# alexlee-gk/video_prediction

Measured on AMD Instinct MI355X. Metric: train frames/sec (whole node), BAIR 64x64 seq30 SAVP, higher is better.
Workload: dtype bf16

## Files before the change

### include/savp_hip.h

```cpp
#ifndef SAVP_HIP_H
#define SAVP_HIP_H

#include <stdint.h>

#ifdef __cplusplus
extern "C" {
#endif

#define SAVP_OK 0
#define SAVP_EINVAL (-1)
#define SAVP_ELAUNCH (-2)

const char* savp_version(void);

int savp_set_option(const char* name, int32_t value);
int savp_get_option(const char* name, int32_t* value);

int savp_allreduce_bucket(void* comm, void* stream, void* buf, int64_t count);

int savp_prof_event_create(void** ev);
int savp_prof_event_destroy(void* ev);
int savp_prof_arm(void* start, void* stop);
int savp_prof_armed(void);
int savp_prof_elapsed_us(void* start, void* stop, float* us);

enum { SAVP_CONV_FPROP = 0, SAVP_CONV_DGRAD = 1, SAVP_CONV_WGRAD = 2 };
enum { SAVP_PREC_F32 = 0, SAVP_PREC_BF16 = 1 };
enum { SAVP_ACT_NONE = 0, SAVP_ACT_LRELU = 1, SAVP_ACT_SIGMOID = 2, SAVP_ACT_DLRELU_FROM_OUT = 3 };

typedef struct SavpConvArgs {
    int32_t mode;
    int32_t N, D, H, W, Cx;
    int32_t Do, Ho, Wo, Cy;
    int32_t kd, kh, kw;
    int32_t sd, sh, sw;
    int32_t pd, ph, pw;
    int32_t beta;
    int32_t act;
    float alpha;
    int32_t splitk;
    int32_t tile;
    int32_t precision;
    void* x; int64_t x_sn, x_sd, x_sh, x_sw;
    void* y; int64_t y_sn, y_sd, y_sh, y_sw;
    void* w;
    const float* bias;
    const float* aux;
    const void* w_bf16;
    int32_t src_bf16;
    int32_t out_bf16;
    double* stats;
    void* ws; int64_t ws_bytes;
    int32_t dst_gap_at, dst_gap;
    const float* nb_x; int64_t nb_x_sn, nb_x_sp;
    const float *nb_mean, *nb_rstd;
    const float *nb_gamma, *nb_beta;
    double* nb_ws;
    int32_t nb_c0, nb_nc, nb_act; float nb_alpha;
    const void* w_frag;
    const void* w_frag_il;
} SavpConvArgs;

int savp_conv(void* stream, const SavpConvArgs* args);

int savp_tiled_z_weff(void* stream, const float* w, int32_t kh, int32_t kw, int32_t ph, int32_t pw, int32_t Cin, int32_t Cout,
                      int32_t z0, int32_t nz, float* weff);
int savp_tiled_z_grad(void* stream, const void* dy, int32_t dy_bf16, int64_t nimg, int32_t H, int32_t W, int32_t C,
                      const float* weff, int32_t nz, float* dz, int32_t beta, void* ws, int64_t ws_bytes);
int64_t savp_tiled_z_workspace_bytes(int64_t nimg, int32_t C);
int savp_conv_stats_ok(const SavpConvArgs* args);
int64_t savp_conv_workspace_bytes(const SavpConvArgs* args);
int savp_conv_special(const SavpConvArgs* args);


typedef struct SavpView { void* p; int64_t sn; int64_t sp; } SavpView;

typedef struct SavpInormArgs {
    int32_t N, HW, C;
    int32_t act; float alpha; float eps;
    SavpView x;
    const float* gamma; const float* beta;
    int32_t nout; SavpView out[4];
    float* mean; float* rstd;
    int32_t ndy; SavpView dy[4];
    SavpView dx; int32_t dx_beta;
    double* dgamma; double* dbeta;
    void* ws;
    int32_t ws_clean;
    int32_t out_c0[4], out_nc[4];
    int32_t dy_c0[4], dy_nc[4];
    int32_t out_bf16;
    int32_t stats_ready;
    const float* stats_shift;
    int32_t dx_bf16;
} SavpInormArgs;
int savp_instnorm_act_fwd(void* stream, const SavpInormArgs* a);
int savp_instnorm_act_bwd(void* stream, const SavpInormArgs* a);

typedef struct SavpGnormArgs {
    SavpInormArgs norm;
    int32_t G;
    double* ws_group;
    double* dsum;
} SavpGnormArgs;
int savp_groupnorm_act_fwd(void* stream, const SavpGnormArgs* a);
int savp_groupnorm_act_bwd(void* stream, const SavpGnormArgs* a);

typedef struct SavpLnLstmArgs {
    int32_t N, HW, F; float forget_bias;
    const float* gn;
    SavpView c_prev;
    float* c_pre;
    const float* cn;
    int32_t nh; SavpView h[4]; int32_t h_bf16;
    int32_t ndh; SavpView dh[4];
    const float* dc_new;
    float* dcn;
    float* dgn;
    const float* dc_pre;
    float* dc_prev;
} SavpLnLstmArgs;
int savp_lnlstm_fwd(void* stream, const SavpLnLstmArgs* a, int32_t stage);
int savp_lnlstm_bwd(void* stream, const SavpLnLstmArgs* a, int32_t stage);

typedef struct SavpLstmArgs {
    int32_t N, HW, F;
    float eps, forget_bias;
    const void* gates;
    SavpView c_prev;
    const float *gamma1, *beta1, *gamma2, *beta2;
    float* c_new;
    int32_t nh; SavpView h[4];
    float *mean1, *rstd1, *mean2, *rstd2;
    int32_t ndh; SavpView dh[4];
    const float* dc_new;
    float* dgates;
    float* dc_prev;
    double *dgamma1, *dbeta1, *dgamma2, *dbeta2;
    float* ws; int64_t ws_floats;
    float* ws_stats;
    int32_t ws_stats_clean;
    int32_t gates_bf16;
    int32_t stats1_ready;
    int32_t h_bf16;
    int32_t dgates_bf16;
    float* dgates_raw;
    int32_t no_norm;
} SavpLstmArgs;
int savp_convlstm_gates_fwd(void* stream, const SavpLstmArgs* a);
int savp_convlstm_gates_bwd(void* stream, const SavpLstmArgs* a);

int savp_tile_channels(void* stream, const float* z, int64_t R, int32_t HW, int32_t C, float scale, SavpView out, int32_t beta);
int savp_tile_channels_bf16(void* stream, const float* z, int64_t R, int32_t HW, int32_t C, float scale, SavpView out);
#define SAVP_COLSUM_WS_FLOATS (1024 * 4 * 256)
int savp_colsum(void* stream, SavpView in, int64_t R, int32_t HW, int32_t C, float scale, float* out, int32_t per_row,
                float* ws, int64_t ws_floats);
int savp_select(void* stream, int32_t N, int32_t HW, int32_t C, const int32_t* mask, SavpView a, SavpView b, int32_t nout,
                const SavpView* outs);
int savp_select_bwd(void* stream, int32_t N, int32_t HW, int32_t C, const int32_t* mask, int32_t nin, const SavpView* dins,
                    SavpView db);
int savp_gather_clips(void* stream, float* src, float* dst, const int32_t* t_start, int32_t B, int32_t clip, int64_t E,
                      int64_t src_t_stride, int32_t adjoint);
int savp_sigmoid_bwd(void* stream, SavpView dy, SavpView y, float* out, int64_t N, int32_t HW, int32_t C);
int savp_dense_fwd(void* stream, const float* x, int64_t x_row_stride, int32_t M, int64_t K, int32_t C, const float* W,
                   const float* bias, const float* scale, float* out, float* ws, int64_t ws_floats);
int savp_axpby(void* stream, int64_t n, float a, const float* x, float b, const float* y, float* out);
int savp_fill_view(void* stream, SavpView out, int64_t R, int32_t HW, int32_t C, float value);
int savp_adam(void* stream, int64_t n, float* p, const float* g, float* m, float* v, float lr_t, float beta1, float beta2,
              float eps, float gscale, const float* lr_t_dev);

int savp_cdna_kernels_fwd(void* stream, const float* raw, float* kern, int32_t N, int32_t kh, int32_t kw, int32_t K);
int savp_cdna_kernels_bwd(void* stream, const float* raw, const double* dkern, float* draw, int32_t N, int32_t kh, int32_t kw,
                          int32_t K);
typedef struct SavpCdnaArgs {
    int32_t N, H, W, C, K, kh, kw;
    SavpView img;
    const float* kern;
    SavpView out;
    SavpView dout;
    SavpView dimg; int32_t dimg_beta;
    double* dkern;
} SavpCdnaArgs;
int savp_cdna_apply_fwd(void* stream, const SavpCdnaArgs* a);
int savp_cdna_apply_bwd(void* stream, const SavpCdnaArgs* a);
#define SAVP_MAX_SOURCES 4
typedef struct SavpCdnaMultiArgs {
    int32_t N, H, W, C, K, kh, kw;
    int32_t nsrc;
    SavpView img[SAVP_MAX_SOURCES];
    const float* kern;
    SavpView out;
    SavpView dout;
    SavpView dimg[SAVP_MAX_SOURCES]; int32_t dimg_beta[SAVP_MAX_SOURCES];
    double* dkern;
} SavpCdnaMultiArgs;
int savp_cdna_apply_multi_fwd(void* stream, const SavpCdnaMultiArgs* a);
int savp_cdna_apply_multi_bwd(void* stream, const SavpCdnaMultiArgs* a);
typedef struct SavpCompositeArgs {
    int32_t N, HW, M, C;
    const float* logits;
    int32_t logits_stride;
    SavpView timgs;
    SavpView gen;
    float* masks;
    SavpView dgen;
    float* dlogits;
    SavpView drow;
    int32_t timgs_offset, row_channels;
    int32_t nnext; SavpView next[2];
    const int32_t* gt_mask;
    SavpView gt_img;
} SavpCompositeArgs;
int savp_composite_fwd(void* stream, const SavpCompositeArgs* a);
int savp_composite_bwd(void* stream, const SavpCompositeArgs* a);

typedef struct SavpConvLstmCellArgs { SavpConvArgs conv; SavpLstmArgs gates; } SavpConvLstmCellArgs;
typedef struct SavpConvNormArgs { SavpConvArgs conv; SavpInormArgs norm; } SavpConvNormArgs;
int savp_convlstm_cell_fwd(void* stream, const SavpConvLstmCellArgs* a);
int savp_convlstm_cell_bwd(void* stream, const SavpConvLstmCellArgs* a);
int savp_conv_in_act_fwd(void* stream, const SavpConvNormArgs* a);
int savp_conv_in_act_bwd(void* stream, const SavpConvNormArgs* a);

int savp_lstm_z_fwd(void* stream, const float* zs, const float* W, const float* bias, float* hout, float* gates, float* cs,
                    int32_t T, int32_t B, int32_t nz, float forget_bias);
int savp_lstm_z_bwd(void* stream, const float* zs, const float* W, const float* hout, const float* gates, const float* cs,
                    const float* dh_out, float* dzs, double* dW, double* db, int32_t T, int32_t B, int32_t nz, float forget_bias);
int savp_lstm_z_fwd_init(void* stream, const float* zs, const float* W, const float* bias, float* hout, float* gates, float* cs,
                         int32_t T, int32_t B, int32_t nz, float forget_bias, const float* c0, const float* h0);
int savp_lstm_z_bwd_init(void* stream, const float* zs, const float* W, const float* hout, const float* gates, const float* cs,
                         const float* dh_out, float* dzs, double* dW, double* db, int32_t T, int32_t B, int32_t nz, float forget_bias,
                         const float* c0, const float* h0, double* dc0, double* dh0);
int savp_lstm_seq_fwd(void* stream, float* A, const float* W, const float* bias, float* hout, float* gates, float* cs,
                      int32_t T, int32_t B, int32_t I, int32_t U, float forget_bias);
int savp_lstm_seq_bwd(void* stream, const float* A, const float* W, const float* gates, const float* cs, const float* dh_out,
                      float* dG, float* dA, int32_t T, int32_t B, int32_t I, int32_t U, float forget_bias);
int savp_gru_seq_fwd(void* stream, float* A, float* A2, const float* Wg, const float* bg, const float* Wc, const float* bc, float* hout,
                     float* ru, float* cand, int32_t T, int32_t B, int32_t I, int32_t U);
int savp_gru_seq_bwd(void* stream, const float* A, const float* Wg, const float* Wc, const float* ru, const float* cand, const float* dh_out,
                     float* dGg, float* dGc, float* dA, int32_t T, int32_t B, int32_t I, int32_t U);
int savp_gru_seq_fwd_init(void* stream, float* A, float* A2, const float* Wg, const float* bg, const float* Wc, const float* bc, float* hout,
                          float* ru, float* cand, int32_t T, int32_t B, int32_t I, int32_t U, const float* h0);
int savp_gru_seq_bwd_init(void* stream, const float* A, const float* Wg, const float* Wc, const float* ru, const float* cand, const float* dh_out,
                          float* dGg, float* dGc, float* dA, int32_t T, int32_t B, int32_t I, int32_t U, double* dh0);
int savp_kl_gauss(void* stream, int64_t n, int32_t rows, const float* mu1, const float* ls1_raw, const float* mu2,
                  const float* ls2_raw, double* kl_out, float klw, const float* klw_dev, float* dmu1, float* dls1, float* dmu2,
                  float* dls2);
int savp_reparam_fwd(void* stream, int64_t n, int32_t rows, const float* mu, const float* ls_raw, const float* eps, float* ls,
                     float* z, double* kl_out);
int savp_reparam_bwd(void* stream, int64_t n, int32_t rows, const float* mu, const float* ls_raw, const float* eps,
                     const float* dz, float klw, float* dmu, float* dls_raw, const float* klw_dev);
int savp_lp_loss(void* stream, int64_t rows, int64_t row_len, int64_t pred_row_stride, int64_t target_row_stride, int32_t p2,
                 const float* pred, const float* target, float weight, double* loss_out, float* dpred);
int savp_tv_loss(void* stream, const float* flows, int32_t n_img, int32_t H, int32_t W, int32_t C, int64_t img_stride, int64_t px_stride,
                 float s1, float s2, float weight, double* loss_out, float* dflows);
int savp_gan_loss(void* stream, int32_t n, int32_t type, const float* logits, float label, float weight, double* loss_out,
                  float* dlogits, int32_t beta);
int savp_lsgan_loss(void* stream, int32_t n, const float* logits, float label, float weight, double* loss_out, float* dlogits,
                    int32_t beta);
int savp_cosine_distance(void* stream, int64_t P, int32_t C, const float* f0, const float* f1, float weight, float eps,
                         double* loss_out, float* df0, int32_t beta);

int savp_pack_weights(void* stream, const float* src, int64_t T, int32_t Cx, int32_t Cy, const float* scale, float* wt, float* wd,
                      void* wt_bf16, void* wd_bf16);

typedef struct {
    const float* src; const float* scale;
    float* wt; float* wd; void* wt_bf16; void* wd_bf16;
    int64_t T; int32_t Cx, Cy;
} SavpPackItem;
int savp_pack_weights_batch(void* stream, int32_t n, const SavpPackItem* items);
int savp_fold_pool(void* stream, const float* in, float* out, int32_t k, int64_t C, int32_t adjoint);
int savp_fold_bilinear(void* stream, const float* in, float* out, int32_t k, int32_t Cin, int32_t F, int32_t adjoint);
int savp_sn_fwd(void* stream, const float* W, int64_t K, int32_t C, const float* u, float* ws, float* u_new);
int savp_sn_bwd(void* stream, const float* W, int64_t K, int32_t C, const float* u, float* ws, const float* G, float* dW,
                int32_t beta);
typedef struct SavpSnItem {
    const float* W; int64_t K; int32_t C; const float* u; float* ws; float* u_new; const float* G; float* dW; int32_t beta;
} SavpSnItem;
int savp_sn_fwd_batch(void* stream, int32_t n, const SavpSnItem* items);
int savp_sn_bwd_batch(void* stream, int32_t n, const SavpSnItem* items);

typedef struct SavpWarpArgs {
    int32_t N, H, W, C, K;
    SavpView img;
    const float* flows;
    SavpView out;
    SavpView dout;
    float* dflows;
    float* dimg;
} SavpWarpArgs;
int savp_image_warp_fwd(void* stream, const SavpWarpArgs* a);
int savp_image_warp_bwd(void* stream, const SavpWarpArgs* a);
typedef struct SavpDnaArgs {
    int32_t N, H, W, C, K, kh, kw;
    SavpView img;
    const float* raw;
    float* kern;
    SavpView out;
    SavpView dout;
    float* draw;
    SavpView dimg; int32_t dimg_beta;
} SavpDnaArgs;
int savp_dna_apply_fwd(void* stream, const SavpDnaArgs* a);
int savp_dna_apply_bwd(void* stream, const SavpDnaArgs* a);
typedef struct SavpWarpMultiArgs {
    int32_t N, H, W, C, K;
    int32_t nsrc;
    SavpView img[SAVP_MAX_SOURCES];
    const float* flows;
    SavpView out;
    SavpView dout;
    float* dflows;
    SavpView dimg[SAVP_MAX_SOURCES]; int32_t dimg_beta[SAVP_MAX_SOURCES];
} SavpWarpMultiArgs;
int savp_image_warp_multi_fwd(void* stream, const SavpWarpMultiArgs* a);
int savp_image_warp_multi_bwd(void* stream, const SavpWarpMultiArgs* a);
typedef struct SavpDnaMultiArgs {
    int32_t N, H, W, C, K, kh, kw;
    int32_t nsrc;
    SavpView img[SAVP_MAX_SOURCES];
    const float* raw;
    float* kern;
    SavpView out;
    SavpView dout;
    float* draw;
    SavpView dimg[SAVP_MAX_SOURCES]; int32_t dimg_beta[SAVP_MAX_SOURCES];
} SavpDnaMultiArgs;
int savp_dna_apply_multi_fwd(void* stream, const SavpDnaMultiArgs* a);
int savp_dna_apply_multi_bwd(void* stream, const SavpDnaMultiArgs* a);

typedef struct SavpGruArgs {
    int32_t N, HW, F;
    float eps;
    const float* pre;
    SavpView h;
    const float *gamma, *beta;
    float *mean, *rstd;
    float* u;
    SavpView rh;
    int32_t nout; SavpView out[4];
    int32_t ndy; SavpView dy[4];
    float* dpre;
    float* du;
    SavpView dh;
    SavpView drh;
    double *dgamma, *dbeta;
} SavpGruArgs;
int savp_convgru_gates_fwd(void* stream, const SavpGruArgs* a);
int savp_convgru_out_fwd(void* stream, const SavpGruArgs* a);
int savp_convgru_out_bwd(void* stream, const SavpGruArgs* a);
int savp_convgru_gates_bwd(void* stream, const SavpGruArgs* a);

int savp_u8_frames_to_f32(void* stream, const uint8_t* in, float* out, int32_t B, int32_t T, int64_t frame);

int savp_frame_mse_psnr(void* stream, const float* a, int64_t a_st, int64_t a_sb, const float* b, int64_t b_st, int64_t b_sb,
                        int32_t T, int32_t B, int32_t inner, float* mse, float* psnr);
int savp_frame_ssim(void* stream, const float* a, int64_t a_st, int64_t a_sb, const float* b, int64_t b_st, int64_t b_sb,
                    int32_t T, int32_t B, int32_t H, int32_t W, int32_t C, float* out);
int savp_eval_accumulate(void* stream, const float* metric, float* vmin, float* vsum, float* vmax, int32_t* cond_min,
                         int32_t* cond_max, int32_t T, int32_t B);
int savp_select_batch(void* stream, const int32_t* cond, const float* x, int64_t x_st, int64_t x_sb, float* out, int64_t o_st,
                      int64_t o_sb, int32_t T, int32_t B, int32_t inner, int32_t mode);

#define SAVP_EVAL_PSNR 0
#define SAVP_EVAL_MSE 1
#define SAVP_EVAL_SSIM 2
#define SAVP_EVAL_NMETRICS 3
typedef struct {
    float *vmin, *vsum, *vmax;
    float *gmin, *gsum, *gmax;
} SavpEvalFoldState;
int64_t savp_eval_fold_ws_floats(int32_t F, int32_t S, int32_t B, int32_t C);
int savp_eval_fold_samples(void* stream, const float* target, int64_t t_st, int64_t t_sb, const float* pred, int64_t p_st, int64_t p_sb,
                           int32_t F, int32_t T1, int32_t S, int32_t B, int32_t H, int32_t W, int32_t C, const int32_t* n_valid,
                           const SavpEvalFoldState* states, float* ws, int64_t ws_floats);

int savp_fold_f64(void* stream, const int32_t* idx, int64_t n, double* src, float* dst);

int savp_state_pred_fwd(void* stream, int32_t T, int32_t N, int32_t na, int32_t ns, const float* actions, const float* states_in,
                        const int32_t* gt, const float* W, const float* b, float* sa, float* gen);
int savp_state_pred_bwd(void* stream, int32_t T, int32_t N, int32_t na, int32_t ns, const int32_t* gt, const float* W, const float* sa,
                        float* dgen, double* dW, double* db);

int64_t savp_gate_weights_bytes(int32_t taps, int32_t Cx, int32_t Cy);
int savp_pack_gate_weights(void* stream, const float* src, int32_t taps, int32_t Cx, int32_t Cy, void* out, int32_t interleave);

int savp_debug_poison_lds(void* stream, uint32_t pattern, void* sink);
int savp_debug_fill_u32(void* stream, void* p, int64_t words, uint32_t pattern);
int savp_debug_probe_lds(void* stream, uint32_t pattern, void* out2);

#ifdef __cplusplus
}
#endif
#endif
```

### video_prediction_amd/csrc/common.hip

```cpp
#include <hip/hip_runtime.h>
#include <dlfcn.h>
#include <string.h>
#include "savp_hip.h"
#include "opts.h"
#include "conv_common.h"

extern "C" const char* savp_version(void) { return "savp_hip 0.1 gfx950"; }

thread_local hipEvent_t g_savp_prof_start = nullptr;
thread_local hipEvent_t g_savp_prof_stop = nullptr;

extern "C" int savp_prof_event_create(void** ev) {
    if (!ev) return SAVP_EINVAL;
    hipEvent_t e;
    if (hipEventCreate(&e) != hipSuccess) return SAVP_ELAUNCH;
    *ev = (void*)e;
    return SAVP_OK;
}
extern "C" int savp_prof_event_destroy(void* ev) { return (ev && hipEventDestroy((hipEvent_t)ev) == hipSuccess) ? SAVP_OK : SAVP_EINVAL; }
extern "C" int savp_prof_arm(void* start, void* stop) {
    if ((start == nullptr) != (stop == nullptr)) return SAVP_EINVAL;
    g_savp_prof_start = (hipEvent_t)start; g_savp_prof_stop = (hipEvent_t)stop;
    return SAVP_OK;
}
extern "C" int savp_prof_armed(void) { return g_savp_prof_start != nullptr; }
extern "C" int savp_prof_elapsed_us(void* start, void* stop, float* us) {
    if (!start || !stop || !us) return SAVP_EINVAL;
    float ms = 0.f;
    if (hipEventElapsedTime(&ms, (hipEvent_t)start, (hipEvent_t)stop) != hipSuccess) return SAVP_ELAUNCH;
    *us = ms * 1e3f;
    return SAVP_OK;
}

static struct { const char* name; int value; } g_opts[OPT_COUNT] = {
    {"conv_ring", 0}, {"s2dgrad", 1}, {"thin", 1}, {"wgp_cfg", 0}, {"wgp_split", 0}, {"inorm_min_hw", 64}, {"colsum_2stage", 1},
    {"dense_legacy", 0}, {"cdna_legacy", 0}, {"lstm_fused", 1}, {"ring_dma", 1}, {"lstm_q", 0}, {"ring_wwarm", 1}, {"wgp_dma", 1}, {"ring_early", 1}, {"gate_kernel", 1}, {"gate_alt", 0}, {"gate_cell", 1}, {"gate_wwarm", 1}, {"splitk_reduced", 0},
};
int savp_opt(int id) { return g_opts[id].value; }
void savp_opt_count(int id) { ++g_opts[id].value; }
extern "C" int savp_set_option(const char* name, int value) {
    if (!name) return SAVP_EINVAL;
    for (int i = 0; i < OPT_COUNT; ++i)
        if (!strcmp(g_opts[i].name, name)) { g_opts[i].value = value; return SAVP_OK; }
    return SAVP_EINVAL;
}
extern "C" int savp_get_option(const char* name, int* value) {
    if (!name || !value) return SAVP_EINVAL;
    for (int i = 0; i < OPT_COUNT; ++i)
        if (!strcmp(g_opts[i].name, name)) { *value = g_opts[i].value; return SAVP_OK; }
    return SAVP_EINVAL;
}

typedef int (*rccl_allreduce_fn)(const void*, void*, size_t, int, int, void*, hipStream_t);
extern "C" int savp_allreduce_bucket(void* comm, void* stream, void* buf, int64_t count) {
    if (!comm || !buf || count < 0) return SAVP_EINVAL;
    if (count == 0) return SAVP_OK;
    static rccl_allreduce_fn fn = nullptr;
    if (!fn) {
        void* h = dlopen("librccl.so", RTLD_NOW | RTLD_GLOBAL);
        if (!h) h = dlopen("librccl.so.1", RTLD_NOW | RTLD_GLOBAL);
        if (!h) h = dlopen("/opt/rocm/lib/librccl.so", RTLD_NOW | RTLD_GLOBAL);
        if (!h) return SAVP_ELAUNCH;
        fn = (rccl_allreduce_fn)dlsym(h, "ncclAllReduce");
        if (!fn) return SAVP_ELAUNCH;
    }
    return fn(buf, buf, (size_t)count, 7, 0, comm, (hipStream_t)stream) == 0 ? SAVP_OK : SAVP_ELAUNCH;
}

int splitk_fit(const SavpConvArgs* a, int want, long long block_elems) {
    if (want <= 1) return 1;
    if (!a->ws || a->ws_bytes <= 0 || block_elems <= 0 || (((uintptr_t)a->ws) & 15)) { savp_opt_count(OPT_SPLITK_REDUCED); return 1; }
    const long long fit = a->ws_bytes / (block_elems * (long long)sizeof(float));
    if (fit < want) savp_opt_count(OPT_SPLITK_REDUCED);
    if (fit < 2) return 1;
    return want < fit ? want : (int)fit;
}

__global__ __launch_bounds__(256) void splitk_fold_kernel(float* __restrict__ out, const float* __restrict__ part, int splitk, long long n4, long long n,
                                                          int beta, int Cd, int gap_at, int gap) {
    const long long stride = (long long)gridDim.x * 256;
    for (long long i = (long long)blockIdx.x * 256 + threadIdx.x; i < n4; i += stride) {
        float4 s = beta ? reinterpret_cast<const float4*>(out)[i] : make_float4(0.f, 0.f, 0.f, 0.f);
        for (int k = 0; k < splitk; ++k) {
            const float4 v = reinterpret_cast<const float4*>(part + (long long)k * n)[i];
            s.x += v.x; s.y += v.y; s.z += v.z; s.w += v.w;
        }
        if (gap) {
            const int c = (int)((i * 4) % Cd);
            float* e = &s.x;
#pragma unroll
            for (int j = 0; j < 4; ++j)
                if (c + j >= gap_at && c + j < gap_at + gap) e[j] = beta ? reinterpret_cast<const float*>(out)[i * 4 + j] : 0.f;
        }
        reinterpret_cast<float4*>(out)[i] = s;
    }
}

__global__ __launch_bounds__(256) void splitk_fold_scalar_kernel(float* __restrict__ out, const float* __restrict__ part, int splitk, long long n, int beta,
                                                                 int Cd, int gap_at, int gap) {
    const long long stride = (long long)gridDim.x * 256;
    for (long long i = (long long)blockIdx.x * 256 + threadIdx.x; i < n; i += stride) {
        const int c = (int)(i % Cd);
        if (gap && c >= gap_at && c < gap_at + gap) { if (!beta) out[i] = 0.f; continue; }
        float s = beta ? out[i] : 0.f;
        for (int k = 0; k < splitk; ++k) s += part[(long long)k * n + i];
        out[i] = s;
    }
}

void splitk_fold(float* out, const float* part, int splitk, long long n, int beta, int Cd, int gap_at, int gap, hipStream_t st) {
    const bool vec = (n % 4 == 0) && (Cd % 4 == 0) && ((((uintptr_t)out) & 15) == 0) && ((((uintptr_t)part) & 15) == 0);
    const long long work = vec ? n / 4 : n;
    long long blocks = (work + 255) / 256;
    if (blocks > 2048) blocks = 2048;
    if (blocks < 1) blocks = 1;
    if (vec) hipLaunchKernelGGL(splitk_fold_kernel, dim3((unsigned)blocks), dim3(256), 0, st, out, part, splitk, n / 4, n, beta, Cd, gap_at, gap);
    else hipLaunchKernelGGL(splitk_fold_scalar_kernel, dim3((unsigned)blocks), dim3(256), 0, st, out, part, splitk, n, beta, Cd, gap_at, gap);
}

typedef float fold_f4 __attribute__((ext_vector_type(4)));
template <bool VEC>
__global__ __launch_bounds__(256) void wgrad_fold_kernel(float* __restrict__ out, const float* __restrict__ part, int nsplit, long long n, long long slice) {
    const long long i = (long long)blockIdx.x * 256 + threadIdx.x;
    if (i >= n) return;
    if constexpr (VEC) {
        fold_f4 s = reinterpret_cast<const fold_f4*>(out)[i];
        const fold_f4* __restrict__ q = reinterpret_cast<const fold_f4*>(part) + i;
        const long long st4 = slice >> 2;
        int k = 0;
        for (; k + 8 <= nsplit; k += 8) {
            fold_f4 v[8];
#pragma unroll
            for (int j = 0; j < 8; ++j) v[j] = __builtin_nontemporal_load(q + (long long)(k + j) * st4);
#pragma unroll
            for (int j = 0; j < 8; ++j) s += v[j];
        }
        for (; k < nsplit; ++k) s += __builtin_nontemporal_load(q + (long long)k * st4);
        reinterpret_cast<fold_f4*>(out)[i] = s;
    } else {
        float s = out[i];
        for (int k = 0; k < nsplit; ++k) s += part[(long long)k * slice + i];
        out[i] = s;
    }
}

void wgrad_fold(float* out, const float* part, int nsplit, long long n, hipStream_t st, long long slice) {
    if (nsplit < 1 || n <= 0) return;
    if (slice <= 0) slice = n;
    const bool vec = (n % 4 == 0) && (slice % 4 == 0) && ((((uintptr_t)out) & 15) == 0) && ((((uintptr_t)part) & 15) == 0);
    const long long work = vec ? n / 4 : n;
    const unsigned blocks = (unsigned)((work + 255) / 256);
    if (vec) hipLaunchKernelGGL(wgrad_fold_kernel<true>, dim3(blocks), dim3(256), 0, st, out, part, nsplit, work, slice);
    else hipLaunchKernelGGL(wgrad_fold_kernel<false>, dim3(blocks), dim3(256), 0, st, out, part, nsplit, work, slice);
}
```

### video_prediction_amd/csrc/conv_common.h

```cpp
#pragma once
#include <hip/hip_runtime.h>
#include <stdint.h>
#include "savp_hip.h"
#include "opts.h"

typedef float f32x16 __attribute__((ext_vector_type(16)));
typedef __bf16 bf16x8 __attribute__((ext_vector_type(8)));
typedef __bf16 bf16x4 __attribute__((ext_vector_type(4)));

#define BK 32
#define BKP 36
#define NTHREADS 256

struct DimGeom {
    int Mdim;
    int base, mstep;
    int jstep;
    int nt;
    int t0, tstep;
    int ob, os;
    int srcN;
};

__host__ __device__ __forceinline__ DimGeom make_geom(bool dgrad, int f, int In, int Out, int k, int s, int p) {
    DimGeom g;
    if (!dgrad) {
        g.Mdim = Out; g.base = -p; g.mstep = s; g.jstep = 1; g.nt = k; g.t0 = 0; g.tstep = 1;
        g.ob = 0; g.os = 1; g.srcN = In;
    } else {
        int u0 = (f + p) % s;
        g.nt = (k > u0) ? (k - u0 + s - 1) / s : 0;
        g.base = (f + p - u0) / s; g.mstep = 1; g.jstep = -1;
        g.t0 = u0; g.tstep = s;
        g.Mdim = (In > f) ? (In - f + s - 1) / s : 0;
        g.ob = f; g.os = s; g.srcN = Out;
    }
    return g;
}

struct ConvP {
    int mode;
    int N, D, H, W, Cx;
    int Do, Ho, Wo, Cy;
    int kd, kh, kw, sd, sh, sw, pd, ph, pw;
    int beta, act;
    float alpha;
    const float* x; long long x_sn, x_sd, x_sh, x_sw;
    const float* y; long long y_sn, y_sd, y_sh, y_sw;
    const float* w;
    const unsigned short* w16;
    float* out;
    const float* bias;
    const float* aux;
    int splitk;
    float* part; long long part_sz;
    int bf16;
    int tm, tn;
    unsigned long long magW, magHW, magDHW;
    int s1_pitch, s1_nch, s1_spp;
    int s1_ph, s1_pw, s1_th, s1_tw, s1_tih;
    unsigned long long s1_magDm;
    unsigned long long s1_magPI, s1_magPW, s1_magC4;
    int src16;
    int cell;
    double* stats;
    int dma_patch;
    const void* zero16;
    unsigned long long s1_magPI8, s1_magP8, s1_magC8;
    int pre;
    const float* nb_x; long long nb_x_sn, nb_x_sp; const float *nb_mean, *nb_rstd, *nb_gamma, *nb_beta; double* nb_ws;
    int nb_c0, nb_nc, nb_act; float nb_alpha;
    int gap_at, gap;
    int wwarm;
    int early;
    DimGeom gD, gH, gW;
    int s1_tih_sh;
    int s1_ngs, s1_itper;
    unsigned long long s1_magTm, s1_magTHW, s1_magTW;
    unsigned long long s1_magKw, s1_magSpp, s1_magTail;
};

__device__ __forceinline__ unsigned fastdiv(unsigned p, unsigned long long magic) {
    return (unsigned)(((unsigned long long)p * magic) >> 40);
}

__device__ __forceinline__ float4 ldg4(const float* p) { return *reinterpret_cast<const float4*>(p); }

__device__ __forceinline__ int xcd_logical(int b, int n) {
    const int q = n >> 3, r = n & 7, xcd = b & 7;
    return (xcd < r ? xcd * (q + 1) : r * (q + 1) + (xcd - r) * q) + (b >> 3);
}


static inline unsigned long long magic40(int d) {
    if (d <= 0) d = 1;
    return ((1ULL << 40) + (unsigned long long)d - 1ULL) / (unsigned long long)d;
}

static inline void patch_launch_constants(ConvP& p, const SavpConvArgs* a, int phases, int tih, int nch, int spp, int tW, int splitk) {
    const bool dg = a->mode == SAVP_CONV_DGRAD;
    int sh_ = 0;
    while ((1 << sh_) < tih) ++sh_;
    p.s1_tih_sh = sh_;
    const int ngs = (nch + spp - 1) / spp;
    p.s1_ngs = ngs;
    p.pre = 0;
    if (phases != 1 || (dg && (a->sh != 1 || a->sw != 1))) return;
    p.gD = make_geom(dg, 0, a->D, a->Do, a->kd, 1, a->pd);
    p.gH = make_geom(dg, 0, a->H, a->Ho, a->kh, a->sh, a->ph);
    p.gW = make_geom(dg, 0, a->W, a->Wo, a->kw, a->sw, a->pw);
    const long long it_all = (long long)p.gD.nt * p.gH.nt * p.gW.nt * nch;
    p.s1_itper = (int)((it_all + splitk - 1) / splitk);
    const int thw = p.s1_th * tW;
    p.s1_magTm = magic40(p.tm); p.s1_magTHW = magic40(thw); p.s1_magTW = magic40(tW);
    p.s1_magKw = magic40(p.gW.nt); p.s1_magSpp = magic40(spp); p.s1_magTail = magic40(nch - (ngs - 1) * spp);
    if ((long long)p.tm * p.tn < (1 << 24) && p.tm < 65536 && thw < 65536 && it_all < (1 << 24) && p.gW.nt >= 1 && p.gH.nt >= 1) p.pre = 1;
}

bool conv_thin_try(const SavpConvArgs* a, hipStream_t st, int* rc);
bool conv_thin_applies(const SavpConvArgs* a);
long long conv_thin_workspace_bytes(const SavpConvArgs* a);

bool conv_s2dgrad_try(const SavpConvArgs* a, hipStream_t st, int* rc);
bool conv_s2dgrad_applies(const SavpConvArgs* a);

extern thread_local hipEvent_t g_savp_prof_start, g_savp_prof_stop;

int splitk_fit(const SavpConvArgs* a, int want, long long block_elems);
void splitk_fold(float* out, const float* part, int splitk, long long n, int beta, int Cd, int gap_at, int gap, hipStream_t st);

static inline bool aligned16(const void* p) { return (((uintptr_t)p) & 15) == 0; }

#ifdef SAVP_CONV_ABLATE
#include <stdlib.h>
static __constant__ int g_ablate;
#define ABL(bit) (g_ablate & (bit))
static inline void ablate_init() {
    static bool done = false;
    if (!done) { const char* e = getenv("SAVP_ABLATE"); int v = e ? atoi(e) : 0; hipMemcpyToSymbol(HIP_SYMBOL(g_ablate), &v, sizeof(int)); done = true; }
}
#else
#define ABL(bit) false
static inline void ablate_init() {}
#endif

bool conv_patch_try(ConvP& p, const SavpConvArgs* a, int wm, int wn, bool forced, hipStream_t st, int* rc);
bool conv_wgrad_patch_try(ConvP& p, const SavpConvArgs* a, hipStream_t st, int* rc, long long* plan_bytes = nullptr);
void wgrad_fold(float* out, const float* part, int nsplit, long long n, hipStream_t st, long long slice = 0);
bool conv_ring_try(ConvP& p, const SavpConvArgs* a, int wm, int wn, hipStream_t st, int* rc, bool dry = false);
bool conv_gate_applies(const SavpConvArgs* a);
bool conv_gate_try(const SavpConvArgs* a, hipStream_t st, int* rc);
struct SavpConvLstmCellArgs;
bool conv_gate_cell_try(const SavpConvLstmCellArgs* c, hipStream_t st, int* rc);
```

### video_prediction_amd/csrc/conv_igemm.hip

```cpp
#include <hip/hip_runtime.h>
#include <stdint.h>
#include "savp_hip.h"
#include "zero_fill.h"

#include "conv_common.h"
#include <stdlib.h>

template <int WM, int WN, bool VEC, bool BF16, bool WB16>
__global__ __launch_bounds__(NTHREADS) void conv_fd_kernel(ConvP p) {
    constexpr int BM = 64 * WM, BN = 64 * WN;
    constexpr int BKT = BF16 ? 64 : 32;
    constexpr int KV = BKT / 4;
    constexpr int RP = NTHREADS / KV;
    constexpr int RA = BM / RP, RB = BN / RP;
    constexpr int ROWB = BF16 ? (BKT + 8) * 2 : BKP * 4;
    extern __shared__ __attribute__((aligned(16))) float smem[];
    char* As = reinterpret_cast<char*>(smem);
    char* Bs = As + 2 * BM * ROWB;

    const bool dgrad = (p.mode == SAVP_CONV_DGRAD);
    const int split = blockIdx.z % p.splitk;
    int fz = blockIdx.z / p.splitk;
    int fw = dgrad ? fz % p.sw : 0; fz = dgrad ? fz / p.sw : 0;
    int fh = dgrad ? fz % p.sh : 0; fz = dgrad ? fz / p.sh : 0;
// ... 449 lines not shown

template <int WM, int WN>
__global__ __launch_bounds__(NTHREADS) void conv_wgrad_bf16_kernel(ConvP p) {
    constexpr int BM = 64 * WM, BN = 64 * WN;
    constexpr int BKT = 64;
    constexpr int ROWB = (BKT + 8) * 2;
    constexpr int PA = BM / 64, PB = BN / 64;
    extern __shared__ __attribute__((aligned(16))) float smem[];
    char* As = reinterpret_cast<char*>(smem);
    char* Bs = As + 2 * BM * ROWB;

    const int M = p.kd * p.kh * p.kw * p.Cx;
    const int Nn = p.Cy;
    const int HWo = p.Ho * p.Wo, DHWo = p.Do * HWo;
    const int Ktot = p.N * DHWo;
    const int llog = xcd_logical(blockIdx.x, p.tm * p.tn * p.splitk);
    const int zsplit = llog / (p.tm * p.tn), tl = llog % (p.tm * p.tn);
    const int m0 = (tl % p.tm) * BM, n0 = (tl / p.tm) * BN;
    const int ktiles = (Ktot + BKT - 1) / BKT;
    const int per = (ktiles + p.splitk - 1) / p.splitk;
    const int kt_begin = zsplit * per;
    const int kt_end = min(ktiles, kt_begin + per);
    if (kt_begin >= kt_end) return;

    const float* __restrict__ X = p.x;
    const float* __restrict__ Y = p.y;
    const int tid = threadIdx.x, lane = tid & 63, wave = tid >> 6;
    const int kq = tid & 15, rq0 = tid >> 4;

    int a_c[PA], a_td[PA], a_th[PA], a_tw[PA]; bool a_ok[PA];
#pragma unroll
    for (int j = 0; j < PA; ++j) {
        int m = m0 + 4 * (rq0 + 16 * j);
        a_ok[j] = m < M;
        int mm = a_ok[j] ? m : 0;
        a_c[j] = mm % p.Cx; int tap = mm / p.Cx;
        a_tw[j] = tap % p.kw; tap /= p.kw;
        a_th[j] = tap % p.kh; a_td[j] = tap / p.kh;
    }
    int b_n[PB]; bool b_ok[PB];
#pragma unroll
    for (int j = 0; j < PB; ++j) { b_n[j] = n0 + 4 * (rq0 + 16 * j); b_ok[j] = b_n[j] < Nn; }

    float4 ra[PA][4], rb[PB][4];

    auto fetch = [&](int kt) {
        if (ABL(1)) return;
#pragma unroll
        for (int i = 0; i < 4; ++i) {
            const int pix = kt * BKT + kq * 4 + i;
            const bool pok = pix < Ktot;
            unsigned up = (unsigned)(pok ? pix : 0);
            int n = (int)fastdiv(up, p.magDHW); unsigned r = up - (unsigned)n * DHWo;
            int od = (int)fastdiv(r, p.magHW); r -= (unsigned)od * HWo;
            int oy = (int)fastdiv(r, p.magW); int ox = (int)(r - (unsigned)oy * p.Wo);
            const long long nb = (long long)n * p.x_sn;
#pragma unroll
            for (int j = 0; j < PA; ++j) {
                int zd = od * p.sd - p.pd + a_td[j], zh = oy * p.sh - p.ph + a_th[j], zw = ox * p.sw - p.pw + a_tw[j];
                float4 v = make_float4(0.f, 0.f, 0.f, 0.f);
                if (pok && a_ok[j] && (unsigned)zd < (unsigned)p.D && (unsigned)zh < (unsigned)p.H && (unsigned)zw < (unsigned)p.W)
                    v = ldg4(X + nb + zd * p.x_sd + zh * p.x_sh + zw * p.x_sw + a_c[j]);
                ra[j][i] = v;
            }
            const float* q = Y + (long long)n * p.y_sn + od * p.y_sd + oy * p.y_sh + ox * p.y_sw;
#pragma unroll
            for (int j = 0; j < PB; ++j) {
                float4 v = make_float4(0.f, 0.f, 0.f, 0.f);
                if (pok && b_ok[j]) v = ldg4(q + b_n[j]);
                rb[j][i] = v;
            }
        }
    };
    auto stage = [&](int buf) {
        if (ABL(64)) return;
        char* a = As + buf * BM * ROWB;
        char* b = Bs + buf * BN * ROWB;
#pragma unroll
        for (int j = 0; j < PA; ++j) {
            char* base = a + (4 * (rq0 + 16 * j)) * ROWB + kq * 8;
            bf16x4 v0 = {(__bf16)ra[j][0].x, (__bf16)ra[j][1].x, (__bf16)ra[j][2].x, (__bf16)ra[j][3].x};
            bf16x4 v1 = {(__bf16)ra[j][0].y, (__bf16)ra[j][1].y, (__bf16)ra[j][2].y, (__bf16)ra[j][3].y};
            bf16x4 v2 = {(__bf16)ra[j][0].z, (__bf16)ra[j][1].z, (__bf16)ra[j][2].z, (__bf16)ra[j][3].z};
            bf16x4 v3 = {(__bf16)ra[j][0].w, (__bf16)ra[j][1].w, (__bf16)ra[j][2].w, (__bf16)ra[j][3].w};
            *reinterpret_cast<bf16x4*>(base) = v0;
            *reinterpret_cast<bf16x4*>(base + ROWB) = v1;
            *reinterpret_cast<bf16x4*>(base + 2 * ROWB) = v2;
            *reinterpret_cast<bf16x4*>(base + 3 * ROWB) = v3;
        }
#pragma unroll
        for (int j = 0; j < PB; ++j) {
            char* base = b + (4 * (rq0 + 16 * j)) * ROWB + kq * 8;
            bf16x4 v0 = {(__bf16)rb[j][0].x, (__bf16)rb[j][1].x, (__bf16)rb[j][2].x, (__bf16)rb[j][3].x};
            bf16x4 v1 = {(__bf16)rb[j][0].y, (__bf16)rb[j][1].y, (__bf16)rb[j][2].y, (__bf16)rb[j][3].y};
            bf16x4 v2 = {(__bf16)rb[j][0].z, (__bf16)rb[j][1].z, (__bf16)rb[j][2].z, (__bf16)rb[j][3].z};
            bf16x4 v3 = {(__bf16)rb[j][0].w, (__bf16)rb[j][1].w, (__bf16)rb[j][2].w, (__bf16)rb[j][3].w};
            *reinterpret_cast<bf16x4*>(base) = v0;
            *reinterpret_cast<bf16x4*>(base + ROWB) = v1;
            *reinterpret_cast<bf16x4*>(base + 2 * ROWB) = v2;
            *reinterpret_cast<bf16x4*>(base + 3 * ROWB) = v3;
        }
    };

    f32x16 acc[WM][WN];
#pragma unroll
    for (int i = 0; i < WM; ++i)
#pragma unroll
        for (int j = 0; j < WN; ++j)
#pragma unroll
            for (int r = 0; r < 16; ++r) acc[i][j][r] = 0.f;

    const int wm0 = (wave >> 1) * 32 * WM, wn0 = (wave & 1) * 32 * WN;
    const int l31 = lane & 31, khalf = lane >> 5;

    fetch(kt_begin);
    stage(0);
    __syncthreads();
    for (int kt = kt_begin; kt < kt_end; ++kt) {
        const int cur = (kt - kt_begin) & 1;
        if (kt + 1 < kt_end) fetch(kt + 1);
        const char* a = As + cur * BM * ROWB;
        const char* b = Bs + cur * BN * ROWB;
#pragma unroll
        for (int ks = 0; ks < (ABL(2) ? 0 : BKT / 16); ++ks) {
            bf16x8 af[WM], bf[WN];
#pragma unroll
            for (int i = 0; i < WM; ++i)
                af[i] = *reinterpret_cast<const bf16x8*>(a + (wm0 + i * 32 + l31) * ROWB + (ks * 16 + khalf * 8) * 2);
#pragma unroll
            for (int j = 0; j < WN; ++j)
                bf[j] = *reinterpret_cast<const bf16x8*>(b + (wn0 + j * 32 + l31) * ROWB + (ks * 16 + khalf * 8) * 2);
#pragma unroll
            for (int i = 0; i < WM; ++i)
#pragma unroll
                for (int j = 0; j < WN; ++j)
                    acc[i][j] = __builtin_amdgcn_mfma_f32_32x32x16_bf16(af[i], bf[j], acc[i][j], 0, 0, 0);
        }
        if (kt + 1 < kt_end) stage(cur ^ 1);
        __syncthreads();
    }

    const bool sliced = p.part != nullptr;
    float* __restrict__ dW = sliced ? p.part + (long long)zsplit * p.part_sz : p.out;
#pragma unroll
    for (int j = 0; j < WN; ++j) {
        const int col = n0 + wn0 + j * 32 + l31;
        if (col >= Nn) continue;
#pragma unroll
        for (int i = 0; i < WM; ++i)
#pragma unroll
            for (int r = 0; r < 16; ++r) {
                const int row = m0 + wm0 + i * 32 + (r & 3) + 8 * (r >> 2) + 4 * khalf;
                if (row < M) {
                    if (sliced) dW[(long long)row * Nn + col] = acc[i][j][r];
                    else unsafeAtomicAdd(dW + (long long)row * Nn + col, acc[i][j][r]);
                }
            }
    }
}

template <int WM, int WN>
static hipError_t launch_wg_bf16(const ConvP& p, dim3 grid, hipStream_t st) {
    size_t lds = (size_t)2 * (64 * WM + 64 * WN) * (64 + 8) * 2;
    static bool attr_done = false;
    if (!attr_done) {
        hipFuncSetAttribute((const void*)conv_wgrad_bf16_kernel<WM, WN>, hipFuncAttributeMaxDynamicSharedMemorySize, (int)lds);
        attr_done = true;
    }
    hipLaunchKernelGGL((conv_wgrad_bf16_kernel<WM, WN>), grid, dim3(NTHREADS), lds, st, p);
    return hipGetLastError();
}


template <int WM, int WN, bool VEC, bool BF16, bool WB16 = false>
static hipError_t launch_fd1(const ConvP& p, dim3 grid, hipStream_t st) {
    constexpr int BKT = BF16 ? 64 : 32;
    constexpr size_t rowb = BF16 ? (BKT + 8) * 2 : BKP * 4;
    size_t lds = (size_t)2 * (64 * WM + 64 * WN) * rowb;
    if (lds < (size_t)64 * WM * sizeof(long long)) lds = (size_t)64 * WM * sizeof(long long);
    static bool attr_done = false;
    if (!attr_done) {
        hipFuncSetAttribute((const void*)conv_fd_kernel<WM, WN, VEC, BF16, WB16>, hipFuncAttributeMaxDynamicSharedMemorySize, (int)lds);
        attr_done = true;
    }
    hipLaunchKernelGGL((conv_fd_kernel<WM, WN, VEC, BF16, WB16>), grid, dim3(NTHREADS), lds, st, p);
    return hipGetLastError();
}

template <int WM, int WN>
static hipError_t launch_fd(const ConvP& p, bool vec, dim3 grid, hipStream_t st) {
    if (p.bf16 && vec && p.w16) return launch_fd1<WM, WN, true, true, true>(p, grid, st);
    if (p.bf16) return vec ? launch_fd1<WM, WN, true, true>(p, grid, st) : launch_fd1<WM, WN, false, true>(p, grid, st);
    return vec ? launch_fd1<WM, WN, true, false>(p, grid, st) : launch_fd1<WM, WN, false, false>(p, grid, st);
}

template <int WM, int WN>
static hipError_t launch_wg(const ConvP& p, bool va, bool vb, dim3 grid, hipStream_t st) {
    size_t lds = (size_t)2 * BK * ((64 * WM + 4) + (64 * WN + 4)) * sizeof(float);
#define WG_CASE(A, B)                                                                                              \
    {                                                                                                              \
        hipFuncSetAttribute((const void*)conv_wgrad_kernel<WM, WN, A, B>, hipFuncAttributeMaxDynamicSharedMemorySize, \
                            (int)lds);                                                                             \
        hipLaunchKernelGGL((conv_wgrad_kernel<WM, WN, A, B>), grid, dim3(NTHREADS), lds, st, p);                   \
    }
    if (va && vb) WG_CASE(true, true)
    else if (va) WG_CASE(true, false)
    else if (vb) WG_CASE(false, true)
    else WG_CASE(false, false)
#undef WG_CASE
    return hipGetLastError();
}


static void pick_tile(long long M, long long N, int& wm, int& wn) {
    const int opts[4][2] = {{2, 2}, {2, 1}, {1, 2}, {1, 1}};
    double best = 1e300;
    for (int i = 0; i < 4; ++i) {
        long long bm = 64 * opts[i][0], bn = 64 * opts[i][1];
        long long tm = (M + bm - 1) / bm, tn = (N + bn - 1) / bn;
        double wgs = (double)tm * tn;
        double rounds = wgs <= 256.0 ? 1.0 : wgs / 256.0;
        double eff = (bm * bn == 128 * 128) ? 1.0 : (bm * bn == 64 * 64 ? 1.3 : 1.12);
        double cost = rounds * (double)(bm * bn) * eff;
        if (cost < best) { best = cost; wm = opts[i][0]; wn = opts[i][1]; }
    }
}

static bool ring_default() {
    return savp_opt(OPT_CONV_RING) != 0;
}

struct WgPlan { int wm, wn, splitk; long long M, ktiles, part_sz; bool va, vb, wbf16; };
static bool wgrad_generic_plan(const SavpConvArgs* a, bool bf16, int wm, int wn, WgPlan& g) {
    const bool xs4 = (a->x_sn % 4 == 0) && (a->x_sd % 4 == 0) && (a->x_sh % 4 == 0) && (a->x_sw % 4 == 0) && aligned16(a->x);
    const bool ys4 = (a->y_sn % 4 == 0) && (a->y_sd % 4 == 0) && (a->y_sh % 4 == 0) && (a->y_sw % 4 == 0) && aligned16(a->y);
    g.M = (long long)a->kd * a->kh * a->kw * a->Cx;
    const long long Ktot = (long long)a->N * a->Do * a->Ho * a->Wo;
    if (Ktot <= 0 || (double)Ktot * (double)((long long)a->Do * a->Ho * a->Wo) >= 1099511627776.0) return false;
    g.va = (a->Cx % 4 == 0) && xs4;
    g.vb = (a->Cy % 4 == 0) && ys4;
    if (!wm) {
        wm = (g.M > 64) ? 2 : 1;
        wn = (a->Cy > 64) ? 2 : 1;
    }
    g.wm = wm; g.wn = wn;
    const int BM = 64 * wm, BN = 64 * wn;
    const long long tiles = ((g.M + BM - 1) / BM) * ((a->Cy + BN - 1) / BN);
    g.wbf16 = bf16 && g.va && g.vb;
    const int bkt = g.wbf16 ? 64 : BK;
    g.ktiles = (Ktot + bkt - 1) / bkt;
    long long splitk = a->splitk;
    if (splitk <= 0) {
        long long want = (512 + tiles - 1) / tiles;
        long long maxs = g.ktiles / 8 > 0 ? g.ktiles / 8 : 1;
        splitk = want < maxs ? want : maxs;
    }
    if (splitk > g.ktiles) splitk = g.ktiles;
    if (splitk < 1) splitk = 1;
    const long long per = (g.ktiles + splitk - 1) / splitk;
    g.splitk = (int)((g.ktiles + per - 1) / per);
    g.part_sz = g.M * a->Cy;
    return true;
}

extern "C" int64_t savp_conv_workspace_bytes(const SavpConvArgs* a) {
    if (!a) return 0;
    if (a->mode == SAVP_CONV_FPROP || a->mode == SAVP_CONV_DGRAD) {
        if (a->act != SAVP_ACT_NONE || a->out_bf16 || a->stats || a->splitk == 1) return 0;
        const bool dg = a->mode == SAVP_CONV_DGRAD;
        const long long dD = dg ? a->D : a->Do, dH = dg ? a->H : a->Ho, dW_ = dg ? a->W : a->Wo;
        const long long Cd = (dg ? a->Cx : a->Cy) + (a->dst_gap > 0 ? a->dst_gap : 0);
        const long long block = (long long)a->N * dD * dH * dW_ * Cd;
        long long S = a->splitk;
        if (S <= 0) {
            const long long tiles = ((block / Cd + 255) / 256) * ((Cd + 127) / 128);
            if (tiles > 192) return 0;
            S = 512 / tiles;
            if (S > 16) S = 16;
        }
        return S > 1 ? S * block * (long long)sizeof(float) : 0;
    }
    if (a->mode != SAVP_CONV_WGRAD) return 0;
    const int algo = (a->tile >> 8) & 3;
    long long need = 0;
    const long long thin = algo == 0 ? conv_thin_workspace_bytes(a) : 0;
    if (thin) need = thin;
    else {
        int wm = 0, wn = 0;
        if (a->tile & 0xff) { wm = (a->tile >> 4) & 15; wn = a->tile & 15; if (wm < 1 || wm > 2 || wn < 1 || wn > 2) return 0; }
        ConvP p;
        p.bf16 = (a->precision == SAVP_PREC_BF16) ? 1 : 0;
        int rc = SAVP_OK;
        long long patch_bytes = 0;
        WgPlan g;
        if (algo != 1 && conv_wgrad_patch_try(p, a, nullptr, &rc, &patch_bytes)) need = patch_bytes;
        else if (algo != 2 && wgrad_generic_plan(a, p.bf16 != 0, wm, wn, g) && g.splitk > 1) need = (long long)g.splitk * g.part_sz * (long long)sizeof(float);
        const long long bias = a->bias ? (long long)SAVP_COLSUM_WS_FLOATS * 4 : 0;
        if (bias > need) need = bias;
    }
    return need;
}

extern "C" int savp_conv_special(const SavpConvArgs* a) {
    if (a && conv_gate_applies(a)) return 1;
    if (!a || ((a->tile >> 8) & 3) != 0) return 0;
    return (conv_thin_applies(a) || conv_s2dgrad_applies(a) || conv_gate_applies(a)) ? 1 : 0;
}

extern "C" int savp_conv_stats_ok(const SavpConvArgs* a) {
    if (!a || (a->mode != SAVP_CONV_FPROP && a->mode != SAVP_CONV_DGRAD) || a->precision != SAVP_PREC_BF16) return 0;
    if (((a->tile >> 8) & 3) == 0 && (conv_thin_applies(a) || conv_s2dgrad_applies(a))) return 0;
    const bool dg = a->mode == SAVP_CONV_DGRAD;
    const int Cred = dg ? a->Cy : a->Cx;
    if (!(a->w_bf16 && (Cred % 8 == 0) && aligned16(a->w_bf16))) return 0;
    ConvP p;
    p.bf16 = 1; p.w16 = (const unsigned short*)a->w_bf16; p.src16 = a->src_bf16 ? 1 : 0; p.splitk = 1; p.tm = p.tn = 1;
    p.gap_at = a->dst_gap ? a->dst_gap_at : 0x7fffffff; p.gap = a->dst_gap;
    p.nb_ws = (double*)a->nb_ws; p.nb_c0 = a->nb_c0; p.nb_nc = a->nb_nc; p.part = nullptr; p.part_sz = 0;
    if (a->dst_gap && !a->nb_ws) return 0;
    SavpConvArgs b = *a;
    if (!b.stats && !b.nb_ws) b.stats = (double*)(uintptr_t)16;
    int wm = 0, wn = 0;
    if (b.tile & 0xff) { wm = (b.tile >> 4) & 15; wn = b.tile & 15; if (wm < 1 || wm > 2 || wn < 1 || wn > 2) return 0; }
    int rc = SAVP_OK;
    return conv_ring_try(p, &b, wm, wn, nullptr, &rc, true) ? 1 : 0;
}

extern "C" int savp_conv(void* stream, const SavpConvArgs* a) {
    if (!a || !a->x || !a->y || !a->w) return SAVP_EINVAL;
    if (a->sd < 1 || a->sh < 1 || a->sw < 1 || a->kd < 1 || a->kh < 1 || a->kw < 1) return SAVP_EINVAL;
    hipStream_t st = (hipStream_t)stream;
    ConvP p;
    p.mode = a->mode;
    p.N = a->N; p.D = a->D; p.H = a->H; p.W = a->W; p.Cx = a->Cx;
    p.Do = a->Do; p.Ho = a->Ho; p.Wo = a->Wo; p.Cy = a->Cy;
    p.kd = a->kd; p.kh = a->kh; p.kw = a->kw; p.sd = a->sd; p.sh = a->sh; p.sw = a->sw;
    p.pd = a->pd; p.ph = a->ph; p.pw = a->pw;
    p.beta = a->beta; p.act = a->act; p.alpha = a->alpha;
    p.x = (const float*)a->x; p.x_sn = a->x_sn; p.x_sd = a->x_sd; p.x_sh = a->x_sh; p.x_sw = a->x_sw;
    p.y = (const float*)a->y; p.y_sn = a->y_sn; p.y_sd = a->y_sd; p.y_sh = a->y_sh; p.y_sw = a->y_sw;
    p.w = (const float*)a->w;
    p.w16 = nullptr;
    p.bias = a->bias; p.aux = a->aux;
    p.splitk = 1; p.tm = p.tn = 1; p.part = nullptr; p.part_sz = 0;
    p.src16 = a->src_bf16 ? 1 : 0; p.cell = 0; p.stats = nullptr;
    p.bf16 = (a->precision == SAVP_PREC_BF16) ? 1 : 0;
    const bool gapped = a->dst_gap != 0;
    if (gapped && (a->dst_gap < 0 || a->dst_gap_at < 0 || a->mode == SAVP_CONV_WGRAD)) return SAVP_EINVAL;
    p.gap_at = gapped ? a->dst_gap_at : 0x7fffffff; p.gap = gapped ? a->dst_gap : 0;
    p.nb_ws = (double*)a->nb_ws;
    if (a->nb_ws) {
        if (a->mode == SAVP_CONV_WGRAD || !a->nb_x || !a->nb_mean || !a->nb_rstd || !a->nb_gamma || !a->nb_beta || a->nb_c0 < 0 || a->nb_nc < 1 ||
            a->nb_act < 0 || a->nb_act > 2)
            return SAVP_EINVAL;
        p.nb_x = a->nb_x; p.nb_x_sn = a->nb_x_sn; p.nb_x_sp = a->nb_x_sp; p.nb_mean = a->nb_mean; p.nb_rstd = a->nb_rstd;
        p.nb_gamma = a->nb_gamma; p.nb_beta = a->nb_beta; p.nb_c0 = a->nb_c0; p.nb_nc = a->nb_nc; p.nb_act = a->nb_act; p.nb_alpha = a->nb_alpha;
    }
    p.magW = magic40(a->Wo); p.magHW = magic40(a->Ho * a->Wo); p.magDHW = magic40(a->Do * a->Ho * a->Wo);
    int wm = 0, wn = 0;
    const int algo = (a->tile >> 8) & 3;
    if (a->tile & 0xff) { wm = (a->tile >> 4) & 15; wn = a->tile & 15; if (wm < 1 || wm > 2 || wn < 1 || wn > 2) return SAVP_EINVAL; }
    hipError_t err;
    ablate_init();
    const bool xs4 = (a->x_sn % 4 == 0) && (a->x_sd % 4 == 0) && (a->x_sh % 4 == 0) && (a->x_sw % 4 == 0) && aligned16(a->x);
    const bool ys4 = (a->y_sn % 4 == 0) && (a->y_sd % 4 == 0) && (a->y_sh % 4 == 0) && (a->y_sw % 4 == 0) && aligned16(a->y);
    if (algo == 0 && !gapped && !a->nb_ws) {
        int rc = SAVP_OK;
        if (conv_thin_try(a, st, &rc)) return rc;
    }
    if (algo == 0 && !gapped && !a->nb_ws && a->mode == SAVP_CONV_DGRAD) {
        int rc = SAVP_OK;
        if (conv_s2dgrad_try(a, st, &rc)) return rc;
    }
    if (a->mode == SAVP_CONV_FPROP) {
        int rc = SAVP_OK;
        if (conv_gate_try(a, st, &rc)) return rc;
    }
    if (a->mode == SAVP_CONV_FPROP || a->mode == SAVP_CONV_DGRAD) {
        const bool dg = a->mode == SAVP_CONV_DGRAD;
        p.out = (float*)(dg ? a->x : a->y);
        const int Cred = dg ? a->Cy : a->Cx;
        const int Nout = dg ? a->Cx : a->Cy;
        const bool vec = (Cred % 4 == 0) && (dg ? ys4 : xs4) && aligned16(a->w);
        if (a->w_bf16 && (Cred % 8 == 0) && aligned16(a->w_bf16)) p.w16 = (const unsigned short*)a->w_bf16;
        long long Mmax;
        int phases = 1;
        if (dg) {
            phases = a->sd * a->sh * a->sw;
            Mmax = (long long)a->N * ((a->D + a->sd - 1) / a->sd) * ((a->H + a->sh - 1) / a->sh) * ((a->W + a->sw - 1) / a->sw);
        } else {
            Mmax = (long long)a->N * a->Do * a->Ho * a->Wo;
        }
        if (Mmax <= 0 || Nout <= 0) return SAVP_EINVAL;
        const bool needs_ring = a->out_bf16 || a->src_bf16 || a->stats || gapped || a->nb_ws;
        if (algo == 3 || needs_ring || (algo == 0 && ring_default())) {
            int rc = SAVP_OK;
            if (conv_ring_try(p, a, wm, wn, st, &rc)) return rc;
            if (algo == 3 || needs_ring) return SAVP_EINVAL;
        }
        if (algo != 1) {
            int rc = SAVP_OK;
            if (conv_patch_try(p, a, wm, wn, algo == 2, st, &rc)) return rc;
            if (algo == 2) return SAVP_EINVAL;
        }
        if (!wm) pick_tile(Mmax * phases, Nout, wm, wn);
        const int BM = 64 * wm, BN = 64 * wn;
        int splitk = a->splitk;
        const long long tiles = ((Mmax + BM - 1) / BM) * ((Nout + BN - 1) / BN) * phases;
        const long long taps_max = (long long)a->kd * a->kh * a->kw / (dg ? phases : 1);
        const long long nkt = (taps_max * Cred + (p.bf16 ? 63 : 31)) / (p.bf16 ? 64 : 32);
        const bool can_split = (a->act == SAVP_ACT_NONE);
        if (!can_split) splitk = 1;
        else if (splitk <= 0) {
            splitk = 1;
            if (tiles <= 192 && nkt >= 16) {
                long long s1 = 512 / tiles, s2 = nkt / 8;
                splitk = (int)(s1 < s2 ? s1 : s2);
                if (splitk < 1) splitk = 1;
                if (splitk > 16) splitk = 16;
            }
        }
        if (splitk > 1) {
            const long long dD = dg ? a->D : a->Do, dH = dg ? a->H : a->Ho, dW_ = dg ? a->W : a->Wo;
            const long long s_n = dg ? a->x_sn : a->y_sn, s_d = dg ? a->x_sd : a->y_sd, s_h = dg ? a->x_sh : a->y_sh,
                            s_w = dg ? a->x_sw : a->y_sw;
            const bool dense = (s_w == Nout) && (s_h == dW_ * Nout) && (dD == 1 || s_d == dH * dW_ * Nout) &&
                               (s_n == dD * dH * dW_ * Nout);
            if (!dense) splitk = 1;
            else {
                p.part_sz = (long long)a->N * dD * dH * dW_ * Nout;
                splitk = splitk_fit(a, splitk, p.part_sz);
                p.part = (float*)a->ws;
            }
        }
        p.splitk = splitk;
        p.tm = (int)((Mmax + BM - 1) / BM); p.tn = (int)((Nout + BN - 1) / BN);
        dim3 grid((unsigned)(p.tm * p.tn), 1, (unsigned)(phases * splitk));
        if (wm == 2 && wn == 2) err = launch_fd<2, 2>(p, vec, grid, st);
        else if (wm == 2 && wn == 1) err = launch_fd<2, 1>(p, vec, grid, st);
        else if (wm == 1 && wn == 2) err = launch_fd<1, 2>(p, vec, grid, st);
        else err = launch_fd<1, 1>(p, vec, grid, st);
        if (splitk > 1 && err == hipSuccess) {
            splitk_fold(p.out, p.part, splitk, p.part_sz, a->beta, Nout, 0, 0, st);
            err = hipGetLastError();
        }
    } else if (a->mode == SAVP_CONV_WGRAD) {
        p.out = (float*)a->w;
        if (algo != 1) {
            int rc = SAVP_OK;
            if (conv_wgrad_patch_try(p, a, st, &rc)) return rc;
            if (algo == 2) return SAVP_EINVAL;
        }
        if (a->src_bf16 || a->out_bf16) return SAVP_EINVAL;
        WgPlan g;
        if (!wgrad_generic_plan(a, p.bf16 != 0, wm, wn, g)) return SAVP_EINVAL;
        wm = g.wm; wn = g.wn;
        const long long M = g.M, ktiles = g.ktiles;
        const bool va = g.va, vb = g.vb, wbf16 = g.wbf16;
        const int BM = 64 * wm, BN = 64 * wn;
        int splitk = g.splitk;
        p.part = nullptr; p.part_sz = g.part_sz;
        if (splitk > 1) {
            const int fit = splitk_fit(a, splitk, p.part_sz);
            if (fit > 1) {
                const long long per = (ktiles + fit - 1) / fit;
                splitk = (int)((ktiles + per - 1) / per);
                p.part = (float*)a->ws;
            }
        }
        p.splitk = splitk;
        p.tm = (int)((M + BM - 1) / BM); p.tn = (int)((a->Cy + BN - 1) / BN);
        dim3 grid((unsigned)(p.tm * p.tn * splitk), 1, 1);
        if (wbf16) {
            if (wm == 2 && wn == 2) err = launch_wg_bf16<2, 2>(p, grid, st);
            else if (wm == 2 && wn == 1) err = launch_wg_bf16<2, 1>(p, grid, st);
            else if (wm == 1 && wn == 2) err = launch_wg_bf16<1, 2>(p, grid, st);
            else err = launch_wg_bf16<1, 1>(p, grid, st);
        } else if (wm == 2 && wn == 2) err = launch_wg<2, 2>(p, va, vb, grid, st);
        else if (wm == 2 && wn == 1) err = launch_wg<2, 1>(p, va, vb, grid, st);
        else if (wm == 1 && wn == 2) err = launch_wg<1, 2>(p, va, vb, grid, st);
        else err = launch_wg<1, 1>(p, va, vb, grid, st);
        if (p.part && err == hipSuccess) {
            wgrad_fold(p.out, p.part, splitk, p.part_sz, st);
            err = hipGetLastError();
        }
        if (a->bias && err == hipSuccess) {
            const long long px = (long long)a->Do * a->Ho * a->Wo;
            const bool joint = (a->y_sh == a->Wo * a->y_sw) && (a->Do == 1 || a->y_sd == a->Ho * a->y_sh);
            if (!joint) return SAVP_EINVAL;
            SavpView yv; yv.p = (void*)a->y; yv.sn = a->y_sn; yv.sp = a->y_sw;
            int rc2 = savp_colsum(stream, yv, a->N, (int32_t)px, a->Cy, 1.f, (float*)a->bias, 0, (float*)a->ws, a->ws ? a->ws_bytes / 4 : 0);
            if (rc2 != SAVP_OK) return rc2;
        }
    } else {
        return SAVP_EINVAL;
    }
    return err == hipSuccess ? SAVP_OK : SAVP_ELAUNCH;
}
```

### video_prediction_amd/csrc/opts.h

```cpp
#pragma once

enum SavpOptId {
    OPT_CONV_RING = 0,
    OPT_S2DGRAD,
    OPT_THIN,
    OPT_WGP_CFG,
    OPT_WGP_SPLIT,
    OPT_INORM_MIN_HW,
    OPT_COLSUM_2STAGE,
    OPT_DENSE_LEGACY,
    OPT_CDNA_LEGACY,
    OPT_LSTM_FUSED,
    OPT_RING_DMA,
    OPT_LSTM_Q,
    OPT_RING_WWARM,
    OPT_WGP_DMA,
    OPT_RING_EARLY,
    OPT_GATE_KERNEL,
    OPT_GATE_ALT,
    OPT_GATE_CELL,
    OPT_GATE_WWARM,
    OPT_SPLITK_REDUCED,
    OPT_COUNT
};

int savp_opt(int id);
void savp_opt_count(int id);

#ifdef __HIPCC__
template <int BYTES>
__device__ __forceinline__ void kernarg_warm() {
    constexpr int LINES = (BYTES + 63) / 64;
    const unsigned long long ka = (unsigned long long)__builtin_amdgcn_kernarg_segment_ptr();
    unsigned t[LINES];
#pragma unroll
    for (int i = 0; i < LINES; ++i) asm volatile("s_load_dword %0, %1, %2" : "=&s"(t[i]) : "s"(ka), "n"(i * 64) : "memory");
    asm volatile("s_waitcnt lgkmcnt(0)" ::: "memory");
#pragma unroll
    for (int i = 0; i < LINES; ++i) asm volatile("" :: "s"(t[i]));
}
#endif
```

### video_prediction_amd/csrc/weight_prep.hip

```cpp
#include <hip/hip_runtime.h>
#include <stdint.h>
#include "savp_hip.h"
#include "zero_fill.h"

#define NT 256
#define LAUNCH_OK() (hipGetLastError() == hipSuccess ? SAVP_OK : SAVP_ELAUNCH)

__device__ __forceinline__ float wsum(float v) {
#pragma unroll
    for (int o = 32; o > 0; o >>= 1) v += __shfl_xor(v, o);
    return v;
}
__device__ __forceinline__ float block_sum1(float v, float* sh) {
    const int lane = threadIdx.x & 63, wave = threadIdx.x >> 6;
    __syncthreads();
    float s = wsum(v);
    if (lane == 0) sh[wave] = s;
    __syncthreads();
    float t = 0.f;
    for (int w = 0; w < (int)(blockDim.x >> 6); ++w) t += sh[w];
    return t;
}

__global__ void pack_weights_kernel(const float* __restrict__ src, long long T, int Cx, int Cy, const float* scale, float* wt,
                                    float* wd, __bf16* wt16, __bf16* wd16) {
    const long long total = T * Cx * Cy;
    const float s = scale ? *scale : 1.f;
    for (long long i = blockIdx.x * (long long)blockDim.x + threadIdx.x; i < total; i += (long long)gridDim.x * blockDim.x) {
        int cy = (int)(i % Cy);
        long long r = i / Cy;
        int cx = (int)(r % Cx);
        long long t = r / Cx;
        float v = src[i] * s;
        if (wt) wt[(long long)cy * (T * Cx) + t * Cx + cx] = v;
        if (wd) wd[(long long)cx * (T * Cy) + t * Cy + cy] = v;
        if (wt16) wt16[(long long)cy * (T * Cx) + t * Cx + cx] = (__bf16)v;
        if (wd16) wd16[(long long)cx * (T * Cy) + t * Cy + cy] = (__bf16)v;
    }
}

extern "C" int savp_pack_weights(void* stream, const float* src, int64_t T, int32_t Cx, int32_t Cy, const float* scale,
                                 float* wt, float* wd, void* wt_bf16, void* wd_bf16) {
    if (!src || (!wt && !wd && !wt_bf16 && !wd_bf16)) return SAVP_EINVAL;
    long long total = (long long)T * Cx * Cy;
    unsigned nb = (unsigned)((total + NT - 1) / NT);
    if (nb > 8192) nb = 8192;
    hipLaunchKernelGGL(pack_weights_kernel, dim3(nb), dim3(NT), 0, (hipStream_t)stream, src, (long long)T, Cx, Cy, scale, wt, wd,
                       (__bf16*)wt_bf16, (__bf16*)wd_bf16);
    return LAUNCH_OK();
}

#define PACK_MAX 32
struct PackBatch {
    const float* src[PACK_MAX]; const float* scale[PACK_MAX];
    float* wt[PACK_MAX]; float* wd[PACK_MAX]; __bf16* wt16[PACK_MAX]; __bf16* wd16[PACK_MAX];
    long long T[PACK_MAX]; int Cx[PACK_MAX], Cy[PACK_MAX];
};

#define PK_T 64
__global__ __launch_bounds__(256) void pack_weights_batch_kernel(PackBatch b) {
    __shared__ float tile[PK_T][PK_T + 1];
    const int it = blockIdx.y;
    const float* __restrict__ src = b.src[it];
    const long long T = b.T[it];
    const int Cx = b.Cx[it], Cy = b.Cy[it];
    float* __restrict__ wt = b.wt[it]; float* __restrict__ wd = b.wd[it];
    __bf16* __restrict__ wt16 = b.wt16[it]; __bf16* __restrict__ wd16 = b.wd16[it];
    const long long R = T * Cx;
    const float s = b.scale[it] ? *b.scale[it] : 1.f;
    const int tc = (Cy + PK_T - 1) / PK_T;
    const long long tiles = ((R + PK_T - 1) / PK_T) * tc;
    const int tx = threadIdx.x & 63, ty = threadIdx.x >> 6;
    for (long long tl = blockIdx.x; tl < tiles; tl += gridDim.x) {
        const long long r0 = (tl / tc) * PK_T;
        const int c0 = (int)(tl % tc) * PK_T;
        __syncthreads();
#pragma unroll 4
        for (int j = ty; j < PK_T; j += 4) {
            const long long r = r0 + j;
            const int cy = c0 + tx;
            if (r < R && cy < Cy) {
                const float v = src[r * Cy + cy] * s;
                tile[j][tx] = v;
                const long long t = r / Cx;
                const int cx = (int)(r - t * Cx);
                const long long o = (long long)cx * (T * Cy) + t * Cy + cy;
                if (wd) wd[o] = v;
                if (wd16) wd16[o] = (__bf16)v;
            }
        }
        __syncthreads();
        if (wt || wt16) {
#pragma unroll 4
            for (int j = ty; j < PK_T; j += 4) {
                const int cy = c0 + j;
                const long long r = r0 + tx;
                if (r < R && cy < Cy) {
                    const float v = tile[tx][j];
                    if (wt) wt[(long long)cy * R + r] = v;
                    if (wt16) wt16[(long long)cy * R + r] = (__bf16)v;
                }
            }
        }
    }
}

extern "C" int savp_pack_weights_batch(void* stream, int32_t n, const SavpPackItem* items) {
    if (!items || n < 1 || n > PACK_MAX) return SAVP_EINVAL;
    PackBatch b;
    long long most = 0;
    for (int i = 0; i < n; ++i) {
        const SavpPackItem& q = items[i];
        if (!q.src || (!q.wt && !q.wd && !q.wt_bf16 && !q.wd_bf16) || q.T < 1 || q.Cx < 1 || q.Cy < 1) return SAVP_EINVAL;
        b.src[i] = q.src; b.scale[i] = q.scale; b.wt[i] = q.wt; b.wd[i] = q.wd;
        b.wt16[i] = (__bf16*)q.wt_bf16; b.wd16[i] = (__bf16*)q.wd_bf16;
        b.T[i] = q.T; b.Cx[i] = q.Cx; b.Cy[i] = q.Cy;
        const long long tiles = (((long long)q.T * q.Cx + PK_T - 1) / PK_T) * ((q.Cy + PK_T - 1) / PK_T);
        if (tiles > most) most = tiles;
    }
    long long nb = most;
    if (nb > 512) nb = 512;
    hipLaunchKernelGGL(pack_weights_batch_kernel, dim3((unsigned)nb, (unsigned)n), dim3(256), 0, (hipStream_t)stream, b);
    return LAUNCH_OK();
}

__global__ void fold_pool_kernel(const float* __restrict__ in, float* __restrict__ out, int k, long long C, int adjoint) {
    const int ko = k + 1;
    const long long total = adjoint ? (long long)k * k * C : (long long)ko * ko * C;
    for (long long i = blockIdx.x * (long long)blockDim.x + threadIdx.x; i < total; i += (long long)gridDim.x * blockDim.x) {
        long long c = i % C;
        long long r = i / C;
        float s = 0.f;
        if (!adjoint) {
            int b = (int)(r % ko), a = (int)(r / ko);
            for (int di = 0; di < 2; ++di)
                for (int dj = 0; dj < 2; ++dj) {
                    int u = a - di, v = b - dj;
                    if (u >= 0 && u < k && v >= 0 && v < k) s += in[((long long)u * k + v) * C + c];
                }
            out[i] = 0.25f * s;
        } else {
            int v = (int)(r % k), u = (int)(r / k);
            for (int di = 0; di < 2; ++di)
                for (int dj = 0; dj < 2; ++dj) s += in[((long long)(u + di) * ko + (v + dj)) * C + c];
            out[i] += 0.25f * s;
        }
    }
}

extern "C" int savp_fold_pool(void* stream, const float* in, float* out, int32_t k, int64_t C, int32_t adjoint) {
    if (!in || !out || k < 1) return SAVP_EINVAL;
    long long total = (long long)(k + 1) * (k + 1) * C;
    unsigned nb = (unsigned)((total + NT - 1) / NT);
    if (nb > 8192) nb = 8192;
    hipLaunchKernelGGL(fold_pool_kernel, dim3(nb), dim3(NT), 0, (hipStream_t)stream, in, out, k, (long long)C, adjoint);
    return LAUNCH_OK();
}

__device__ __forceinline__ float bil1(int i) { return (i == 0 || i == 3) ? 0.25f : ((i == 1 || i == 2) ? 0.75f : 0.f); }

__global__ void fold_bilinear_kernel(const float* __restrict__ in, float* __restrict__ out, int k, int Cin, int F, int adjoint) {
    const int ko = k + 3;
    const long long total = adjoint ? (long long)k * k * Cin * F : (long long)ko * ko * Cin * F;
    for (long long i = blockIdx.x * (long long)blockDim.x + threadIdx.x; i < total; i += (long long)gridDim.x * blockDim.x) {
        if (!adjoint) {
            int ci = (int)(i % Cin); long long r = i / Cin;
            int f = (int)(r % F); r /= F;
            int b = (int)(r % ko), a = (int)(r / ko);
            float s = 0.f;
            for (int u = 0; u < k; ++u) {
                float wu = bil1(a + u - (k - 1));
                if (wu == 0.f) continue;
                for (int v = 0; v < k; ++v) {
                    float wv = bil1(b + v - (k - 1));
                    if (wv == 0.f) continue;
                    s += wu * wv * in[(((long long)u * k + v) * Cin + ci) * F + f];
                }
            }
            out[i] = s;
        } else {
            int f = (int)(i % F); long long r = i / F;
            int ci = (int)(r % Cin); r /= Cin;
            int v = (int)(r % k), u = (int)(r / k);
            float s = 0.f;
            for (int a = 0; a < ko; ++a) {
                float wu = bil1(a + u - (k - 1));
                if (wu == 0.f) continue;
                for (int b = 0; b < ko; ++b) {
                    float wv = bil1(b + v - (k - 1));
                    if (wv == 0.f) continue;
                    s += wu * wv * in[(((long long)a * ko + b) * F + f) * Cin + ci];
                }
            }
            out[i] += s;
        }
    }
}

extern "C" int savp_fold_bilinear(void* stream, const float* in, float* out, int32_t k, int32_t Cin, int32_t F, int32_t adjoint) {
    if (!in || !out || k < 1) return SAVP_EINVAL;
    long long total = (long long)(k + 3) * (k + 3) * Cin * F;
    unsigned nb = (unsigned)((total + NT - 1) / NT);
    if (nb > 8192) nb = 8192;
    hipLaunchKernelGGL(fold_bilinear_kernel, dim3(nb), dim3(NT), 0, (hipStream_t)stream, in, out, k, Cin, F, adjoint);
    return LAUNCH_OK();
}

#define SN_EPS 1e-12f
__host__ __device__ __forceinline__ double* sn_acc64(float* ws, long long K, int C) { return reinterpret_cast<double*>(ws + 8 + 2 * C + 2 * K); }

__device__ __forceinline__ void sn_rows_body(const float* __restrict__ W, long long K, int C, const float* __restrict__ x,
                                             float xscale, float* __restrict__ y, double* sq, const float* z, double* dotz, int bx, int gx) {
    const int lane = threadIdx.x & 63, wave = threadIdx.x >> 6;
    float sqacc = 0.f, dzacc = 0.f;
    for (long long k = bx * 4LL + wave; k < K; k += (long long)gx * 4) {
        float s = 0.f;
        for (int c = lane; c < C; c += 64) s += W[k * C + c] * x[c];
        s = wsum(s) * xscale;
        if (lane == 0) {
            y[k] = s;
            sqacc += s * s;
            if (z) dzacc += s * z[k];
        }
    }
    if (lane == 0) {
        if (sq) unsafeAtomicAdd(sq, (double)sqacc);
        if (dotz) unsafeAtomicAdd(dotz, (double)dzacc);
    }
}

__global__ __launch_bounds__(NT) void sn_gemv_rows_kernel(const float* __restrict__ W, long long K, int C, const float* __restrict__ x,
                                                          float xscale, float* __restrict__ y, double* sq, const float* z,
                                                          double* dotz) {
    sn_rows_body(W, K, C, x, xscale, y, sq, z, dotz, blockIdx.x, gridDim.x);
}

__device__ __forceinline__ void sn_rows_vec_body(const float* __restrict__ W, long long K, int C, const float* __restrict__ x,
                                                 float xscale, float* __restrict__ y, double* sq, const float* z, double* dotz, int bx, int gx) {
    const int lane = threadIdx.x & 63, wave = threadIdx.x >> 6;
    const int lpr = C >> 2, rpw = 64 / lpr;
    const int c4 = lane & (lpr - 1), sub = lane / lpr;
    const float4 xv = *reinterpret_cast<const float4*>(x + c4 * 4);
    float sqacc = 0.f, dzacc = 0.f;
    const long long stride = (long long)gx * 4 * rpw;
    for (long long k0 = ((long long)bx * 4 + wave) * rpw; k0 < K; k0 += 2 * stride) {
        const long long ka = k0 + sub, kb = k0 + stride + sub;
        float4 wa = make_float4(0.f, 0.f, 0.f, 0.f), wb = wa;
        if (ka < K) wa = *reinterpret_cast<const float4*>(W + ka * C + c4 * 4);
        if (kb < K) wb = *reinterpret_cast<const float4*>(W + kb * C + c4 * 4);
        float sa = wa.x * xv.x + wa.y * xv.y + wa.z * xv.z + wa.w * xv.w;
        float sb = wb.x * xv.x + wb.y * xv.y + wb.z * xv.z + wb.w * xv.w;
        for (int o = lpr >> 1; o > 0; o >>= 1) { sa += __shfl_xor(sa, o); sb += __shfl_xor(sb, o); }
        if (c4 == 0) {
            sa *= xscale; sb *= xscale;
            if (ka < K) { y[ka] = sa; sqacc += sa * sa; if (z) dzacc += sa * z[ka]; }
            if (kb < K) { y[kb] = sb; sqacc += sb * sb; if (z) dzacc += sb * z[kb]; }
        }
    }
    __shared__ float sn_part[2][4];
    sqacc = wsum(sqacc); dzacc = wsum(dzacc);
    if (lane == 0) { sn_part[0][wave] = sqacc; sn_part[1][wave] = dzacc; }
    __syncthreads();
    if (threadIdx.x == 0) {
        if (sq) unsafeAtomicAdd(sq, (double)(sn_part[0][0] + sn_part[0][1]) + (double)(sn_part[0][2] + sn_part[0][3]));
        if (dotz) unsafeAtomicAdd(dotz, (double)(sn_part[1][0] + sn_part[1][1]) + (double)(sn_part[1][2] + sn_part[1][3]));
    }
}

__global__ __launch_bounds__(NT) void sn_gemv_rows_vec_kernel(const float* __restrict__ W, long long K, int C, const float* __restrict__ x,
                                                              float xscale, float* __restrict__ y, double* sq, const float* z,
                                                              double* dotz) {
    sn_rows_vec_body(W, K, C, x, xscale, y, sq, z, dotz, blockIdx.x, gridDim.x);
}

static bool sn_vec_ok(const float* W, const float* x, int C) {
    const int lpr = C >> 2;
    return (C % 4 == 0) && lpr >= 1 && lpr <= 64 && (lpr & (lpr - 1)) == 0 && ((((uintptr_t)W) | ((uintptr_t)x)) & 15) == 0;
}

__device__ __forceinline__ void sn_rows_narrow_body(const float* __restrict__ W, long long K, int C, const float* __restrict__ x,
                                                    float xscale, float* __restrict__ y, double* sq, const float* z, double* dotz, int bx, int gx,
                                                    float* sh) {
    float sqacc = 0.f, dzacc = 0.f;
    for (long long k = bx * (long long)NT + threadIdx.x; k < K; k += (long long)gx * NT) {
        float s = 0.f;
        for (int c = 0; c < C; ++c) s += W[k * C + c] * x[c];
        s *= xscale;
        y[k] = s;
        sqacc += s * s;
        if (z) dzacc += s * z[k];
    }
    float t = block_sum1(sqacc, sh);
    if (threadIdx.x == 0 && sq) unsafeAtomicAdd(sq, (double)t);
    if (dotz) {
        float t2 = block_sum1(dzacc, sh);
        if (threadIdx.x == 0) unsafeAtomicAdd(dotz, (double)t2);
    }
}

__global__ __launch_bounds__(NT) void sn_gemv_rows_narrow_kernel(const float* __restrict__ W, long long K, int C, const float* __restrict__ x,
                                                                 float xscale, float* __restrict__ y, double* sq, const float* z,
                                                                 double* dotz) {
    __shared__ float sh[4];
    sn_rows_narrow_body(W, K, C, x, xscale, y, sq, z, dotz, blockIdx.x, gridDim.x, sh);
}

__device__ __forceinline__ void sn_cols_body(const float* __restrict__ W, long long K, int C, const float* __restrict__ x,
                                             double* __restrict__ y, int rows_per_block, int bx) {
    const long long k0 = (long long)bx * rows_per_block;
    const long long k1 = min(K, k0 + rows_per_block);
    for (int c = threadIdx.x; c < C; c += NT) {
        float s = 0.f;
        for (long long k = k0; k < k1; ++k) s += W[k * C + c] * x[k];
        unsafeAtomicAdd(y + c, (double)s);
    }
}

__global__ __launch_bounds__(NT) void sn_gemv_cols_kernel(const float* __restrict__ W, long long K, int C, const float* __restrict__ x,
                                                          double* __restrict__ y, int rows_per_block) {
    sn_cols_body(W, K, C, x, y, rows_per_block, blockIdx.x);
}

__device__ __forceinline__ void sn_cols_narrow_body(const float* __restrict__ W, long long K, int C, const float* __restrict__ x,
                                                    double* __restrict__ y, int rows_per_block, int bx, float* sh4) {
    const long long k0 = (long long)bx * rows_per_block;
    const long long k1 = min(K, k0 + rows_per_block);
    float acc[16];
#pragma unroll
    for (int c = 0; c < 16; ++c) acc[c] = 0.f;
    for (long long k = k0 + threadIdx.x; k < k1; k += NT) {
        const float xv = x[k];
#pragma unroll
        for (int c = 0; c < 16; ++c)
            if (c < C) acc[c] += W[k * C + c] * xv;
    }
#pragma unroll
    for (int c = 0; c < 16; ++c) {
        if (c < C) {
            const float t = block_sum1(acc[c], sh4);
            if (threadIdx.x == 0) unsafeAtomicAdd(y + c, (double)t);
        }
    }
}

__device__ __forceinline__ void sn_cols_vec_body(const float* __restrict__ W, long long K, int C, const float* __restrict__ x,
                                                 double* __restrict__ y, int rows_per_block, int bx, float4* sh) {
    const int lpr = C >> 2, slots = NT / lpr;
    const int c4 = threadIdx.x & (lpr - 1), sub = threadIdx.x / lpr;
    const long long k0 = (long long)bx * rows_per_block;
    const long long k1 = min(K, k0 + rows_per_block);
    float4 acc = make_float4(0.f, 0.f, 0.f, 0.f);
    long long k = k0 + sub;
    for (; k + 3 * slots < k1; k += 4 * slots) {
        float4 w[4];
        float xv[4];
#pragma unroll
        for (int j = 0; j < 4; ++j) { w[j] = *reinterpret_cast<const float4*>(W + (k + j * slots) * C + c4 * 4); xv[j] = x[k + j * slots]; }
#pragma unroll
        for (int j = 0; j < 4; ++j) { acc.x += w[j].x * xv[j]; acc.y += w[j].y * xv[j]; acc.z += w[j].z * xv[j]; acc.w += w[j].w * xv[j]; }
    }
    for (; k < k1; k += slots) {
        const float4 w = *reinterpret_cast<const float4*>(W + k * C + c4 * 4);
        const float xv = x[k];
        acc.x += w.x * xv; acc.y += w.y * xv; acc.z += w.z * xv; acc.w += w.w * xv;
    }
    sh[threadIdx.x] = acc;
    __syncthreads();
    if (threadIdx.x < lpr) {
        float4 t = sh[threadIdx.x];
        for (int r = 1; r < slots; ++r) { const float4 v = sh[r * lpr + threadIdx.x]; t.x += v.x; t.y += v.y; t.z += v.z; t.w += v.w; }
        unsafeAtomicAdd(y + c4 * 4, (double)t.x); unsafeAtomicAdd(y + c4 * 4 + 1, (double)t.y);
        unsafeAtomicAdd(y + c4 * 4 + 2, (double)t.z); unsafeAtomicAdd(y + c4 * 4 + 3, (double)t.w);
    }
}

__global__ __launch_bounds__(NT) void sn_gemv_cols_vec_kernel(const float* __restrict__ W, long long K, int C, const float* __restrict__ x,
                                                              double* __restrict__ y, int rows_per_block) {
    __shared__ float4 sh[NT];
    sn_cols_vec_body(W, K, C, x, y, rows_per_block, blockIdx.x, sh);
}

__device__ __forceinline__ void sn_finalize_body(float* ws, long long K, int C, float* u_new, float* sh) {
    const double* acc64 = sn_acc64(ws, K, C);
    const float na = sqrtf((float)acc64[0]);
    const float s = na + SN_EPS;
    float* b = ws + 8;
    float* up = ws + 8 + C;
    float acc = 0.f;
    for (int c = threadIdx.x; c < C; c += NT) { float v = (float)acc64[1 + c] / s; b[c] = v; acc += v * v; }
    const float nb2 = block_sum1(acc, sh);
    const float nb = sqrtf(nb2);
    for (int c = threadIdx.x; c < C; c += NT) { float v = b[c] / (nb + SN_EPS); up[c] = v; if (u_new) u_new[c] = v; }
    if (threadIdx.x == 0) {
        const float sigma = nb2 / (nb + SN_EPS);
        ws[0] = sigma; ws[1] = 1.f / sigma; ws[2] = na; ws[3] = nb;
        ws[4] = (nb + 2.f * SN_EPS) / ((nb + SN_EPS) * (nb + SN_EPS));
    }
}

__global__ __launch_bounds__(NT) void sn_finalize_kernel(float* ws, long long K, int C, float* u_new) {
    __shared__ float sh[4];
    sn_finalize_body(ws, K, C, u_new, sh);
}

extern "C" int savp_sn_fwd(void* stream, const float* W, int64_t K, int32_t C, const float* u, float* ws, float* u_new) {
    if (!W || !u || !ws || K < 1 || C < 1 || (((uintptr_t)ws) & 7)) return SAVP_EINVAL;
    hipStream_t st = (hipStream_t)stream;
    double* acc64 = sn_acc64(ws, K, C);
    savp_zero_async(acc64, (size_t)(C + 1) * sizeof(double), st);
    float* a = ws + 8 + 2 * C;
    unsigned nb = (unsigned)((K + 3) / 4);
    if (nb > 2048) nb = 2048;
    if (C <= 16) {
        unsigned nbn = (unsigned)((K + NT - 1) / NT);
        if (nbn > 1024) nbn = 1024;
        hipLaunchKernelGGL(sn_gemv_rows_narrow_kernel, dim3(nbn), dim3(NT), 0, st, W, (long long)K, C, u, 1.f, a, acc64,
                           (const float*)nullptr, (double*)nullptr);
    } else if (sn_vec_ok(W, u, C)) {
// ... 236 lines not shown
```

### video_prediction_amd/engine.py

```python
import math
import os
from collections import OrderedDict

import numpy as np
import torch

from . import kernels as K
from . import lib
from .variables import is_trainable


def _align4(n):
    return (n + 3) // 4 * 4


class Arena(object):

    def __init__(self, shapes, device):
        self.offsets = OrderedDict()
        off = 0
        for name, shape in shapes.items():
            n = int(np.prod(shape)) if len(shape) else 1
            self.offsets[name] = (off, n, tuple(shape))
            off += _align4(n)
        self.size = max(off, 4)
        self.device = device
        self.flat = torch.zeros(self.size, device=device, dtype=torch.float32)
        self._views = {}

    def view_of(self, flat, name):
        off, n, shape = self.offsets[name]
        return flat[off:off + n].view(shape)

    def __getitem__(self, name):
        v = self._views.get(name)
        if v is None:
            v = self._views[name] = self.view_of(self.flat, name)
        return v

    def __contains__(self, name):
        return name in self.offsets

    def names(self):
        return list(self.offsets.keys())

    def like(self):
        return torch.zeros_like(self.flat)


class ParamGroup(object):

    def __init__(self, shapes, device):
        self.arena = Arena(shapes, device)
        self.p = self.arena.flat
        self.g = self.arena.like()
        self.m = self.arena.like()
        self.v = self.arena.like()
        self.t = 0
        self._gviews = {}
        self.g64 = torch.zeros(self.arena.size, device=device, dtype=torch.float64)
        self._g64views, self._g64idx, self._g64names = {}, None, []

    def param(self, name):
        return self.arena[name]

    def grad(self, name):
        v = self._gviews.get(name)
        if v is None:
            v = self._gviews[name] = self.arena.view_of(self.g, name)
        return v

    def grad64(self, name):
        v = self._g64views.get(name)
        if v is None:
            v = self._g64views[name] = self.arena.view_of(self.g64, name)
            self._g64names.append(name)
            self._g64idx = None
        return v

    def fold64(self):
        if not self._g64names:
            return
        if self._g64idx is None:
            idx = []
            for name in self._g64names:
                off, n, _ = self.arena.offsets[name]
                idx.append(torch.arange(off, off + n, dtype=torch.int32))
            self._g64idx = torch.cat(idx).to(self.g.device)
        K.fold64(self.g64, self.g, self._g64idx)

    def zero_grad(self):
        self.g.zero_()

    def next_lr_t(self, lr, beta1, beta2):
        self.t += 1
        return lr * math.sqrt(1.0 - beta2 ** self.t) / (1.0 - beta1 ** self.t)

    def adam_apply(self, lr_t, beta1, beta2, gscale=1.0, eps=1e-8, lr_t_dev=None):
        K.adam(self.p, self.g, self.m, self.v, lr_t, beta1, beta2, eps=eps, gscale=gscale, lr_t_dev=lr_t_dev)

    def adam_step(self, lr, beta1, beta2, gscale=1.0, eps=1e-8):
        self.adam_apply(self.next_lr_t(lr, beta1, beta2), beta1, beta2, gscale=gscale, eps=eps)


class ParamStore(object):

    def __init__(self, specs, values, device):
        shapes = {'g': OrderedDict(), 'd': OrderedDict(), 'aux': OrderedDict()}
        self.group_of = {}
        for name, (shape, _) in specs.items():
            if not is_trainable(name):
                grp = 'aux'
            elif name.startswith('discriminator/'):
                grp = 'd'
            else:
                grp = 'g'
            shapes[grp][name] = shape
            self.group_of[name] = grp
        self.groups = {k: ParamGroup(v, device) for k, v in shapes.items()}
        self.specs = specs
        self.device = device
        self.load(values)

    def load(self, values):
        for name, val in values.items():
            if name not in self.group_of:
                continue
            t = torch.as_tensor(np.asarray(val, dtype=np.float32))
            self[name].copy_(t.reshape(self[name].shape))

    def __getitem__(self, name):
        return self.groups[self.group_of[name]].param(name)

    def __contains__(self, name):
        return name in self.group_of

    def grad(self, name):
        return self.groups[self.group_of[name]].grad(name)

    def grad64(self, name):
        return self.groups[self.group_of[name]].grad64(name)

    def names(self):
        return list(self.group_of.keys())

    def chunk_of(self, group, prefix):
        offs = self.groups[group].arena.offsets
        lo = hi = None
        inside = done = False
        for name, (off, n, _) in offs.items():
            if name.startswith(prefix):
                if done:
                    raise ValueError('variables under %r are not contiguous in group %r' % (prefix, group))
                if not inside:
                    lo, inside = off, True
                hi = off + _align4(n)
            elif inside:
                inside, done = False, True
        if lo is None:
            return (0, 0)
        return (lo, hi)

    def to_numpy(self):
        return OrderedDict((n, self[n].detach().cpu().numpy().copy()) for n in self.specs)

    def grads_to_numpy(self):
        for grp in self.groups.values():
            grp.fold64()
        return OrderedDict((n, self.grad(n).detach().cpu().numpy().copy()) for n in self.specs if self.group_of[n] != 'aux')


def same_pad_before(k, s, in_size):
    out = -(-in_size // s)
    total = max((out - 1) * s + k - in_size, 0)
    return total // 2


class ConvLayer(object):

    def __init__(self, store, kernel_name, bias_name, kind, ksize, stride, pad, sn_u=None, cx_pad=None, cy_pad=None):
        self.store = store
        self.kernel_name, self.bias_name, self.kind = kernel_name, bias_name, kind
        W = store[kernel_name]
        self.W = W
        self.dW = store.grad(kernel_name) if store.group_of[kernel_name] != 'aux' else None
        self.bias = store[bias_name] if bias_name else None
        self.dbias = store.grad(bias_name) if bias_name else None
        dev = W.device
        if kind == 'conv':
            self.cx, self.cy = W.shape[-2], W.shape[-1]
            self.wf = W
            self.dwf = None
            k3 = tuple(ksize)
        elif kind == 'pool':
            k, _, cin, cout = W.shape
            self.cx, self.cy = cin, cout
            self.wf = torch.empty(k + 1, k + 1, cin, cout, device=dev)
            self.dwf = torch.zeros_like(self.wf)
            k3 = (1, k + 1, k + 1)
        elif kind == 'up':
            k, _, cin, f = W.shape
            self.cx, self.cy = f, cin
            self.wf = torch.empty(k + 3, k + 3, f, cin, device=dev)
            self.dwf = torch.zeros_like(self.wf)
            k3 = (1, k + 3, k + 3)
        else:
            raise ValueError(kind)
        if len(k3) == 2:
            k3 = (1,) + tuple(k3)
        s3 = tuple(stride) if len(stride) == 3 else (1,) + tuple(stride)
        p3 = tuple(pad) if len(pad) == 3 else (0,) + tuple(pad)
        self.geom = K.ConvGeom(k3, s3, p3)
        self.taps = k3[0] * k3[1] * k3[2]
        self.cx0, self.cy0 = self.cx, self.cy
        self.padded = False
        if (cx_pad and cx_pad != self.cx) or (cy_pad and cy_pad != self.cy):
            if kind == 'up' or sn_u:
                raise NotImplementedError('channel padding for upsample / spectral-norm layers')
            self.padded = True
            self.cx, self.cy = cx_pad or self.cx, cy_pad or self.cy
            self.wfp = torch.zeros(self.taps, self.cx, self.cy, device=dev)
            self.dwfp = torch.zeros(self.taps, self.cx, self.cy, device=dev)
            self.dw_tmp = torch.empty(self.taps, self.cx0, self.cy0, device=dev)
            if self.bias is not None:
                self.bias_master, self.dbias_master = self.bias, self.dbias
                self.bias = torch.zeros(self.cy, device=dev)
                self.dbias = torch.zeros(self.cy, device=dev)
        self.wt = torch.empty(self.cy, self.taps * self.cx, device=dev)
        self.wd = torch.empty(self.cx, self.taps * self.cy, device=dev)
        self.wt16 = torch.empty(self.cy, self.taps * self.cx, device=dev, dtype=torch.bfloat16)
        self.wd16 = torch.empty(self.cx, self.taps * self.cy, device=dev, dtype=torch.bfloat16)
        self.sn_u_name = sn_u
        if sn_u:
            self.u = store[sn_u]
            kdim = W.numel() // self.cy
            self.sn_ws = torch.zeros(K.sn_ws_size(kdim, self.cy), device=dev)
            self.u_next = torch.empty_like(self.u)
            self.dwf = torch.zeros_like(W)
        self.need_wt = self.need_wd = True
        self.wfrag = None
        self.wfrag_il = None
        self.prof = None
        self.ktimer = None

    def sn_entry(self, update_u=False):
        return {'W': self.W, 'u': self.u.reshape(-1), 'ws': self.sn_ws, 'u_new': self.u_next.reshape(-1) if update_u else None}

    def sn_bwd_entry(self):
        return {'W': self.W, 'u': self.u.reshape(-1), 'ws': self.sn_ws, 'G': self.dwf, 'dW': self.dW, 'beta': 1}

    def prep(self, update_u=False, sn_done=False, defer_pack=None):
        scale = None
        if self.kind == 'pool':
            K.fold_pool(self.W, self.wf, self.W.shape[0])
        elif self.kind == 'up':
            k, _, cin, f = self.W.shape
            K.fold_bilinear(self.W, self.wf, k, cin, f)
        if self.sn_u_name:
            if not sn_done:
                K.sn_fwd(self.W, self.u.reshape(-1), self.sn_ws, self.u_next.reshape(-1) if update_u else None)
            scale = self.sn_ws[1:2]
        src = self.wf
        if self.padded:
            copy_view(self.wf.reshape(self.taps, self.cx0, self.cy0), [self.wfp[:, :self.cx0, :self.cy0]])
            if self.bias is not None:
                K.axpby(1.0, self.bias_master, 0.0, None, self.bias[:self.cy0])
            src = self.wfp
        b16 = K.PRECISION['value'] == 1
        entry = {'src': src, 'wt': self.wt if self.need_wt else None, 'wd': self.wd if self.need_wd else None, 'scale': scale,
                 'wt16': self.wt16 if (b16 and self.need_wt) else None, 'wd16': self.wd16 if (b16 and self.need_wd) else None}
        if defer_pack is not None:
            defer_pack.append(entry)
        else:
            K.pack_weights(**entry)
        if self.wfrag is not None and b16:
            K.pack_gate_weights(src, self.wfrag)
            if self.wfrag_il is not None:
                K.pack_gate_weights(src, self.wfrag_il, interleave=True)

    def enable_gate_pack(self, cell=False):
        if self.kind == 'conv' and not self.padded and not self.sn_u_name:
            n = K.gate_weights_elems(self.taps, self.cx, self.cy)
            if n:
                self.wfrag = torch.empty(n, device=self.W.device, dtype=torch.bfloat16)
                if cell and self.cy % 32 == 0:
                    self.wfrag_il = torch.empty(n, device=self.W.device, dtype=torch.bfloat16)

    def commit_u(self):
        if self.sn_u_name:
            self.u.copy_(self.u_next)

    def forward(self, x, y, beta=0, act=0, alpha=0.0, use_bias=True, stats=None, defer=False):
        b = self.bias if use_bias else None
        if self.kind == 'conv' and x.dim() == 2 and x.shape[0] <= 64 and not act and not beta and y.is_contiguous():
            if defer:
                return None
            K.dense_fwd(x, self.W.reshape(-1, self.cy), b, y, scale=self.sn_ws[1:2] if self.sn_u_name else None)
            return
        if defer:
            if self.ktimer is not None or self.prof is not None:
                return None
            if self.kind == 'up':
                return K.conv(lib.CONV_DGRAD, self.geom, y, x, self.wd, bias=b, beta=beta, act=act, alpha=alpha, w16=self.wd16, stats=stats,
                              defer=True)
            return K.conv(lib.CONV_FPROP, self.geom, x, y, self.wt, bias=b, beta=beta, act=act, alpha=alpha, w16=self.wt16, stats=stats,
                          defer=True, w_frag=self.wfrag, w_frag_il=self.wfrag_il)
        if self.ktimer is not None:
            self.ktimer.arm()
        if self.prof is not None:
            e0, e1 = torch.cuda.Event(enable_timing=True), torch.cuda.Event(enable_timing=True)
            e0.record()
        if self.kind == 'up':
            K.conv(lib.CONV_DGRAD, self.geom, y, x, self.wd, bias=b, beta=beta, act=act, alpha=alpha, w16=self.wd16, stats=stats)
        else:
            K.conv(lib.CONV_FPROP, self.geom, x, y, self.wt, bias=b, beta=beta, act=act, alpha=alpha, w16=self.wt16, stats=stats, w_frag=self.wfrag)
        if self.prof is not None:
            e1.record()
            self.prof.append((e0, e1))
        if self.ktimer is not None:
            self.ktimer.taken()

    def stats_ok(self, x, y):
        if K.PRECISION['value'] != 1:
            return False
        if self.kind == 'up':
            return K.conv_stats_ok(lib.CONV_DGRAD, self.geom, y, x, self.wd, bias=self.bias, w16=self.wd16)
        return K.conv_stats_ok(lib.CONV_FPROP, self.geom, x, y, self.wt, bias=self.bias, w16=self.wt16)

    def backward_data(self, dy, dx, beta=0, act=0, alpha=0.0, aux=None, skip=None, norm_bwd=None, defer=False):
        if self.kind == 'up':
            return K.conv(lib.CONV_FPROP, self.geom, dy, dx, self.wt, beta=beta, act=act, alpha=alpha, aux=aux, w16=self.wt16, dst_gap=skip,
                          norm_bwd=norm_bwd, defer=defer)
        return K.conv(lib.CONV_DGRAD, self.geom, dx, dy, self.wd, beta=beta, act=act, alpha=alpha, aux=aux, w16=self.wd16, dst_gap=skip,
                      norm_bwd=norm_bwd, defer=defer)

    def norm_bwd_ok(self, dy, dx, norm_bwd, skip=None):
        if K.PRECISION['value'] != 1:
            return False
        nb = dict(norm_bwd, ws=None)
        if self.kind == 'up':
            return K.conv_stats_ok(lib.CONV_FPROP, self.geom, dy, dx, self.wt, w16=self.wt16, dst_gap=skip, norm_bwd=nb)
        return K.conv_stats_ok(lib.CONV_DGRAD, self.geom, dx, dy, self.wd, w16=self.wd16, dst_gap=skip, norm_bwd=nb)

    def backward_weights(self, x, dy, feeds_instance_norm=False):
        target = self.dwfp if self.padded else (self.dwf if self.dwf is not None else self.dW)
        if dy.dtype == torch.bfloat16 and self.dbias is not None and not feeds_instance_norm:
            raise NotImplementedError('bias gradient from a bf16 output gradient: only for a convolution in front of an instance norm '
                                      '(feeds_instance_norm=True), whose bias gradient is identically zero')
        db = None if (feeds_instance_norm and dy.dtype == torch.bfloat16) else self.dbias
        if self.kind == 'up':
            K.conv(lib.CONV_WGRAD, self.geom, dy, x, target)
            if db is not None:
                K.colsum(dy, db)
        else:
            K.conv(lib.CONV_WGRAD, self.geom, x, dy, target, bias=db)

    def finish_weight_grad(self, sn_done=False):
        if self.padded:
            copy_view(self.dwfp[:, :self.cx0, :self.cy0], [self.dw_tmp])
            tgt = self.dwf if self.dwf is not None else self.dW
            K.axpby(1.0, self.dw_tmp.reshape(-1), 1.0, tgt.reshape(-1), tgt.reshape(-1))
            self.dwfp.zero_()
            if self.bias is not None:
                K.axpby(1.0, self.dbias[:self.cy0], 1.0, self.dbias_master, self.dbias_master)
                self.dbias.zero_()
        if self.dwf is None:
            return
        if self.sn_u_name:
            if not sn_done:
                K.sn_bwd(self.W, self.u.reshape(-1), self.sn_ws, self.dwf, self.dW, beta=1)
        elif self.kind == 'pool':
            K.fold_pool(self.dwf, self.dW, self.W.shape[0], adjoint=True)
        elif self.kind == 'up':
            k, _, cin, f = self.W.shape
            K.fold_bilinear(self.dwf, self.dW, k, cin, f, adjoint=True)
        self.dwf.zero_()


class _TensorStore(object):

    def __init__(self, tensors, grads):
        self.t, self.g = tensors, grads
        self.group_of = {k: 'g' for k in tensors}

    def __getitem__(self, name):
        return self.t[name]

    def grad(self, name):
        return self.g[name]


def prep_layers(convs, **kw):
    if os.environ.get('SAVP_PACK_BATCH', '1') != '1':
        for c in convs:
            c.prep(**kw)
        return
    packs = []
    for c in convs:
        c.prep(defer_pack=packs, **kw)
    if packs:
        K.pack_weights_batch(packs)


class ConcatConv(object):

    def __init__(self, store, parts, ksize, stride, pad):
        self.parts = []
        off = 0
        W0 = store[parts[0][0]]
        self.lead = tuple(W0.shape[:-1])
        dev = W0.device
        for kname, bname in parts:
            W = store[kname]
            if tuple(W.shape[:-1]) != self.lead:
                raise ValueError('ConcatConv parts must share kernel size and input channels')
            cy = W.shape[-1]
            self.parts.append(dict(W=W, dW=store.grad(kname), b=store[bname], db=store.grad(bname), off=off, cy=cy))
            off += cy
        self.cy = off
        self.Wcat = torch.empty(self.lead + (off,), device=dev)
        self.dWcat = torch.zeros(self.lead + (off,), device=dev)
        self.bcat = torch.zeros(off, device=dev)
        self.dbcat = torch.zeros(off, device=dev)
        shim = _TensorStore({'k': self.Wcat, 'b': self.bcat}, {'k': self.dWcat, 'b': self.dbcat})
        self.inner = ConvLayer(shim, 'k', 'b', 'conv', ksize, stride, pad)
        self.R = int(np.prod(self.lead))

    @property
    def prof(self):
        return self.inner.prof

    def prep(self, update_u=False, defer_pack=None):
        R = self.R
        for P in self.parts:
            copy_view(P['W'].reshape(R, P['cy']), [self.Wcat.reshape(R, self.cy)[:, P['off']:P['off'] + P['cy']]])
            copy_view(P['b'].reshape(1, P['cy']), [self.bcat.reshape(1, self.cy)[:, P['off']:P['off'] + P['cy']]])
        self.inner.prep(defer_pack=defer_pack)

    def forward(self, x, y, **kw):
        return self.inner.forward(x, y, **kw)

    def stats_ok(self, x, y):
        return self.inner.stats_ok(x, y)

    def backward_data(self, dy, dx, **kw):
        return self.inner.backward_data(dy, dx, **kw)

    def norm_bwd_ok(self, dy, dx, norm_bwd, skip=None):
        return self.inner.norm_bwd_ok(dy, dx, norm_bwd, skip)

    def backward_weights(self, x, dy, feeds_instance_norm=False):
        self.inner.backward_weights(x, dy, feeds_instance_norm=feeds_instance_norm)

    def finish_weight_grad(self):
        self.inner.finish_weight_grad()
        R = self.R
        for P in self.parts:
            add_views([self.dWcat.reshape(R, self.cy)[:, P['off']:P['off'] + P['cy']]], P['dW'].reshape(R, P['cy']))
            add_views([self.dbcat.reshape(1, self.cy)[:, P['off']:P['off'] + P['cy']]], P['db'].reshape(1, P['cy']))
        self.dWcat.zero_()
        self.dbcat.zero_()

    def commit_u(self):
        pass


class Tape(object):

    def __init__(self):
        self.ops = []

    def add(self, fn):
        self.ops.append(fn)

    def backward(self):
        for fn in reversed(self.ops):
            fn()
        self.ops = []


_CONST = {}


def const_i32(n, value, device):
    key = (n, value, str(device))
    t = _CONST.get(key)
    if t is None:
        t = _CONST[key] = torch.full((n,), value, dtype=torch.int32, device=device)
    return t


def copy_view(src, dsts):
    K.select(const_i32(src.shape[0], 1, src.device), src, None, dsts)


def add_views(srcs, dst):
    K.select_bwd(const_i32(dst.shape[0], 0, dst.device), srcs, dst)
```

### video_prediction_amd/kernels.py

```python
import ctypes

import torch

from . import debug as _debug
from . import lib
from .lib import (c_f32, c_i32, c_i64, c_vp, ptr)


def _nd(t):
    if t.stride(-1) != 1 and t.shape[-1] != 1:
        raise ValueError('channel stride must be 1')
    if t.dim() == 4:
        N, H, W, C = t.shape
        sn, sh, sw, _ = t.stride()
        return N, 1, H, W, C, sn, 0, sh, sw
    if t.dim() == 5:
        N, D, H, W, C = t.shape
        sn, sd, sh, sw, _ = t.stride()
        return N, D, H, W, C, sn, sd, sh, sw
    if t.dim() == 2:
        N, C = t.shape
        return N, 1, 1, 1, C, t.stride(0), 0, 0, 0
    raise ValueError('expected 2-D, 4-D or 5-D tensor')

# ... 835 lines not shown

def gather_clips(src, dst, t_start, adjoint=False):
    lib.require_device(src, dst)
    L, B = src.shape[:2]
    clip = dst.shape[1]
    E = src[0, 0].numel()
    assert dst.is_contiguous() and dst.shape[0] == B and src[0, 0].is_contiguous() and src.stride(1) == E
    lib.check(_L().savp_gather_clips(lib.stream(), _p(src), _p(dst), _p(t_start), B, clip, E, src.stride(0), int(adjoint)),
              'savp_gather_clips')


def sigmoid_bwd(dy, y, out):
    assert out.is_contiguous()
    lib.check(_L().savp_sigmoid_bwd(lib.stream(), view(dy), view(y), _p(out), dy.shape[0], _hw(dy), dy.shape[-1]), 'savp_sigmoid_bwd')


def axpby(a, x, b, y, out):
    assert x.is_contiguous() and out.is_contiguous() and (y is None or y.is_contiguous())
    lib.check(_L().savp_axpby(lib.stream(), x.numel(), float(a), _p(x), float(b), _p(y), _p(out)), 'savp_axpby')


def fill_view(out, value=0.0):
    lib.check(_L().savp_fill_view(lib.stream(), view(out), out.shape[0], _hw(out), out.shape[-1], float(value)), 'savp_fill_view')


def fold64(src64, dst32, idx=None):
    lib.require_device(dst32)
    lib.require_stats(src64)
    if idx is not None:
        _require_i32(idx)
    n = idx.numel() if idx is not None else src64.numel()
    lib.check(_L().savp_fold_f64(lib.stream(), _p(idx), n, _p(src64), _p(dst32)), 'savp_fold_f64')


def state_pred_fwd(actions, states_in, gt, W, b, sa, gen):
    T, N, ns = states_in.shape
    na = actions.shape[-1] if actions is not None else 0
    for t_ in (actions, states_in, W, b, sa, gen):
        if t_ is not None:
            lib.require_device(t_)
            assert t_.is_contiguous() and t_.dtype == torch.float32
    _require_i32(gt)
    assert gt.is_contiguous() and tuple(gt.shape) == (T, N) and tuple(W.shape) == (na + ns, ns) and tuple(sa.shape) == (T, N, na + ns)
    assert tuple(gen.shape) == (T, N, ns) and (actions is None or tuple(actions.shape[:2]) == (T, N))
    lib.check(_L().savp_state_pred_fwd(lib.stream(), T, N, na, ns, _p(actions), _p(states_in), _p(gt), _p(W), _p(b), _p(sa), _p(gen)),
              'savp_state_pred_fwd')


def state_pred_bwd(gt, W, sa, dgen, dW64, db64):
    T, N, ns = dgen.shape
    na = sa.shape[-1] - ns
    lib.require_stats(dW64)
    lib.require_stats(db64)
    _require_i32(gt)
    assert dgen.is_contiguous() and sa.is_contiguous() and dW64.numel() == (na + ns) * ns and db64.numel() == ns
    lib.check(_L().savp_state_pred_bwd(lib.stream(), T, N, na, ns, _p(gt), _p(W), _p(sa), _p(dgen), _p(dW64), _p(db64)),
              'savp_state_pred_bwd')


def adam(p, g, m, v, lr_t, beta1, beta2, eps=1e-8, gscale=1.0, lr_t_dev=None):
    lib.check(_L().savp_adam(lib.stream(), p.numel(), _p(p), _p(g), _p(m), _p(v), float(lr_t), float(beta1), float(beta2),
                             float(eps), float(gscale), _p(lr_t_dev) if lr_t_dev is not None else None), 'savp_adam')


def cdna_kernels_fwd(raw, kern, kh, kw, K):
    lib.check(_L().savp_cdna_kernels_fwd(lib.stream(), _p(raw), _p(kern), raw.shape[0], kh, kw, K), 'savp_cdna_kernels_fwd')


def cdna_kernels_bwd(raw, dkern, draw, kh, kw, K):
    lib.require_stats(dkern)
    lib.check(_L().savp_cdna_kernels_bwd(lib.stream(), _p(raw), _p(dkern), _p(draw), raw.shape[0], kh, kw, K),
              'savp_cdna_kernels_bwd')


def _cdna_args(img, kern, kh, kw, K):
    a = lib.SavpCdnaArgs()
    a.N, a.H, a.W, a.C = img.shape
    a.K, a.kh, a.kw = K, kh, kw
    a.img = view(img)
    a.kern = _p(kern)
    return a


def cdna_apply_fwd(img, kern, out, kh, kw, K):
    a = _cdna_args(img, kern, kh, kw, K)
    a.out = view(out)
    lib.check(_L().savp_cdna_apply_fwd(lib.stream(), ctypes.byref(a)), 'savp_cdna_apply_fwd')


def cdna_apply_bwd(img, kern, dout, dimg, dkern, kh, kw, K, dimg_beta=0):
    a = _cdna_args(img, kern, kh, kw, K)
    a.dout = view(dout)
    if dimg is not None:
        a.dimg = view(dimg)
    a.dimg_beta = int(dimg_beta)
    lib.require_stats(dkern)
    a.dkern = _p(dkern)
    lib.check(_L().savp_cdna_apply_bwd(lib.stream(), ctypes.byref(a)), 'savp_cdna_apply_bwd')


def _set_sources(a, imgs, dimgs=None, dimg_beta=0):
    if not 1 <= len(imgs) <= lib.MAX_SOURCES:
        raise ValueError('1 .. %d source images, got %d' % (lib.MAX_SOURCES, len(imgs)))
    if any(tuple(im.shape) != tuple(imgs[0].shape) for im in imgs):
        raise ValueError('source images differ in shape: %s' % [tuple(im.shape) for im in imgs])
    a.N, a.H, a.W, a.C = imgs[0].shape
    a.nsrc = len(imgs)
    for j, im in enumerate(imgs):
        a.img[j] = view(im)
    if dimgs is not None:
        if len(dimgs) != len(imgs):
            raise ValueError('one gradient destination (or None) per source image')
        betas = dimg_beta if isinstance(dimg_beta, (list, tuple)) else [dimg_beta] * len(imgs)
        for j, d in enumerate(dimgs):
            if d is not None:
                a.dimg[j] = view(d)
            a.dimg_beta[j] = int(betas[j])
    return a


def cdna_apply_multi_fwd(imgs, kern, out, kh, kw, K):
    a = _set_sources(lib.SavpCdnaMultiArgs(), imgs)
    a.K, a.kh, a.kw = K, kh, kw
    a.kern = _p(kern)
    a.out = view(out)
    lib.check(_L().savp_cdna_apply_multi_fwd(lib.stream(), ctypes.byref(a)), 'savp_cdna_apply_multi_fwd')


def cdna_apply_multi_bwd(imgs, kern, dout, dimgs, dkern, kh, kw, K, dimg_beta=0):
    a = _set_sources(lib.SavpCdnaMultiArgs(), imgs, dimgs, dimg_beta)
    a.K, a.kh, a.kw = K, kh, kw
    a.kern = _p(kern)
    a.dout = view(dout)
    lib.require_stats(dkern)
    a.dkern = _p(dkern)
    lib.check(_L().savp_cdna_apply_multi_bwd(lib.stream(), ctypes.byref(a)), 'savp_cdna_apply_multi_bwd')


def _comp_args(logits, timgs, C, M):
    a = lib.SavpCompositeArgs()
    a.N, a.HW, a.M, a.C = logits.shape[0], _hw(logits), M, C
    assert logits.is_contiguous()
    a.logits = _p(logits)
    a.logits_stride = logits.shape[-1]
    a.timgs = view(timgs)
    return a


def composite_fwd(logits, timgs, gen, masks=None, M=None, next_inputs=None):
    M = M or logits.shape[-1]
    a = _comp_args(logits, timgs, gen.shape[-1], M)
    a.gen = view(gen)
    a.masks = _p(masks)
    if next_inputs is not None:
        gt_mask, gt_img, dsts = next_inputs
        lib.require_device(gt_img)
        _require_i32(gt_mask)
        if len(dsts) > 2:
            raise ValueError('composite_fwd: at most two next-input views')
        a.nnext = len(dsts)
        for i, d in enumerate(dsts):
            a.next[i] = view(d)
        a.gt_mask = gt_mask.data_ptr()
        a.gt_img = view(gt_img)
    lib.check(_L().savp_composite_fwd(lib.stream(), ctypes.byref(a)), 'savp_composite_fwd')


def composite_bwd(logits, timgs, dgen, dlogits, drow, timgs_offset, M=None):
    M = M or logits.shape[-1]
    a = _comp_args(logits, timgs, dgen.shape[-1], M)
    a.dgen = view(dgen)
    assert dlogits.is_contiguous() and dlogits.shape == logits.shape
    a.dlogits = _p(dlogits)
    a.drow = view(drow)
    a.timgs_offset, a.row_channels = int(timgs_offset), drow.shape[-1]
    lib.check(_L().savp_composite_bwd(lib.stream(), ctypes.byref(a)), 'savp_composite_bwd')


def lstm_z_fwd(zs, W, b, hout, gates, cs, forget_bias=1.0, init=None):
    T, B, nz = zs.shape
    c0, h0 = init if init is not None else (None, None)
    lib.require_device(zs, W, b, hout, gates, cs, c0, h0)
    lib.check(_L().savp_lstm_z_fwd_init(lib.stream(), _p(zs), _p(W), _p(b), _p(hout), _p(gates), _p(cs), T, B, nz, float(forget_bias),
                                        _p(c0), _p(h0)), 'savp_lstm_z_fwd')


def lstm_z_bwd(zs, W, hout, gates, cs, dh_out, dzs, dW, db, forget_bias=1.0, init=None, dinit=None):
    T, B, nz = zs.shape
    c0, h0 = init if init is not None else (None, None)
    dc0, dh0 = dinit if dinit is not None else (None, None)
    lib.require_device(c0, h0)
    acc = _Acc64(dW, db, dc0, dh0)
    lib.check(_L().savp_lstm_z_bwd_init(lib.stream(), _p(zs), _p(W), _p(hout), _p(gates), _p(cs), _p(dh_out), _p(dzs), acc.addr(0), acc.addr(1),
                                        T, B, nz, float(forget_bias), _p(c0), _p(h0), acc.addr(2), acc.addr(3)), 'savp_lstm_z_bwd')
    acc.finish()


def gru_seq_fwd(A, A2, Wg, bg, Wc, bc, hout, ru, cand, n_in, h0=None):
    T, B, Kd = A.shape
    U = Kd - n_in
    lib.require_device(A, A2, Wg, bg, Wc, bc, hout, ru, cand, h0)
    if h0 is not None:
        lib.check(_L().savp_gru_seq_fwd_init(lib.stream(), _p(A), _p(A2), _p(Wg), _p(bg), _p(Wc), _p(bc), _p(hout), _p(ru), _p(cand), T, B, n_in,
                                             U, _p(h0)), 'savp_gru_seq_fwd_init')
        return
    lib.check(_L().savp_gru_seq_fwd(lib.stream(), _p(A), _p(A2), _p(Wg), _p(bg), _p(Wc), _p(bc), _p(hout), _p(ru), _p(cand), T, B, n_in, U),
              'savp_gru_seq_fwd')


def gru_seq_bwd(A, Wg, Wc, ru, cand, dh_out, dGg, dGc, dA, n_in, dh0=None):
    T, B, Kd = A.shape
    U = Kd - n_in
    lib.require_device(A, Wg, Wc, ru, cand, dh_out, dGg, dGc, dA)
    if dh0 is not None:
        lib.require_stats(dh0)
        lib.check(_L().savp_gru_seq_bwd_init(lib.stream(), _p(A), _p(Wg), _p(Wc), _p(ru), _p(cand), _p(dh_out), _p(dGg), _p(dGc), _p(dA), T, B,
                                             n_in, U, _p(dh0)), 'savp_gru_seq_bwd_init')
        return
    lib.check(_L().savp_gru_seq_bwd(lib.stream(), _p(A), _p(Wg), _p(Wc), _p(ru), _p(cand), _p(dh_out), _p(dGg), _p(dGc), _p(dA), T, B, n_in, U),
              'savp_gru_seq_bwd')


def lstm_seq_fwd(A, W, b, hout, gates, cs, n_in, forget_bias=1.0):
    T, B, K = A.shape
    U = K - n_in
    lib.require_device(A, W, b, hout, gates, cs)
    lib.check(_L().savp_lstm_seq_fwd(lib.stream(), _p(A), _p(W), _p(b), _p(hout), _p(gates), _p(cs), T, B, n_in, U,
                                     float(forget_bias)), 'savp_lstm_seq_fwd')


def lstm_seq_bwd(A, W, gates, cs, dh_out, dG, dA, n_in, forget_bias=1.0):
    T, B, K = A.shape
    U = K - n_in
    lib.require_device(A, W, gates, cs, dh_out, dG, dA)
    lib.check(_L().savp_lstm_seq_bwd(lib.stream(), _p(A), _p(W), _p(gates), _p(cs), _p(dh_out), _p(dG), _p(dA), T, B, n_in, U,
                                     float(forget_bias)), 'savp_lstm_seq_bwd')


def kl_gauss(mu1, ls1_raw, mu2, ls2_raw, kl_out=None, klw=0.0, klw_dev=None, grads=None):
    rows = mu1.numel() // mu1.shape[-1]
    g = grads or (None, None, None, None)
    lib.require_device(mu1, ls1_raw, mu2, ls2_raw)
    acc = _Acc64(kl_out)
    lib.check(_L().savp_kl_gauss(lib.stream(), mu1.numel(), rows, _p(mu1), _p(ls1_raw), _p(mu2), _p(ls2_raw),
                                 acc.addr(0), float(klw),
                                 _p(klw_dev) if klw_dev is not None else None, *[(_p(t) if t is not None else None) for t in g]),
              'savp_kl_gauss')
    acc.finish()


def reparam_fwd(mu, ls_raw, eps, ls, z, kl_out=None):
    rows = mu.numel() // mu.shape[-1]
    acc = _Acc64(kl_out)
    lib.check(_L().savp_reparam_fwd(lib.stream(), mu.numel(), rows, _p(mu), _p(ls_raw), _p(eps), _p(ls), _p(z), acc.addr(0)),
              'savp_reparam_fwd')
    acc.finish()


def reparam_bwd(mu, ls_raw, eps, dz, klw, dmu, dls_raw, klw_dev=None):
    rows = mu.numel() // mu.shape[-1]
    lib.check(_L().savp_reparam_bwd(lib.stream(), mu.numel(), rows, _p(mu), _p(ls_raw), _p(eps), _p(dz), float(klw), _p(dmu),
                                    _p(dls_raw), _p(klw_dev) if klw_dev is not None else None), 'savp_reparam_bwd')


def lp_loss(pred, target, weight, loss_out=None, dpred=None, p2=False):
    rows = pred.shape[0]
    row_len = pred[0].numel()
    assert pred[0].is_contiguous() and target[0].is_contiguous() and target.shape == pred.shape
    if dpred is not None:
        assert dpred.stride() == pred.stride()
    acc = _Acc64(loss_out)
    lib.check(_L().savp_lp_loss(lib.stream(), rows, row_len, pred.stride(0), target.stride(0), int(p2), _p(pred), _p(target),
                                float(weight), acc.addr(0), _p(dpred)), 'savp_lp_loss')
    acc.finish()


def tv_loss(flows, n_channels, s1, s2, weight, loss_out=None, dflows=None):
    lib.require_device_any(flows)
    assert flows.dtype == torch.float32 and flows.dim() == 4 and flows.stride(3) == 1 and flows.stride(1) == flows.shape[2] * flows.stride(2)
    if dflows is not None:
        assert dflows.stride() == flows.stride() and dflows.dtype == torch.float32
    lib.require_stats(loss_out)
    n, H, W, _ = flows.shape
    lib.check(_L().savp_tv_loss(lib.stream(), _p(flows), n, H, W, int(n_channels), flows.stride(0), flows.stride(2), float(s1), float(s2),
                                float(weight), _p(loss_out), _p(dflows)), 'savp_tv_loss')


def lsgan_loss(logits, label, weight, loss_out=None, dlogits=None, beta=0):
    acc = _Acc64(loss_out)
    lib.check(_L().savp_lsgan_loss(lib.stream(), logits.numel(), _p(logits), float(label), float(weight), acc.addr(0), _p(dlogits),
                                   int(beta)), 'savp_lsgan_loss')
    acc.finish()


def cosine_distance(f0, f1, weight, loss_out=None, df0=None, beta=0, eps=1e-10):
    assert f0.is_contiguous() and f1.is_contiguous()
    C = f0.shape[-1]
    acc = _Acc64(loss_out)
    lib.check(_L().savp_cosine_distance(lib.stream(), f0.numel() // C, C, _p(f0), _p(f1), float(weight), float(eps), acc.addr(0),
                                        _p(df0), int(beta)), 'savp_cosine_distance')
    acc.finish()


def pack_weights(src, wt=None, wd=None, scale=None, wt16=None, wd16=None):
    Cx, Cy = src.shape[-2], src.shape[-1]
    T = src.numel() // (Cx * Cy)
    lib.check(_L().savp_pack_weights(lib.stream(), _p(src), T, Cx, Cy, _p(scale), _p(wt), _p(wd), _p(wt16), _p(wd16)),
              'savp_pack_weights')


def pack_weights_batch(entries):
    for lo in range(0, len(entries), 32):
        part = entries[lo:lo + 32]
        arr = (lib.SavpPackItem * len(part))()
        for i, e in enumerate(part):
            src = e['src']
            lib.require_device(src)
            it = arr[i]
            it.src, it.scale = _p(src), _p(e.get('scale'))
            it.wt, it.wd, it.wt_bf16, it.wd_bf16 = _p(e.get('wt')), _p(e.get('wd')), _p(e.get('wt16')), _p(e.get('wd16'))
            it.Cx, it.Cy = src.shape[-2], src.shape[-1]
            it.T = src.numel() // (it.Cx * it.Cy)
        lib.check(_L().savp_pack_weights_batch(lib.stream(), len(part), arr), 'savp_pack_weights_batch')


def gate_weights_elems(taps, Cx, Cy):
    return int(lib.get().savp_gate_weights_bytes(int(taps), int(Cx), int(Cy))) // 2


def pack_gate_weights(src, out, interleave=False):
    lib.require_device(src)
    Cx, Cy = src.shape[-2], src.shape[-1]
    taps = src.numel() // (Cx * Cy)
    if out.dtype != torch.bfloat16 or out.numel() != gate_weights_elems(taps, Cx, Cy):
        raise ValueError('gate weight pack: expected %d bf16 elements' % gate_weights_elems(taps, Cx, Cy))
    lib.check(_L().savp_pack_gate_weights(lib.stream(), _p(src), taps, Cx, Cy, _p(out), int(bool(interleave))), 'savp_pack_gate_weights')


def fold_pool(inp, out, k, adjoint=False):
    C = (out.numel() if adjoint else inp.numel()) // (k * k)
    lib.check(_L().savp_fold_pool(lib.stream(), _p(inp), _p(out), k, C, int(adjoint)), 'savp_fold_pool')


def fold_bilinear(inp, out, k, Cin, F, adjoint=False):
    lib.check(_L().savp_fold_bilinear(lib.stream(), _p(inp), _p(out), k, Cin, F, int(adjoint)), 'savp_fold_bilinear')


def sn_ws_size(K, C):
    return 8 + 2 * C + 2 * K + 2 * (C + 2)


def sn_fwd(W, u, ws, u_new=None):
    C = W.shape[-1]
    K = W.numel() // C
    lib.check(_L().savp_sn_fwd(lib.stream(), _p(W), K, C, _p(u), _p(ws), _p(u_new)), 'savp_sn_fwd')


def _sn_items(entries, bwd):
    arr = (lib.SavpSnItem * len(entries))()
    for i, e in enumerate(entries):
        W = e['W']
        C = W.shape[-1]
        arr[i].W, arr[i].K, arr[i].C = W.data_ptr(), W.numel() // C, C
        arr[i].u, arr[i].ws = e['u'].data_ptr(), e['ws'].data_ptr()
        arr[i].u_new = e['u_new'].data_ptr() if e.get('u_new') is not None else None
        if bwd:
            arr[i].G, arr[i].dW, arr[i].beta = e['G'].data_ptr(), e['dW'].data_ptr(), int(e.get('beta', 0))
    return arr


def sn_fwd_batch(entries):
    for lo in range(0, len(entries), 16):
        part = entries[lo:lo + 16]
        arr = _sn_items(part, False)
        lib.check(_L().savp_sn_fwd_batch(lib.stream(), len(part), arr), 'savp_sn_fwd_batch')


def sn_bwd_batch(entries):
    for lo in range(0, len(entries), 16):
        part = entries[lo:lo + 16]
        arr = _sn_items(part, True)
        lib.check(_L().savp_sn_bwd_batch(lib.stream(), len(part), arr), 'savp_sn_bwd_batch')


def sn_bwd(W, u, ws, G, dW, beta=0):
    C = W.shape[-1]
    K = W.numel() // C
    lib.check(_L().savp_sn_bwd(lib.stream(), _p(W), K, C, _p(u), _p(ws), _p(G), _p(dW), int(beta)), 'savp_sn_bwd')


def dense_fwd(x, W, bias, out, scale=None):
    M, Kd = x.shape
    C = W.shape[-1]
    assert out.is_contiguous() and x.stride(1) == 1 and W.is_contiguous()
    ws = scratch(x.device, 64 * M * C)
    lib.check(_L().savp_dense_fwd(lib.stream(), _p(x), x.stride(0), M, Kd, C, _p(W), _p(bias), _p(scale), _p(out), _p(ws), ws.numel()),
              'savp_dense_fwd')


def _warp_args(img, flows, K_):
    a = lib.SavpWarpArgs()
    a.N, a.H, a.W, a.C = img.shape
    a.K = K_
    a.img = view(img)
    assert flows.is_contiguous() and flows.shape[-1] == 2 * K_
    a.flows = _p(flows)
    return a


def image_warp_fwd(img, flows, out, K_):
    a = _warp_args(img, flows, K_)
    a.out = view(out)
    lib.check(_L().savp_image_warp_fwd(lib.stream(), ctypes.byref(a)), 'savp_image_warp_fwd')


def image_warp_bwd(img, flows, dout, dflows, dimg, K_):
    a = _warp_args(img, flows, K_)
    a.dout = view(dout)
    assert dflows.is_contiguous() and (dimg is None or dimg.is_contiguous())
    a.dflows, a.dimg = _p(dflows), _p(dimg)
    lib.check(_L().savp_image_warp_bwd(lib.stream(), ctypes.byref(a)), 'savp_image_warp_bwd')


def _warp_multi_args(imgs, flows, K_, dimgs=None, dimg_beta=0):
    a = _set_sources(lib.SavpWarpMultiArgs(), imgs, dimgs, dimg_beta)
    a.K = K_
    assert flows.is_contiguous() and flows.shape[-1] == 2 * K_ * len(imgs)
    a.flows = _p(flows)
    return a


def image_warp_multi_fwd(imgs, flows, out, K_):
    a = _warp_multi_args(imgs, flows, K_)
    a.out = view(out)
    lib.check(_L().savp_image_warp_multi_fwd(lib.stream(), ctypes.byref(a)), 'savp_image_warp_multi_fwd')


def image_warp_multi_bwd(imgs, flows, dout, dflows, dimgs, K_, dimg_beta=0):
    a = _warp_multi_args(imgs, flows, K_, dimgs, dimg_beta)
    a.dout = view(dout)
    assert dflows.is_contiguous()
    a.dflows = _p(dflows)
    lib.check(_L().savp_image_warp_multi_bwd(lib.stream(), ctypes.byref(a)), 'savp_image_warp_multi_bwd')


def _dna_args(img, raw, kern, kh, kw, K_):
    a = lib.SavpDnaArgs()
    a.N, a.H, a.W, a.C = img.shape
    a.K, a.kh, a.kw = K_, kh, kw
    a.img = view(img)
    assert raw.is_contiguous() and kern.is_contiguous()
    a.raw, a.kern = _p(raw), _p(kern)
    return a


def dna_apply_fwd(img, raw, kern, out, kh, kw, K_):
    a = _dna_args(img, raw, kern, kh, kw, K_)
    a.out = view(out)
    lib.check(_L().savp_dna_apply_fwd(lib.stream(), ctypes.byref(a)), 'savp_dna_apply_fwd')


def dna_apply_bwd(img, raw, kern, dout, draw, dimg, kh, kw, K_, dimg_beta=0):
    a = _dna_args(img, raw, kern, kh, kw, K_)
    a.dout = view(dout)
    a.draw = _p(draw)
    if dimg is not None:
        a.dimg = view(dimg)
    a.dimg_beta = int(dimg_beta)
    lib.check(_L().savp_dna_apply_bwd(lib.stream(), ctypes.byref(a)), 'savp_dna_apply_bwd')


def _dna_multi_args(imgs, raw, kern, kh, kw, K_, dimgs=None, dimg_beta=0):
    a = _set_sources(lib.SavpDnaMultiArgs(), imgs, dimgs, dimg_beta)
    a.K, a.kh, a.kw = K_, kh, kw
    assert raw.is_contiguous() and kern.is_contiguous()
    a.raw, a.kern = _p(raw), _p(kern)
    return a


def dna_apply_multi_fwd(imgs, raw, kern, out, kh, kw, K_):
    a = _dna_multi_args(imgs, raw, kern, kh, kw, K_)
    a.out = view(out)
    lib.check(_L().savp_dna_apply_multi_fwd(lib.stream(), ctypes.byref(a)), 'savp_dna_apply_multi_fwd')


def dna_apply_multi_bwd(imgs, raw, kern, dout, draw, dimgs, kh, kw, K_, dimg_beta=0):
    a = _dna_multi_args(imgs, raw, kern, kh, kw, K_, dimgs, dimg_beta)
    a.dout = view(dout)
    a.draw = _p(draw)
    lib.check(_L().savp_dna_apply_multi_bwd(lib.stream(), ctypes.byref(a)), 'savp_dna_apply_multi_bwd')


def _gru_args(pre, h, gamma, beta, mean, rstd, F, eps):
    a = lib.SavpGruArgs()
    a.N, a.HW, a.F, a.eps = pre.shape[0], _hw(pre), F, float(eps)
    assert pre.is_contiguous()
    a.pre = _p(pre)
    a.h = view(h)
    a.gamma, a.beta, a.mean, a.rstd = _p(gamma), _p(beta), _p(mean), _p(rstd)
    return a


def convgru_gates_fwd(pre, h, gamma, beta, mean, rstd, u, rh, eps=1e-6):
    a = _gru_args(pre, h, gamma, beta, mean, rstd, pre.shape[-1] // 2, eps)
    a.u, a.rh = _p(u), view(rh)
    lib.check(_L().savp_convgru_gates_fwd(lib.stream(), ctypes.byref(a)), 'savp_convgru_gates_fwd')


def convgru_out_fwd(pre, h, gamma, beta, mean, rstd, u, outs, eps=1e-6):
    a = _gru_args(pre, h, gamma, beta, mean, rstd, pre.shape[-1], eps)
    a.u = _p(u)
    a.nout = len(outs)
    _set_views(a.out, outs)
    lib.check(_L().savp_convgru_out_fwd(lib.stream(), ctypes.byref(a)), 'savp_convgru_out_fwd')


def convgru_out_bwd(pre, h, gamma, beta, mean, rstd, u, dys, dpre, du, dh, dgamma, dbeta, eps=1e-6):
    a = _gru_args(pre, h, gamma, beta, mean, rstd, pre.shape[-1], eps)
    a.u = _p(u)
    a.ndy = len(dys)
    _set_views(a.dy, dys)
    a.dpre, a.du, a.dh = _p(dpre), _p(du), view(dh)
    acc = _Acc64(dgamma, dbeta)
    a.dgamma, a.dbeta = acc.addr(0), acc.addr(1)
    lib.check(_L().savp_convgru_out_bwd(lib.stream(), ctypes.byref(a)), 'savp_convgru_out_bwd')
    acc.finish()


def convgru_gates_bwd(pre, h, gamma, beta, mean, rstd, du, drh, dpre, dh, dgamma, dbeta, eps=1e-6):
    a = _gru_args(pre, h, gamma, beta, mean, rstd, pre.shape[-1] // 2, eps)
    a.du, a.drh, a.dpre, a.dh = _p(du), view(drh), _p(dpre), view(dh)
    acc = _Acc64(dgamma, dbeta)
    a.dgamma, a.dbeta = acc.addr(0), acc.addr(1)
    lib.check(_L().savp_convgru_gates_bwd(lib.stream(), ctypes.byref(a)), 'savp_convgru_gates_bwd')
    acc.finish()


GAN_TYPES = {'LSGAN': 0, 'GAN': 1, 'SNGAN': 2}


def gan_loss(logits, label, weight, gan_loss_type='LSGAN', loss_out=None, dlogits=None, beta=0):
    acc = _Acc64(loss_out)
    lib.check(_L().savp_gan_loss(lib.stream(), logits.numel(), GAN_TYPES[gan_loss_type], _p(logits), float(label), float(weight),
                                 acc.addr(0), _p(dlogits), int(beta)), 'savp_gan_loss')
    acc.finish()


def _tb(x):
    if x.dim() < 3 or not x[0, 0].is_contiguous():
        raise ValueError('expected a time-major [T, B, ...] tensor with contiguous frames')
    return x.stride(0), x.stride(1), x[0, 0].numel()


def _require_i32(*tensors):
    for t in tensors:
        if t is not None and (not t.is_cuda or t.dtype != torch.int32):
            raise RuntimeError('expected an int32 device tensor, got %s on %s' % (t.dtype, t.device))


def frame_mse_psnr(a, b, mse=None, psnr=None):
    lib.require_device(a, b, mse, psnr)
    a_st, a_sb, inner = _tb(a)
    b_st, b_sb, _ = _tb(b)
    lib.check(_L().savp_frame_mse_psnr(lib.stream(), _p(a), a_st, a_sb, _p(b), b_st, b_sb, a.shape[0], a.shape[1], inner, _p(mse),
                                       _p(psnr)), 'savp_frame_mse_psnr')


def frame_ssim(a, b, out):
    lib.require_device(a, b, out)
    a_st, a_sb, _ = _tb(a)
    b_st, b_sb, _ = _tb(b)
    T, B, H, W, C = a.shape
    lib.check(_L().savp_frame_ssim(lib.stream(), _p(a), a_st, a_sb, _p(b), b_st, b_sb, T, B, H, W, C, _p(out)), 'savp_frame_ssim')


def eval_accumulate(metric, vmin, vsum, vmax, cond_min, cond_max):
    lib.require_device(metric, vmin, vsum, vmax)
    _require_i32(cond_min, cond_max)
    T, B = metric.shape
    lib.check(_L().savp_eval_accumulate(lib.stream(), _p(metric), _p(vmin), _p(vsum), _p(vmax), _p(cond_min), _p(cond_max), T, B),
              'savp_eval_accumulate')


def select_batch(cond, x, out, mode=0):
    lib.require_device(x, out)
    _require_i32(cond)
    x_st, x_sb, inner = _tb(x)
    o_st, o_sb, _ = _tb(out)
    lib.check(_L().savp_select_batch(lib.stream(), _p(cond), _p(x), x_st, x_sb, _p(out), o_st, o_sb, x.shape[0], x.shape[1], inner,
                                     int(mode)), 'savp_select_batch')


EVAL_FOLD_KEYS = ('psnr', 'mse', 'ssim')


def eval_fold_ws(F, S, B, C, device):
    n = int(_L().savp_eval_fold_ws_floats(int(F), int(S), int(B), int(C)))
    if n <= 0:
        raise ValueError('eval_fold_ws: bad shape %r' % ((F, S, B, C),))
    return torch.empty(n, device=device, dtype=torch.float32)


def eval_fold_samples(target, pred, n_valid, states, ws):
    lib.require_device(target, pred, ws)
    _require_i32(n_valid)
    F, B, H, W, C = target.shape
    T1, SB = pred.shape[:2]
    if tuple(pred.shape[2:]) != (H, W, C) or SB % B or T1 < F:
        raise ValueError('eval_fold_samples: pred %r does not fit target %r' % (tuple(pred.shape), tuple(target.shape)))
    S = SB // B
    t_st, t_sb, _ = _tb(target)
    p_st, p_sb, _ = _tb(pred)
    arr = (lib.SavpEvalFoldState * lib.EVAL_NMETRICS)()
    for k, name in enumerate(EVAL_FOLD_KEYS):
        a = states[name]
        for key, shape in (('min', (F, B)), ('sum', (F, B)), ('max', (F, B)), ('gmin', (T1, B, H, W, C)), ('gsum', (T1, B, H, W, C)),
                           ('gmax', (T1, B, H, W, C))):
            v = a[key]
            lib.require_device(v)
            if tuple(v.shape) != shape or not v.is_contiguous() or v.dtype != torch.float32:
                raise ValueError('eval_fold_samples: state %s/%s must be contiguous fp32 %r' % (name, key, shape))
        arr[k] = lib.SavpEvalFoldState(_p(a['min']), _p(a['sum']), _p(a['max']), _p(a['gmin']), _p(a['gsum']), _p(a['gmax']))
    lib.check(_L().savp_eval_fold_samples(lib.stream(), _p(target), t_st, t_sb, _p(pred), p_st, p_sb, F, T1, S, B, H, W, C, _p(n_valid),
# ... 53 lines not shown
```

### video_prediction_amd/lib.py

```python
import ctypes
import os

import torch

from . import debug as _debug

_HERE = os.path.dirname(os.path.abspath(__file__))
LIB_PATH = os.environ.get('SAVP_LIB') or os.path.join(_HERE, 'libsavp_hip.so')

c_i32, c_i64, c_f32, c_vp = ctypes.c_int32, ctypes.c_int64, ctypes.c_float, ctypes.c_void_p

CONV_FPROP, CONV_DGRAD, CONV_WGRAD = 0, 1, 2
ACT_NONE, ACT_LRELU, ACT_SIGMOID, ACT_DLRELU_FROM_OUT = 0, 1, 2, 3


class SavpConvArgs(ctypes.Structure):
    _fields_ = [
        ('mode', c_i32),
        ('N', c_i32), ('D', c_i32), ('H', c_i32), ('W', c_i32), ('Cx', c_i32),
        ('Do', c_i32), ('Ho', c_i32), ('Wo', c_i32), ('Cy', c_i32),
        ('kd', c_i32), ('kh', c_i32), ('kw', c_i32),
        ('sd', c_i32), ('sh', c_i32), ('sw', c_i32),
        ('pd', c_i32), ('ph', c_i32), ('pw', c_i32),
        ('beta', c_i32), ('act', c_i32), ('alpha', c_f32), ('splitk', c_i32), ('tile', c_i32), ('precision', c_i32),
        ('x', c_vp), ('x_sn', c_i64), ('x_sd', c_i64), ('x_sh', c_i64), ('x_sw', c_i64),
        ('y', c_vp), ('y_sn', c_i64), ('y_sd', c_i64), ('y_sh', c_i64), ('y_sw', c_i64),
        ('w', c_vp), ('bias', c_vp), ('aux', c_vp), ('w_bf16', c_vp),
        ('src_bf16', c_i32), ('out_bf16', c_i32), ('stats', c_vp),
        ('ws', c_vp), ('ws_bytes', c_i64),
        ('dst_gap_at', c_i32), ('dst_gap', c_i32),
        ('nb_x', c_vp), ('nb_x_sn', c_i64), ('nb_x_sp', c_i64), ('nb_mean', c_vp), ('nb_rstd', c_vp), ('nb_gamma', c_vp), ('nb_beta', c_vp),
        ('nb_ws', c_vp), ('nb_c0', c_i32), ('nb_nc', c_i32), ('nb_act', c_i32), ('nb_alpha', c_f32),
        ('w_frag', c_vp), ('w_frag_il', c_vp),
    ]


_lib = None


def get():
    global _lib
    if _lib is None:
        if not os.path.exists(LIB_PATH):
            raise RuntimeError(
                'libsavp_hip.so not found at %s -- build it first (python -c "import __graft_entry__ as g; g.build()"). '
                'video_prediction_amd has no non-HIP fallback.' % LIB_PATH)
        lib = ctypes.CDLL(LIB_PATH)
        lib.savp_version.restype = ctypes.c_char_p
        _declare(lib)
        _lib = lib
        _forward_env_options(lib)
    if _debug.POISON['lds']:
        return _LdsPoisonProxy(_lib)
    return _lib


def get_raw():
    lib = get()
    return lib._lib if isinstance(lib, _LdsPoisonProxy) else lib


class _LdsPoisonProxy(object):

    def __init__(self, lib):
        self._lib = lib

    def __getattr__(self, name):
        fn = getattr(self._lib, name)
        at = getattr(fn, 'argtypes', None)
        if not name.startswith('savp_') or name.startswith(('savp_debug_', 'savp_prof_')) or not at or at[0] is not c_vp or \
                name in ('savp_allreduce_bucket',):
            return fn
        poison = self._lib.savp_debug_poison_lds

        def call(st, *args):
            poison(st, _debug.NAN_WORD, None)
            _debug.COUNTS['lds'] += 1
            return fn(st, *args)
        return call


OPTION_NAMES = ('conv_ring', 's2dgrad', 'thin', 'wgp_cfg', 'wgp_split', 'inorm_min_hw', 'colsum_2stage', 'dense_legacy', 'cdna_legacy',
                'lstm_fused', 'ring_dma', 'lstm_q', 'ring_wwarm', 'wgp_dma', 'ring_early', 'gate_kernel', 'gate_alt', 'gate_cell', 'gate_wwarm', 'splitk_reduced')


def set_option(name, value):
    check(get().savp_set_option(name.encode(), int(value)), 'savp_set_option(%s)' % name)


def get_option(name):
    v = c_i32()
    check(get().savp_get_option(name.encode(), ctypes.byref(v)), 'savp_get_option(%s)' % name)
    return v.value


def _forward_env_options(lib):
    for name in OPTION_NAMES:
        v = os.environ.get('SAVP_' + name.upper())
        if v is not None:
            check(lib.savp_set_option(name.encode(), int(v)), 'savp_set_option(%s)' % name)


EXPORTS = {}


def _sig(lib, name, argtypes, restype=c_i32):
    try:
        fn = getattr(lib, name)
    except AttributeError:
        if os.environ.get('SAVP_LIB'):
            return None
        raise
    fn.argtypes = argtypes
    fn.restype = restype
    EXPORTS[name] = fn
    return fn


def _declare(lib):
    P = ctypes.POINTER
    _sig(lib, 'savp_conv', [c_vp, P(SavpConvArgs)])
    _sig(lib, 'savp_conv_workspace_bytes', [P(SavpConvArgs)], restype=c_i64)
    _sig(lib, 'savp_conv_special', [P(SavpConvArgs)])
    _sig(lib, 'savp_gate_weights_bytes', [c_i32, c_i32, c_i32], restype=c_i64)
    _sig(lib, 'savp_conv_stats_ok', [P(SavpConvArgs)])
    _sig(lib, 'savp_set_option', [ctypes.c_char_p, c_i32])
    _sig(lib, 'savp_get_option', [ctypes.c_char_p, P(c_i32)])
    _sig(lib, 'savp_allreduce_bucket', [c_vp, c_vp, c_vp, c_i64])
    _sig(lib, 'savp_tiled_z_weff', [c_vp, c_vp, c_i32, c_i32, c_i32, c_i32, c_i32, c_i32, c_i32, c_i32, c_vp])
    _sig(lib, 'savp_tiled_z_grad', [c_vp, c_vp, c_i32, c_i64, c_i32, c_i32, c_i32, c_vp, c_i32, c_vp, c_i32, c_vp, c_i64])
    _sig(lib, 'savp_tiled_z_workspace_bytes', [c_i64, c_i32], restype=c_i64)
    _sig(lib, 'savp_eval_fold_ws_floats', [c_i32, c_i32, c_i32, c_i32], restype=c_i64)
    for name, argtypes in _EXTRA_SIGS.items():
        _sig(lib, name, argtypes)


_EXTRA_SIGS = {}


def register(name, argtypes):
    _EXTRA_SIGS[name] = argtypes
    if _lib is not None:
        _sig(_lib, name, argtypes)


def source_id():
    import hashlib
    h = hashlib.sha256()
    root = os.path.dirname(_HERE)
    files = []
    for d, pat in ((os.path.join(_HERE, 'csrc'), ('.hip', '.h')), (os.path.join(root, 'include'), ('.h',)), (_HERE, ('.json',))):
        for f in sorted(os.listdir(d)):
            if f.endswith(pat) and (d != _HERE or f.startswith('tuning_gfx950_')):
                files.append(os.path.join(d, f))
    for f in files:
        h.update(os.path.basename(f).encode())
        with open(f, 'rb') as fh:
            h.update(fh.read())
    return h.hexdigest()[:16]


def stream():
    return ctypes.c_void_p(torch.cuda.current_stream().cuda_stream)


def check(rc, what):
    if rc != 0:
        raise RuntimeError('%s failed with code %d' % (what, rc))


def ptr(t):
    return ctypes.c_void_p(t.data_ptr()) if t is not None else ctypes.c_void_p(0)


def require_device(*tensors):
    for t in tensors:
        if t is None:
            continue
        if not t.is_cuda:
            raise RuntimeError('video_prediction_amd kernels need device tensors (got %s); there is no CPU path' % t.device)
        if t.dtype != torch.float32:
            raise RuntimeError('expected float32, got %s' % t.dtype)


def require_stats(*tensors):
    for t in tensors:
        if t is None:
            continue
        if not t.is_cuda:
            raise RuntimeError('video_prediction_amd kernels need device tensors (got %s); there is no CPU path' % t.device)
        if t.dtype != torch.float64 or (t.data_ptr() & 7):
            raise RuntimeError('statistics workspaces are float64 (kernels.stats_ws), got %s' % t.dtype)


def require_device_any(*tensors):
    for t in tensors:
        if t is None:
            continue
        if not t.is_cuda:
            raise RuntimeError('video_prediction_amd kernels need device tensors (got %s); there is no CPU path' % t.device)
        if t.dtype not in (torch.float32, torch.bfloat16):
            raise RuntimeError('expected float32 or bfloat16, got %s' % t.dtype)


class SavpView(ctypes.Structure):
    _fields_ = [('p', c_vp), ('sn', c_i64), ('sp', c_i64)]


class SavpInormArgs(ctypes.Structure):
    _fields_ = [
        ('N', c_i32), ('HW', c_i32), ('C', c_i32), ('act', c_i32), ('alpha', c_f32), ('eps', c_f32),
        ('x', SavpView), ('gamma', c_vp), ('beta', c_vp),
        ('nout', c_i32), ('out', SavpView * 4), ('mean', c_vp), ('rstd', c_vp),
        ('ndy', c_i32), ('dy', SavpView * 4), ('dx', SavpView), ('dx_beta', c_i32),
        ('dgamma', c_vp), ('dbeta', c_vp), ('ws', c_vp), ('ws_clean', c_i32),
        ('out_c0', c_i32 * 4), ('out_nc', c_i32 * 4), ('dy_c0', c_i32 * 4), ('dy_nc', c_i32 * 4), ('out_bf16', c_i32),
        ('stats_ready', c_i32), ('stats_shift', c_vp), ('dx_bf16', c_i32),
    ]


class SavpGnormArgs(ctypes.Structure):
    _fields_ = [('norm', SavpInormArgs), ('G', c_i32), ('ws_group', c_vp), ('dsum', c_vp)]


class SavpLnLstmArgs(ctypes.Structure):
    _fields_ = [
        ('N', c_i32), ('HW', c_i32), ('F', c_i32), ('forget_bias', c_f32), ('gn', c_vp), ('c_prev', SavpView), ('c_pre', c_vp),
        ('cn', c_vp), ('nh', c_i32), ('h', SavpView * 4), ('h_bf16', c_i32), ('ndh', c_i32), ('dh', SavpView * 4),
        ('dc_new', c_vp), ('dcn', c_vp), ('dgn', c_vp), ('dc_pre', c_vp), ('dc_prev', c_vp),
    ]


class SavpLstmArgs(ctypes.Structure):
    _fields_ = [
        ('N', c_i32), ('HW', c_i32), ('F', c_i32), ('eps', c_f32), ('forget_bias', c_f32),
        ('gates', c_vp), ('c_prev', SavpView),
        ('gamma1', c_vp), ('beta1', c_vp), ('gamma2', c_vp), ('beta2', c_vp),
        ('c_new', c_vp), ('nh', c_i32), ('h', SavpView * 4),
        ('mean1', c_vp), ('rstd1', c_vp), ('mean2', c_vp), ('rstd2', c_vp),
        ('ndh', c_i32), ('dh', SavpView * 4), ('dc_new', c_vp), ('dgates', c_vp), ('dc_prev', c_vp),
        ('dgamma1', c_vp), ('dbeta1', c_vp), ('dgamma2', c_vp), ('dbeta2', c_vp),
        ('ws', c_vp), ('ws_floats', ctypes.c_int64), ('ws_stats', c_vp), ('ws_stats_clean', c_i32),
        ('gates_bf16', c_i32), ('stats1_ready', c_i32), ('h_bf16', c_i32), ('dgates_bf16', c_i32), ('dgates_raw', c_vp), ('no_norm', c_i32),
    ]


class SavpConvLstmCellArgs(ctypes.Structure):
    _fields_ = [('conv', SavpConvArgs), ('gates', SavpLstmArgs)]


class SavpConvNormArgs(ctypes.Structure):
    _fields_ = [('conv', SavpConvArgs), ('norm', SavpInormArgs)]


register('savp_convlstm_cell_fwd', [c_vp, ctypes.POINTER(SavpConvLstmCellArgs)])
register('savp_convlstm_cell_bwd', [c_vp, ctypes.POINTER(SavpConvLstmCellArgs)])
register('savp_conv_in_act_fwd', [c_vp, ctypes.POINTER(SavpConvNormArgs)])
register('savp_conv_in_act_bwd', [c_vp, ctypes.POINTER(SavpConvNormArgs)])
register('savp_instnorm_act_fwd', [c_vp, ctypes.POINTER(SavpInormArgs)])
register('savp_instnorm_act_bwd', [c_vp, ctypes.POINTER(SavpInormArgs)])
register('savp_groupnorm_act_fwd', [c_vp, ctypes.POINTER(SavpGnormArgs)])
register('savp_groupnorm_act_bwd', [c_vp, ctypes.POINTER(SavpGnormArgs)])
register('savp_lnlstm_fwd', [c_vp, ctypes.POINTER(SavpLnLstmArgs), c_i32])
register('savp_lnlstm_bwd', [c_vp, ctypes.POINTER(SavpLnLstmArgs), c_i32])
register('savp_convlstm_gates_fwd', [c_vp, ctypes.POINTER(SavpLstmArgs)])
register('savp_convlstm_gates_bwd', [c_vp, ctypes.POINTER(SavpLstmArgs)])


class SavpCdnaArgs(ctypes.Structure):
    _fields_ = [
        ('N', c_i32), ('H', c_i32), ('W', c_i32), ('C', c_i32), ('K', c_i32), ('kh', c_i32), ('kw', c_i32),
        ('img', SavpView), ('kern', c_vp), ('out', SavpView), ('dout', SavpView),
        ('dimg', SavpView), ('dimg_beta', c_i32), ('dkern', c_vp),
    ]


class SavpCompositeArgs(ctypes.Structure):
    _fields_ = [
        ('N', c_i32), ('HW', c_i32), ('M', c_i32), ('C', c_i32),
        ('logits', c_vp), ('logits_stride', c_i32), ('timgs', SavpView), ('gen', SavpView), ('masks', c_vp),
        ('dgen', SavpView), ('dlogits', c_vp), ('drow', SavpView), ('timgs_offset', c_i32), ('row_channels', c_i32),
        ('nnext', c_i32), ('next', SavpView * 2), ('gt_mask', c_vp), ('gt_img', SavpView),
    ]


_PV = ctypes.POINTER(SavpView)
register('savp_tile_channels', [c_vp, c_vp, c_i64, c_i32, c_i32, c_f32, SavpView, c_i32])
register('savp_tile_channels_bf16', [c_vp, c_vp, c_i64, c_i32, c_i32, c_f32, SavpView])
register('savp_colsum', [c_vp, SavpView, c_i64, c_i32, c_i32, c_f32, c_vp, c_i32, c_vp, c_i64])
register('savp_select', [c_vp, c_i32, c_i32, c_i32, c_vp, SavpView, SavpView, c_i32, _PV])
register('savp_select_bwd', [c_vp, c_i32, c_i32, c_i32, c_vp, c_i32, _PV, SavpView])
register('savp_gather_clips', [c_vp, c_vp, c_vp, c_vp, c_i32, c_i32, c_i64, c_i64, c_i32])
register('savp_sigmoid_bwd', [c_vp, SavpView, SavpView, c_vp, c_i64, c_i32, c_i32])
register('savp_axpby', [c_vp, c_i64, c_f32, c_vp, c_f32, c_vp, c_vp])
register('savp_fill_view', [c_vp, SavpView, c_i64, c_i32, c_i32, c_f32])
register('savp_u8_frames_to_f32', [c_vp, c_vp, c_vp, c_i32, c_i32, c_i64])
register('savp_frame_mse_psnr', [c_vp, c_vp, c_i64, c_i64, c_vp, c_i64, c_i64, c_i32, c_i32, c_i32, c_vp, c_vp])
register('savp_frame_ssim', [c_vp, c_vp, c_i64, c_i64, c_vp, c_i64, c_i64, c_i32, c_i32, c_i32, c_i32, c_i32, c_vp])
register('savp_eval_accumulate', [c_vp, c_vp, c_vp, c_vp, c_vp, c_vp, c_vp, c_i32, c_i32])
register('savp_select_batch', [c_vp, c_vp, c_vp, c_i64, c_i64, c_vp, c_i64, c_i64, c_i32, c_i32, c_i32, c_i32])


EVAL_PSNR, EVAL_MSE, EVAL_SSIM, EVAL_NMETRICS = 0, 1, 2, 3


class SavpEvalFoldState(ctypes.Structure):
    _fields_ = [('vmin', c_vp), ('vsum', c_vp), ('vmax', c_vp), ('gmin', c_vp), ('gsum', c_vp), ('gmax', c_vp)]


register('savp_eval_fold_samples', [c_vp, c_vp, c_i64, c_i64, c_vp, c_i64, c_i64, c_i32, c_i32, c_i32, c_i32, c_i32, c_i32, c_i32, c_vp,
                                    ctypes.POINTER(SavpEvalFoldState), c_vp, c_i64])
register('savp_adam', [c_vp, c_i64, c_vp, c_vp, c_vp, c_vp, c_f32, c_f32, c_f32, c_f32, c_f32, c_vp])
register('savp_cdna_kernels_fwd', [c_vp, c_vp, c_vp, c_i32, c_i32, c_i32, c_i32])
register('savp_cdna_kernels_bwd', [c_vp, c_vp, c_vp, c_vp, c_i32, c_i32, c_i32, c_i32])
register('savp_cdna_apply_fwd', [c_vp, ctypes.POINTER(SavpCdnaArgs)])
register('savp_cdna_apply_bwd', [c_vp, ctypes.POINTER(SavpCdnaArgs)])
register('savp_composite_fwd', [c_vp, ctypes.POINTER(SavpCompositeArgs)])
register('savp_composite_bwd', [c_vp, ctypes.POINTER(SavpCompositeArgs)])
register('savp_lstm_z_fwd', [c_vp, c_vp, c_vp, c_vp, c_vp, c_vp, c_vp, c_i32, c_i32, c_i32, c_f32])
register('savp_lstm_seq_fwd', [c_vp, c_vp, c_vp, c_vp, c_vp, c_vp, c_vp, c_i32, c_i32, c_i32, c_i32, c_f32])
register('savp_lstm_seq_bwd', [c_vp, c_vp, c_vp, c_vp, c_vp, c_vp, c_vp, c_vp, c_i32, c_i32, c_i32, c_i32, c_f32])
register('savp_prof_event_create', [ctypes.POINTER(c_vp)])
register('savp_prof_event_destroy', [c_vp])
register('savp_prof_arm', [c_vp, c_vp])
register('savp_prof_armed', [])
register('savp_prof_elapsed_us', [c_vp, c_vp, ctypes.POINTER(c_f32)])
register('savp_kl_gauss', [c_vp, c_i64, c_i32, c_vp, c_vp, c_vp, c_vp, c_vp, c_f32, c_vp, c_vp, c_vp, c_vp, c_vp])
register('savp_lstm_z_bwd', [c_vp, c_vp, c_vp, c_vp, c_vp, c_vp, c_vp, c_vp, c_vp, c_vp, c_i32, c_i32, c_i32, c_f32])
register('savp_gru_seq_fwd', [c_vp] * 10 + [c_i32] * 4)
register('savp_gru_seq_bwd', [c_vp] * 10 + [c_i32] * 4)
register('savp_gru_seq_fwd_init', [c_vp] * 10 + [c_i32] * 4 + [c_vp])
register('savp_gru_seq_bwd_init', [c_vp] * 10 + [c_i32] * 4 + [c_vp])
register('savp_lstm_z_fwd_init', [c_vp, c_vp, c_vp, c_vp, c_vp, c_vp, c_vp, c_i32, c_i32, c_i32, c_f32, c_vp, c_vp])
register('savp_lstm_z_bwd_init', [c_vp, c_vp, c_vp, c_vp, c_vp, c_vp, c_vp, c_vp, c_vp, c_vp, c_i32, c_i32, c_i32, c_f32, c_vp, c_vp, c_vp, c_vp])
register('savp_reparam_fwd', [c_vp, c_i64, c_i32, c_vp, c_vp, c_vp, c_vp, c_vp, c_vp])
register('savp_reparam_bwd', [c_vp, c_i64, c_i32, c_vp, c_vp, c_vp, c_vp, c_f32, c_vp, c_vp, c_vp])
register('savp_lp_loss', [c_vp, c_i64, c_i64, c_i64, c_i64, c_i32, c_vp, c_vp, c_f32, c_vp, c_vp])
register('savp_lsgan_loss', [c_vp, c_i32, c_vp, c_f32, c_f32, c_vp, c_vp, c_i32])
register('savp_cosine_distance', [c_vp, c_i64, c_i32, c_vp, c_vp, c_f32, c_f32, c_vp, c_vp, c_i32])
register('savp_pack_weights', [c_vp, c_vp, c_i64, c_i32, c_i32, c_vp, c_vp, c_vp, c_vp, c_vp])
register('savp_fold_pool', [c_vp, c_vp, c_vp, c_i32, c_i64, c_i32])
register('savp_fold_bilinear', [c_vp, c_vp, c_vp, c_i32, c_i32, c_i32, c_i32])
class SavpPackItem(ctypes.Structure):
    _fields_ = [('src', c_vp), ('scale', c_vp), ('wt', c_vp), ('wd', c_vp), ('wt_bf16', c_vp), ('wd_bf16', c_vp), ('T', c_i64),
                ('Cx', c_i32), ('Cy', c_i32)]


register('savp_pack_weights_batch', [c_vp, c_i32, ctypes.POINTER(SavpPackItem)])


class SavpSnItem(ctypes.Structure):
    _fields_ = [('W', c_vp), ('K', c_i64), ('C', c_i32), ('u', c_vp), ('ws', c_vp), ('u_new', c_vp), ('G', c_vp), ('dW', c_vp),
                ('beta', c_i32)]


register('savp_sn_fwd_batch', [c_vp, c_i32, ctypes.POINTER(SavpSnItem)])
register('savp_sn_bwd_batch', [c_vp, c_i32, ctypes.POINTER(SavpSnItem)])
register('savp_sn_fwd', [c_vp, c_vp, c_i64, c_i32, c_vp, c_vp, c_vp])
register('savp_sn_bwd', [c_vp, c_vp, c_i64, c_i32, c_vp, c_vp, c_vp, c_vp, c_i32])
register('savp_dense_fwd', [c_vp, c_vp, c_i64, c_i32, c_i64, c_i32, c_vp, c_vp, c_vp, c_vp, c_vp, c_i64])


class SavpWarpArgs(ctypes.Structure):
    _fields_ = [('N', c_i32), ('H', c_i32), ('W', c_i32), ('C', c_i32), ('K', c_i32), ('img', SavpView), ('flows', c_vp),
                ('out', SavpView), ('dout', SavpView), ('dflows', c_vp), ('dimg', c_vp)]


class SavpDnaArgs(ctypes.Structure):
    _fields_ = [('N', c_i32), ('H', c_i32), ('W', c_i32), ('C', c_i32), ('K', c_i32), ('kh', c_i32), ('kw', c_i32),
                ('img', SavpView), ('raw', c_vp), ('kern', c_vp), ('out', SavpView), ('dout', SavpView), ('draw', c_vp),
                ('dimg', SavpView), ('dimg_beta', c_i32)]


MAX_SOURCES = 4


class SavpCdnaMultiArgs(ctypes.Structure):
    _fields_ = [
        ('N', c_i32), ('H', c_i32), ('W', c_i32), ('C', c_i32), ('K', c_i32), ('kh', c_i32), ('kw', c_i32), ('nsrc', c_i32),
        ('img', SavpView * MAX_SOURCES), ('kern', c_vp), ('out', SavpView), ('dout', SavpView),
        ('dimg', SavpView * MAX_SOURCES), ('dimg_beta', c_i32 * MAX_SOURCES), ('dkern', c_vp),
    ]


class SavpWarpMultiArgs(ctypes.Structure):
    _fields_ = [('N', c_i32), ('H', c_i32), ('W', c_i32), ('C', c_i32), ('K', c_i32), ('nsrc', c_i32),
                ('img', SavpView * MAX_SOURCES), ('flows', c_vp), ('out', SavpView), ('dout', SavpView), ('dflows', c_vp),
                ('dimg', SavpView * MAX_SOURCES), ('dimg_beta', c_i32 * MAX_SOURCES)]


class SavpDnaMultiArgs(ctypes.Structure):
    _fields_ = [('N', c_i32), ('H', c_i32), ('W', c_i32), ('C', c_i32), ('K', c_i32), ('kh', c_i32), ('kw', c_i32), ('nsrc', c_i32),
                ('img', SavpView * MAX_SOURCES), ('raw', c_vp), ('kern', c_vp), ('out', SavpView), ('dout', SavpView), ('draw', c_vp),
                ('dimg', SavpView * MAX_SOURCES), ('dimg_beta', c_i32 * MAX_SOURCES)]


register('savp_cdna_apply_multi_fwd', [c_vp, ctypes.POINTER(SavpCdnaMultiArgs)])
register('savp_cdna_apply_multi_bwd', [c_vp, ctypes.POINTER(SavpCdnaMultiArgs)])
register('savp_image_warp_multi_fwd', [c_vp, ctypes.POINTER(SavpWarpMultiArgs)])
register('savp_image_warp_multi_bwd', [c_vp, ctypes.POINTER(SavpWarpMultiArgs)])
register('savp_dna_apply_multi_fwd', [c_vp, ctypes.POINTER(SavpDnaMultiArgs)])
register('savp_dna_apply_multi_bwd', [c_vp, ctypes.POINTER(SavpDnaMultiArgs)])
register('savp_image_warp_fwd', [c_vp, ctypes.POINTER(SavpWarpArgs)])
register('savp_image_warp_bwd', [c_vp, ctypes.POINTER(SavpWarpArgs)])
register('savp_dna_apply_fwd', [c_vp, ctypes.POINTER(SavpDnaArgs)])
register('savp_dna_apply_bwd', [c_vp, ctypes.POINTER(SavpDnaArgs)])


class SavpGruArgs(ctypes.Structure):
    _fields_ = [('N', c_i32), ('HW', c_i32), ('F', c_i32), ('eps', c_f32), ('pre', c_vp), ('h', SavpView),
                ('gamma', c_vp), ('beta', c_vp), ('mean', c_vp), ('rstd', c_vp), ('u', c_vp), ('rh', SavpView),
                ('nout', c_i32), ('out', SavpView * 4), ('ndy', c_i32), ('dy', SavpView * 4), ('dpre', c_vp), ('du', c_vp),
                ('dh', SavpView), ('drh', SavpView), ('dgamma', c_vp), ('dbeta', c_vp)]


for _n in ('savp_convgru_gates_fwd', 'savp_convgru_out_fwd', 'savp_convgru_out_bwd', 'savp_convgru_gates_bwd'):
    register(_n, [c_vp, ctypes.POINTER(SavpGruArgs)])
register('savp_gan_loss', [c_vp, c_i32, c_i32, c_vp, c_f32, c_f32, c_vp, c_vp, c_i32])
register('savp_fold_f64', [c_vp, c_vp, c_i64, c_vp, c_vp])
register('savp_tv_loss', [c_vp, c_vp, c_i32, c_i32, c_i32, c_i32, c_i64, c_i64, c_f32, c_f32, c_f32, c_vp, c_vp])
register('savp_state_pred_fwd', [c_vp, c_i32, c_i32, c_i32, c_i32] + [c_vp] * 7)
register('savp_state_pred_bwd', [c_vp, c_i32, c_i32, c_i32, c_i32] + [c_vp] * 6)
register('savp_pack_gate_weights', [c_vp, c_vp, c_i32, c_i32, c_i32, c_vp, c_i32])
register('savp_debug_poison_lds', [c_vp, ctypes.c_uint32, c_vp])
register('savp_debug_fill_u32', [c_vp, c_vp, c_i64, ctypes.c_uint32])
register('savp_debug_probe_lds', [c_vp, ctypes.c_uint32, c_vp])
```

### video_prediction_amd/models/networks.py

```python
import os

import torch

from .. import kernels as K
from .. import lib
from ..engine import ConvLayer, copy_view, prep_layers
from ..variables import NORM_SCOPES, VIDEO_D_LAYERS, video_discriminator_shapes, image_discriminator_shapes

EPS_IN = 1e-6


class PosteriorEncoder(object):

    def __init__(self, store, hp, image_shape, B, train=True, prefix='generator/encoder/', prior=False, n_actions=0):
        H, W, C = image_shape
        self.hp, self.store = hp, store
        self.T1 = T1 = hp.sequence_length - 1
        self.prior = prior
        self.Tc = Tc = (hp.context_frames - 1) if prior else T1
        self.na = na = int(n_actions)
        if prior and na and Tc != T1:
            raise ValueError('learn_prior with actions: %d action steps against %d context frame pairs (savp_model.py:56-59)' % (T1, Tc))
        self.B, self.M, self.R = B, Tc * B, T1 * B
        M, R = self.M, self.R
        dev = store.device
        self.dev = dev
        if hp.norm_layer not in NORM_SCOPES:
            raise NotImplementedError("HIP encoder covers norm_layer in ('instance', 'layer'), not %r" % hp.norm_layer)
        self.ln = hp.norm_layer == 'layer'
        ns_ = NORM_SCOPES[hp.norm_layer]
        self.recurrent = bool(prior or hp.use_e_rnn)
        if self.recurrent and hp.rnn not in ('lstm', 'gru'):
            raise NotImplementedError(hp.rnn)
        self.gru = bool(self.recurrent and hp.rnn == 'gru')
        self.pairs = torch.zeros(max(M, 1), H, W, 2 * C + na, device=dev)
        self.C = C
        self.layers = []
        cin, h, w = 2 * C + na, H, W
        x = self.pairs
        for i in range(hp.n_layers):
            cout = hp.nef * min(2 ** i, 4)
            s = prefix + 'layer_%d/' % (i + 1)
            L = {'conv': ConvLayer(store, s + 'conv2d/kernel', s + 'conv2d/bias', 'conv', (4, 4), (2, 2), (1, 1)),
                 'x': x, 'normed': i > 0}
            h, w = (h + 2 - 4) // 2 + 1, (w + 2 - 4) // 2 + 1
            L['y'] = torch.empty(max(M, 1), h, w, cout, device=dev)
            L['dy'] = torch.empty(max(M, 1), h, w, cout, device=dev) if train else None
            if i > 0:
                L['pre'] = torch.empty(max(M, 1), h, w, cout, device=dev)
                L['dpre'] = torch.empty(max(M, 1), h, w, cout, device=dev) if train else None
                L['gamma'], L['beta'] = store[s + ns_ + 'gamma'], store[s + ns_ + 'beta']
                L['dgamma'], L['dbeta'] = store.grad64(s + ns_ + 'gamma'), store.grad64(s + ns_ + 'beta')
                ms = 1 if self.ln else cout
                L['mean'], L['rstd'] = torch.empty(max(M, 1), ms, device=dev), torch.empty(max(M, 1), ms, device=dev)
            self.layers.append(L)
            x = L['y']
            cin = cout
        self.hw = h * w
        self.feat = torch.zeros(R, cin, device=dev)
        self.dfeat = torch.zeros(R, cin, device=dev) if train else None
        self.pooled = self.feat[:M]
        self.dpooled = self.dfeat[:M] if train else None
        hin = cin
        if self.recurrent:
            U = self.U = hp.nef * 4
            s = prefix + 'layer_%d/' % (hp.n_layers + 1)
            self.fc = ConvLayer(store, s + 'dense/kernel', s + 'dense/bias', 'conv', (1, 1), (1, 1), (0, 0))
            self.A = torch.zeros(T1, B, 2 * U, device=dev)
            self.hout = torch.empty(T1, B, U, device=dev)
            if train:
                self.dh = torch.empty(T1, B, U, device=dev)
                self.dA = torch.empty(T1, B, 2 * U, device=dev)
            if self.gru:
                s = prefix + 'gru/rnn/gru_cell/'
                self.cell_g = ConvLayer(store, s + 'gates/kernel', s + 'gates/bias', 'conv', (1, 1), (1, 1), (0, 0))
                self.cell_c = ConvLayer(store, s + 'candidate/kernel', s + 'candidate/bias', 'conv', (1, 1), (1, 1), (0, 0))
                for c_ in (self.cell_g, self.cell_c):
                    c_.need_wt = c_.need_wd = False
                self.A2 = torch.zeros(T1, B, 2 * U, device=dev)
                self.ru = torch.empty(T1, B, 2 * U, device=dev)
                self.cand = torch.empty(T1, B, U, device=dev)
                if train:
                    self.dGg = torch.empty(T1, B, 2 * U, device=dev)
                    self.dGc = torch.empty(T1, B, U, device=dev)
            else:
                s = prefix + '%s/rnn/basic_lstm_cell/' % hp.rnn
                self.cell = ConvLayer(store, s + 'kernel', s + 'bias', 'conv', (1, 1), (1, 1), (0, 0))
                self.cell.need_wt = self.cell.need_wd = False
                self.gates = torch.empty(T1, B, 4 * U, device=dev)
                self.cs = torch.empty(T1, B, U, device=dev)
                if train:
                    self.dG = torch.empty(T1, B, 4 * U, device=dev)
            hin = U
        self.mu_fc = ConvLayer(store, prefix + 'z_mu/dense/kernel', prefix + 'z_mu/dense/bias', 'conv', (1, 1), (1, 1), (0, 0))
        self.ls_fc = ConvLayer(store, prefix + 'z_log_sigma_sq/dense/kernel', prefix + 'z_log_sigma_sq/dense/bias', 'conv',
                               (1, 1), (1, 1), (0, 0))
        nz = hp.nz
        self.mu = torch.empty(T1, B, nz, device=dev)
        self.ls_raw = torch.empty(T1, B, nz, device=dev)
        self.ls = torch.empty(T1, B, nz, device=dev)
        self.z = torch.empty(T1, B, nz, device=dev)
        self.dmu = torch.empty(T1, B, nz, device=dev) if train else None
        self.dls = torch.empty(T1, B, nz, device=dev) if train else None
        self.kl = torch.zeros(1, device=dev, dtype=torch.float64)
        self.convs = [L['conv'] for L in self.layers] + ([self.fc] if self.recurrent else []) + [self.mu_fc, self.ls_fc]

    def prep_weights(self):
        prep_layers(self.convs)

    def _head_input(self):
        return self.hout.reshape(self.R, -1) if self.recurrent else self.feat

    def forward(self, images, eps, kl=True, actions=None):
        T1, B, C, M, R, Tc = self.T1, self.B, self.C, self.M, self.R, self.Tc
        if M:
            a = images[:Tc].reshape((M,) + tuple(images.shape[2:]))
            b = images[1:Tc + 1].reshape((M,) + tuple(images.shape[2:]))
            copy_view(a, [self.pairs[..., 0:C]])
            copy_view(b, [self.pairs[..., C:2 * C]])
            if self.na:
                if actions is None:
                    raise ValueError('this encoder was built for inputs with actions')
                K.tile_channels(actions[:Tc].reshape(M, self.na), self.pairs[..., 2 * C:2 * C + self.na])
            for L in self.layers:
                if not L['normed']:
                    L['conv'].forward(L['x'], L['y'], act=lib.ACT_LRELU, alpha=0.2)
                else:
                    L['conv'].forward(L['x'], L['pre'])
                    if self.ln:
                        K.groupnorm_act_fwd(L['pre'], L['gamma'], L['beta'], [L['y']], L['mean'], L['rstd'], groups=1, act='lrelu',
                                            alpha=0.2)
                    else:
                        K.instnorm_act_fwd(L['pre'], L['gamma'], L['beta'], [L['y']], L['mean'], L['rstd'], act='lrelu', alpha=0.2,
                                           eps=EPS_IN)
            last = self.layers[-1]['y']
            self.pooled.zero_()
            K.colsum(last, self.pooled, scale=1.0 / self.hw, per_row=True)
        if self.recurrent:
            U = self.U
            self.fc.forward(self.feat, self.A.reshape(R, 2 * U)[:, :U])
            if self.gru:
                K.gru_seq_fwd(self.A, self.A2, self.cell_g.W, self.cell_g.bias, self.cell_c.W, self.cell_c.bias, self.hout, self.ru,
                              self.cand, U)
            else:
                K.lstm_seq_fwd(self.A, self.cell.W, self.cell.bias, self.hout, self.gates, self.cs, U)
        hin = self._head_input()
        self.mu_fc.forward(hin, self.mu.reshape(R, -1))
        self.ls_fc.forward(hin, self.ls_raw.reshape(R, -1))
        self.eps = eps
        self.kl.zero_()
        K.reparam_fwd(self.mu, self.ls_raw, eps, self.ls, self.z, self.kl if kl else None)
        return self.z

    def backward(self, dz, kl_weight, kl_weight_dev=None):
        self.reparam_backward(dz, kl_weight, kl_weight_dev)
        self.backward_network()

    def reparam_backward(self, dz, kl_weight=0.0, kl_weight_dev=None):
        K.reparam_bwd(self.mu, self.ls_raw, self.eps, dz, kl_weight or 0.0, self.dmu, self.dls, klw_dev=kl_weight_dev)

    def backward_network(self):
        M, R = self.M, self.R
        dmu2, dls2 = self.dmu.reshape(R, -1), self.dls.reshape(R, -1)
        hin = self._head_input()
        dhin = self.dh.reshape(R, -1) if self.recurrent else self.dfeat
        self.mu_fc.backward_data(dmu2, dhin, beta=0)
        self.ls_fc.backward_data(dls2, dhin, beta=1)
        self.mu_fc.backward_weights(hin, dmu2)
        self.ls_fc.backward_weights(hin, dls2)
        if self.recurrent:
            U = self.U
            if self.gru:
                K.gru_seq_bwd(self.A, self.cell_g.W, self.cell_c.W, self.ru, self.cand, self.dh, self.dGg, self.dGc, self.dA, U)
                self.cell_g.backward_weights(self.A.reshape(R, 2 * U), self.dGg.reshape(R, 2 * U))
                self.cell_c.backward_weights(self.A2.reshape(R, 2 * U), self.dGc.reshape(R, U))
            else:
                K.lstm_seq_bwd(self.A, self.cell.W, self.gates, self.cs, self.dh, self.dG, self.dA, U)
                self.cell.backward_weights(self.A.reshape(R, 2 * U), self.dG.reshape(R, 4 * U))
            dx = self.dA.reshape(R, 2 * U)[:, :U]
            self.fc.backward_data(dx, self.dfeat, beta=0)
            self.fc.backward_weights(self.feat, dx)
        if M:
            lastL = self.layers[-1]
            K.tile_channels(self.dpooled, lastL['dy'], scale=1.0 / self.hw)
            for i in range(len(self.layers) - 1, -1, -1):
                L = self.layers[i]
                if L['normed'] and self.ln:
                    K.groupnorm_act_bwd(L['pre'], L['gamma'], L['beta'], L['mean'], L['rstd'], [L['dy']], L['dpre'],
                                        L['dgamma'], L['dbeta'], groups=1, act='lrelu', alpha=0.2)
                if L['normed'] and not self.ln:
                    K.instnorm_act_bwd(L['pre'], L['gamma'], L['beta'], L['y'], L['mean'], L['rstd'], [L['dy']], L['dpre'],
                                       L['dgamma'], L['dbeta'], act='lrelu', alpha=0.2, eps=EPS_IN)
                if L['normed']:
                    dpre = L['dpre']
                else:
                    dpre = L['dy']
                if i > 0:
                    below = self.layers[i - 1]
                    if below['normed']:
                        L['conv'].backward_data(dpre, below['dy'], beta=0)
                    else:
                        L['conv'].backward_data(dpre, below['dy'], beta=0, act=lib.ACT_DLRELU_FROM_OUT, alpha=0.2, aux=below['y'])
                L['conv'].backward_weights(L['x'], dpre)
        for c in self.convs:
            c.finish_weight_grad()


class SNDiscriminator(object):

    def __init__(self, store, hp, image_shape, Nc, prefix, kind='video', train=True):
        H, W, C = image_shape
        self.hp, self.store, self.Nc, self.kind = hp, store, Nc, kind
        self.prefix = prefix
        dev = store.device
        self.dev = dev
        self.frames = 1 if kind == 'image' else hp.clip_length
        self.rows_per_seq = self.frames if kind == 'images' else 1
        self.clip = torch.zeros(Nc, self.frames, H, W, C, device=dev)
        self.dclip = torch.empty(Nc, self.frames, H, W, C, device=dev) if train else None
        self.layers = []
        if kind == 'video':
            layers, flat = video_discriminator_shapes(hp, image_shape)
            x = self.clip
            R = Nc
        else:
            layers, flat = image_discriminator_shapes(hp, image_shape)
            R = Nc * self.frames
            x = self.clip.reshape(R, H, W, C)
            self.x0 = x
            self.dx0 = self.dclip.reshape(R, H, W, C) if train else None
        self.R = R
        for (scope, kshape, st, odims) in layers:
            s = prefix + scope + '/'
            k = kshape[0]
            if kind == 'video':
                conv = ConvLayer(store, s + 'conv3d/kernel', s + 'bias', 'conv', (k, k, k), st, (1, 1, 1), sn_u=s + 'conv3d/u')
            else:
                conv = ConvLayer(store, s + 'conv2d/kernel', s + 'conv2d/bias', 'conv', (k, k), (st, st), (1, 1),
                                 sn_u=s + 'conv2d/u')
            L = {'conv': conv, 'x': x}
            L['y'] = torch.empty((R,) + tuple(odims) + (kshape[-1],), device=dev)
            L['dy'] = torch.empty_like(L['y']) if train else None
            self.layers.append(L)
            x = L['y']
        s = prefix + 'sn_fc4/'
        self.fc = ConvLayer(store, s + 'dense/kernel', s + 'dense/bias', 'conv', (1, 1), (1, 1), (0, 0), sn_u=s + 'dense/u')
        self.flat = flat
        self.logits = torch.empty(R, 1, device=dev)
        self.dlogits = torch.zeros(R, 1, device=dev)
        self.convs = [L['conv'] for L in self.layers] + [self.fc]

    def prep_weights(self, update_u=False):
        batch = os.environ.get('SAVP_SN_BATCH', '1') == '1'
        if batch:
            K.sn_fwd_batch([c.sn_entry(update_u) for c in self.convs])
        prep_layers(self.convs, update_u=update_u, sn_done=batch)

    def commit_u(self):
        for c in self.convs:
            c.commit_u()

    def features(self):
        return [L['y'] for L in self.layers]

    def rows(self, lo, hi):
        return lo * self.rows_per_seq, hi * self.rows_per_seq

    def forward(self, n=None):
        n = (n or self.Nc) * self.rows_per_seq
        for L in self.layers:
            L['conv'].forward(L['x'][:n], L['y'][:n], act=lib.ACT_LRELU, alpha=0.1)
        self.fc.forward(self.layers[-1]['y'][:n].reshape(n, -1), self.logits[:n])
        return self.logits

    def backward(self, lo, hi, weights=True, data=True, feature_grads=False):
        lo, hi = self.rows(lo, hi)
        n = hi - lo
        top = self.layers[-1]
        self.fc.backward_data(self.dlogits[lo:hi], top['dy'][lo:hi].reshape(n, -1), beta=1 if feature_grads else 0,
                              act=lib.ACT_DLRELU_FROM_OUT, alpha=0.1, aux=top['y'][lo:hi].reshape(n, -1))
        if weights:
            self.fc.backward_weights(top['y'][lo:hi].reshape(n, -1), self.dlogits[lo:hi])
        for i in range(len(self.layers) - 1, -1, -1):
            L = self.layers[i]
            dpre = L['dy'][lo:hi]
            if i > 0:
                below = self.layers[i - 1]
                L['conv'].backward_data(dpre, below['dy'][lo:hi], beta=1 if feature_grads else 0,
                                        act=lib.ACT_DLRELU_FROM_OUT, alpha=0.1, aux=below['y'][lo:hi])
            elif data:
                dst = self.dclip if self.kind == 'video' else self.dx0
                L['conv'].backward_data(dpre, dst[lo:hi], beta=0)
            if weights:
                L['conv'].backward_weights(L['x'][lo:hi], dpre)

    def finish_weight_grads(self):
        batch = os.environ.get('SAVP_SN_BATCH', '1') == '1'
        if batch:
            K.sn_bwd_batch([c.sn_bwd_entry() for c in self.convs])
        for c in self.convs:
            c.finish_weight_grad(sn_done=batch)


VideoDiscriminator = SNDiscriminator
```

Before: 10510.

## Add specialized MFMA kernel for video discriminator 3D conv forward

```diff
diff --git a/include/savp_hip.h b/include/savp_hip.h
--- a/include/savp_hip.h
+++ b/include/savp_hip.h
@@ -267,6 +267,7 @@
     const float* src; const float* scale;
     float* wt; float* wd; void* wt_bf16; void* wd_bf16;
     int64_t T; int32_t Cx, Cy;
+    void* wfrag;
 } SavpPackItem;
 int savp_pack_weights_batch(void* stream, int32_t n, const SavpPackItem* items);
 int savp_fold_pool(void* stream, const float* in, float* out, int32_t k, int64_t C, int32_t adjoint);
@@ -383,6 +384,7 @@
                         float* dgen, double* dW, double* db);
 
 int64_t savp_gate_weights_bytes(int32_t taps, int32_t Cx, int32_t Cy);
+int savp_disc3d_shape(int32_t Cx, int32_t k, int32_t sd, int32_t sh, int32_t sw, int32_t Ho, int32_t Wo, int32_t Cy);
 int savp_pack_gate_weights(void* stream, const float* src, int32_t taps, int32_t Cx, int32_t Cy, void* out, int32_t interleave);
 
 int savp_debug_poison_lds(void* stream, uint32_t pattern, void* sink);
diff --git a/video_prediction_amd/csrc/common.hip b/video_prediction_amd/csrc/common.hip
--- a/video_prediction_amd/csrc/common.hip
+++ b/video_prediction_amd/csrc/common.hip
@@ -34,7 +34,7 @@
 
 static struct { const char* name; int value; } g_opts[OPT_COUNT] = {
     {"conv_ring", 0}, {"s2dgrad", 1}, {"thin", 1}, {"wgp_cfg", 0}, {"wgp_split", 0}, {"inorm_min_hw", 64}, {"colsum_2stage", 1},
-    {"dense_legacy", 0}, {"cdna_legacy", 0}, {"lstm_fused", 1}, {"ring_dma", 1}, {"lstm_q", 0}, {"ring_wwarm", 1}, {"wgp_dma", 1}, {"ring_early", 1}, {"gate_kernel", 1}, {"gate_alt", 0}, {"gate_cell", 1}, {"gate_wwarm", 1}, {"splitk_reduced", 0},
+    {"dense_legacy", 0}, {"cdna_legacy", 0}, {"lstm_fused", 1}, {"ring_dma", 1}, {"lstm_q", 0}, {"ring_wwarm", 1}, {"wgp_dma", 1}, {"ring_early", 1}, {"gate_kernel", 1}, {"gate_alt", 0}, {"gate_cell", 1}, {"gate_wwarm", 1}, {"splitk_reduced", 0}, {"disc3d_kernel", 1},
 };
 int savp_opt(int id) { return g_opts[id].value; }
 void savp_opt_count(int id) { ++g_opts[id].value; }
diff --git a/video_prediction_amd/csrc/conv_common.h b/video_prediction_amd/csrc/conv_common.h
--- a/video_prediction_amd/csrc/conv_common.h
+++ b/video_prediction_amd/csrc/conv_common.h
@@ -152,3 +152,5 @@
 bool conv_gate_try(const SavpConvArgs* a, hipStream_t st, int* rc);
 struct SavpConvLstmCellArgs;
 bool conv_gate_cell_try(const SavpConvLstmCellArgs* c, hipStream_t st, int* rc);
+bool conv_disc3d_applies(const SavpConvArgs* a);
+bool conv_disc3d_try(const SavpConvArgs* a, hipStream_t st, int* rc);
diff --git a/video_prediction_amd/csrc/conv_disc3d.hip b/video_prediction_amd/csrc/conv_disc3d.hip
--- /dev/null
+++ b/video_prediction_amd/csrc/conv_disc3d.hip
@@ -0,0 +1,294 @@
+#include "conv_common.h"
+#include "opts.h"
+#include <hip/hip_ext.h>
+#include <type_traits>
+
+extern thread_local hipEvent_t g_savp_prof_start;
+extern thread_local hipEvent_t g_savp_prof_stop;
+
+struct Disc3dP {
+    const float* x; long long x_sn, x_sd, x_sh;
+    const uint4* wfrag;
+    float* y; long long y_sn, y_sd, y_sh;
+    const float* bias;
+    int N, D, H, W, Do, Ho, Wo, Cy;
+    int pd, ph, pw;
+    int act; float alpha; int beta;
+    int ptiles, ctiles;
+};
+
+template <int CIN, int K, int SD, int SH, int SW, int TR, int TC, int WP, int WN, int TN>
+struct D3Cfg {
+    static constexpr int PIX = TR * TC;
+    static constexpr int TM = PIX / (32 * WP);
+    static constexpr int NCW = 32 * TN, NC = NCW * WN;
+    static constexpr int C8 = CIN / 8;
+    static constexpr int C8P = (C8 & 1) ? C8 : C8 + 1;
+    static constexpr int PXB = C8P * 16;
+    static constexpr int PR = (TR - 1) * SH + K;
+    static constexpr int PC = (TC - 1) * SW + K;
+    static constexpr int PCH = (PC + SW - 1) / SW;
+    static constexpr int PCS = PCH * SW;
+    static constexpr int rp_of() {
+        int rp = PCS * PXB;
+        for (int i = 0; i < 64 && ((SH * rp - TC * PXB) % 256 + 256) % 256 != 0; ++i) rp += 16;
+        return rp;
+    }
+    static constexpr int RP = rp_of();
+    static constexpr int PATCHB = PR * RP;
+    static constexpr int KSP = K * K * C8 / 2;
+    static constexpr int KS = K * KSP;
+    static constexpr int ETABB = 2 * KSP * 4 + 64;
+    static constexpr int LDSB = PATCHB + ETABB;
+    static constexpr int PF = 4;
+    static constexpr int PIECES = PR * PCS * C8;
+    static constexpr int aoff(int t) { return ((t * 32) / TC) * SH * RP; }
+    static_assert(CIN % 16 == 0 && PIX % (32 * WP) == 0 && (TM == 1 || TM == 2 || TM == 4) && (TN == 1 || TN == 2) && WP * WN == 4 &&
+                  32 % TC == 0, "shape");
+    static_assert(KSP % PF == 0, "B ring slots are compile-time registers: a plane is a whole number of look-ahead rounds");
+    static_assert(((SH * RP - TC * PXB) % 256 + 256) % 256 == 0, "row pitch");
+    static_assert(LDSB <= 160 * 1024, "LDS");
+};
+
+template <int TM, int TN, int I>
+__device__ __forceinline__ void d3_sched() {
+    constexpr int M = TM * TN, ND = TM + 1, NV = TN;
+    if constexpr (I < M) {
+        constexpr int d = (ND * (I + 1)) / M - (ND * I) / M;
+        constexpr int v = (NV * (I + 1)) / M - (NV * I) / M;
+        if constexpr (d > 0) __builtin_amdgcn_sched_group_barrier(0x100, d, 0);
+        if constexpr (v > 0) __builtin_amdgcn_sched_group_barrier(0x020, v, 0);
+        __builtin_amdgcn_sched_group_barrier(0x008, 1, 0);
+        d3_sched<TM, TN, I + 1>();
+    }
+}
+
+__device__ __forceinline__ uint4 d3_pack8(float4 a, float4 b) {
+    uint4 r;
+    r.x = (unsigned)__builtin_bit_cast(unsigned short, (__bf16)a.x) | ((unsigned)__builtin_bit_cast(unsigned short, (__bf16)a.y) << 16);
+    r.y = (unsigned)__builtin_bit_cast(unsigned short, (__bf16)a.z) | ((unsigned)__builtin_bit_cast(unsigned short, (__bf16)a.w) << 16);
+    r.z = (unsigned)__builtin_bit_cast(unsigned short, (__bf16)b.x) | ((unsigned)__builtin_bit_cast(unsigned short, (__bf16)b.y) << 16);
+    r.w = (unsigned)__builtin_bit_cast(unsigned short, (__bf16)b.z) | ((unsigned)__builtin_bit_cast(unsigned short, (__bf16)b.w) << 16);
+    return r;
+}
+
+template <int CIN, int K, int SD, int SH, int SW, int TR, int TC, int WP, int WN, int TN>
+__global__ __launch_bounds__(256) void conv_disc3d_kernel(Disc3dP p) {
+    using G = D3Cfg<CIN, K, SD, SH, SW, TR, TC, WP, WN, TN>;
+    constexpr int TM = G::TM, KSP = G::KSP, KS = G::KS, PF = G::PF, C8 = G::C8;
+    extern __shared__ __attribute__((aligned(16))) unsigned char dsm[];
+    unsigned char* patch = dsm;
+    unsigned* etab = reinterpret_cast<unsigned*>(dsm + G::PATCHB);
+    const int tid = threadIdx.x, lane = tid & 63;
+    const int wave = __builtin_amdgcn_readfirstlane(tid >> 6);
+    const int wn = wave % WN, wp = wave / WN;
+    const int l31 = lane & 31, khalf = lane >> 5;
+
+    const int logical = xcd_logical((int)blockIdx.x, p.ptiles * p.ctiles);
+    const int pt = logical / p.ctiles, ct = logical - pt * p.ctiles;
+    const int tpr = p.Wo / TC, tpp = (p.Ho / TR) * tpr;
+    const int plane = pt / tpp, rem = pt - plane * tpp;
+    const int n = plane / p.Do, od = plane - n * p.Do;
+    const int oy0 = (rem / tpr) * TR, ox0 = (rem % tpr) * TC;
+    const int n0 = ct * G::NC;
+
+    for (int c = tid; c < 2 * KSP + 16; c += 256) {
+        const int cc = c < 2 * KSP ? c : 0;
+        const int tap = cc / C8, ch = cc - tap * C8;
+        const int kh = tap / K, kw = tap % K;
+        etab[c] = (unsigned)(kh * G::RP + ((kw % SW) * G::PCH + kw / SW) * G::PXB + ch * 16);
+    }
+
+    const uint4* __restrict__ bsrc[TN];
+#pragma unroll
+    for (int j = 0; j < TN; ++j) bsrc[j] = p.wfrag + ((long long)(n0 / 32 + wn * TN + j) * KS) * 64 + lane;
+    const unsigned a0 = (unsigned)((wp * TM * 32 / TC) * SH * G::RP + (l31 / TC) * SH * G::RP + (l31 % TC) * G::PXB);
+    const unsigned* etl = etab + khalf;
+
+    f32x16 acc[TM][TN];
+#pragma unroll
+    for (int i = 0; i < TM; ++i)
+#pragma unroll
+        for (int j = 0; j < TN; ++j)
+#pragma unroll
+            for (int r = 0; r < 16; ++r) acc[i][j][r] = 0.f;
+
+    const int iy0 = oy0 * SH - p.ph, ix0 = ox0 * SW - p.pw;
+    const unsigned char* xn = reinterpret_cast<const unsigned char*>(p.x + (long long)n * p.x_sn);
+    for (int kd = 0; kd < K; ++kd) {
+        const int d = od * SD - p.pd + kd;
+        if ((unsigned)d >= (unsigned)p.D) continue;
+        uint4 bq[PF][TN];
+#pragma unroll
+        for (int u = 0; u < PF; ++u)
+#pragma unroll
+            for (int j = 0; j < TN; ++j) bq[u][j] = bsrc[j][(long long)(kd * KSP + u) * 64];
+        __syncthreads();
+        {
+            const float* xd = reinterpret_cast<const float*>(xn) + (long long)d * p.x_sd;
+            constexpr int U = 8;
+            for (int base = 0; base < G::PIECES; base += 256 * U) {
+                float4 v[U][2];
+                unsigned dst[U];
+#pragma unroll
+                for (int u = 0; u < U; ++u) {
+                    const int q = base + u * 256 + tid;
+                    const int pix = q / C8, ch = q - pix * C8;
+                    const int row = pix / G::PCS, slot = pix - row * G::PCS;
+                    const int col = (slot / G::PCH) + (slot % G::PCH) * SW;
+                    const int iy = iy0 + row, ix = ix0 + col;
+                    const bool ok = q < G::PIECES && col < G::PC && (unsigned)iy < (unsigned)p.H && (unsigned)ix < (unsigned)p.W;
+                    dst[u] = q < G::PIECES ? (unsigned)(row * G::RP + slot * G::PXB + ch * 16) : 0xffffffffu;
+                    if (ok) {
+                        const float* s = xd + (long long)iy * p.x_sh + (long long)ix * CIN + ch * 8;
+                        v[u][0] = *reinterpret_cast<const float4*>(s);
+                        v[u][1] = *reinterpret_cast<const float4*>(s + 4);
+                    } else {
+                        v[u][0] = make_float4(0.f, 0.f, 0.f, 0.f);
+                        v[u][1] = v[u][0];
+                    }
+                }
+#pragma unroll
+                for (int u = 0; u < U; ++u)
+                    if (dst[u] != 0xffffffffu) *reinterpret_cast<uint4*>(patch + dst[u]) = d3_pack8(v[u][0], v[u][1]);
+            }
+        }
+        __syncthreads();
+
+        bf16x8 af[2][TM];
+        auto load_a = [&](bf16x8 (&dst)[TM], unsigned off) {
+            const unsigned char* a = patch + a0 + off;
+#pragma unroll
+            for (int i = 0; i < TM; ++i) dst[i] = *reinterpret_cast<const bf16x8*>(a + G::aoff(i));
+        };
+        load_a(af[0], etl[0]);
+        unsigned off_next = etl[2];
+        const uint4* __restrict__ bk[TN];
+#pragma unroll
+        for (int j = 0; j < TN; ++j) bk[j] = bsrc[j] + (long long)(kd * KSP) * 64;
+        auto kstep = [&](int k, auto uc) {
+            constexpr int u = decltype(uc)::value;
+            load_a(af[(u + 1) & 1], off_next);
+            off_next = etl[2 * (k + 2)];
+            bf16x8 bf[TN];
+#pragma unroll
+            for (int j = 0; j < TN; ++j) bf[j] = __builtin_bit_cast(bf16x8, bq[u][j]);
+#pragma unroll
+            for (int i = 0; i < TM; ++i)
+#pragma unroll
+                for (int j = 0; j < TN; ++j) acc[i][j] = __builtin_amdgcn_mfma_f32_32x32x16_bf16(af[u & 1][i], bf[j], acc[i][j], 0, 0, 0);
+#pragma unroll
+            for (int j = 0; j < TN; ++j) bq[u][j] = bk[j][(long long)(k + PF) * 64];
+            d3_sched<TM, TN, 0>();
+        };
+        using U0 = std::integral_constant<int, 0>; using U1 = std::integral_constant<int, 1>;
+        using U2 = std::integral_constant<int, 2>; using U3 = std::integral_constant<int, 3>;
+        for (int k = 0; k < KSP; k += 4) {
+            kstep(k, U0{}); kstep(k + 1, U1{}); kstep(k + 2, U2{}); kstep(k + 3, U3{});
+        }
+    }
+
+    const float alpha = p.alpha;
+#pragma unroll
+    for (int j = 0; j < TN; ++j) {
+        const int col = n0 + (wn * TN + j) * 32 + l31;
+        const float b = p.bias ? p.bias[col] : 0.f;
+        float* yc = p.y + (long long)n * p.y_sn + (long long)od * p.y_sd + col;
+#pragma unroll
+        for (int i = 0; i < TM; ++i)
+#pragma unroll
+            for (int r = 0; r < 16; ++r) {
+                const int px = (wp * TM + i) * 32 + (r & 3) + 8 * (r >> 2) + 4 * khalf;
+                const int oy = oy0 + px / TC, ox = ox0 + px % TC;
+                float* dst = yc + (long long)oy * p.y_sh + (long long)ox * p.Cy;
+                float v = acc[i][j][r] + b;
+                if (p.beta) v += *dst;
+                if (p.act == SAVP_ACT_LRELU) v = fmaxf(v, alpha * v);
+                *dst = v;
+            }
+    }
+}
+
+template <int CIN, int K, int SD, int SH, int SW, int TR, int TC, int WP, int WN, int TN>
+static hipError_t launch_disc3d(Disc3dP& p, hipStream_t st) {
+    using G = D3Cfg<CIN, K, SD, SH, SW, TR, TC, WP, WN, TN>;
+    auto kern = conv_disc3d_kernel<CIN, K, SD, SH, SW, TR, TC, WP, WN, TN>;
+    static bool attr = false;
+    if (!attr) {
+        if (hipFuncSetAttribute(reinterpret_cast<const void*>(kern), hipFuncAttributeMaxDynamicSharedMemorySize, G::LDSB) != hipSuccess)
+            return hipErrorInvalidValue;
+        attr = true;
+    }
+    p.ptiles = p.N * p.Do * (p.Ho / TR) * (p.Wo / TC);
+    p.ctiles = p.Cy / G::NC;
+    const dim3 grid((unsigned)(p.ptiles * p.ctiles));
+    if (g_savp_prof_start) {
+        hipExtLaunchKernelGGL(kern, grid, dim3(256), G::LDSB, st, g_savp_prof_start, g_savp_prof_stop, 0, p);
+        g_savp_prof_start = g_savp_prof_stop = nullptr;
+    } else {
+        hipLaunchKernelGGL(kern, grid, dim3(256), G::LDSB, st, p);
+    }
+    return hipGetLastError();
+}
+
+#define DISC3D_SHAPES(X)                                                                                                  \
+    X(32, 4, 1, 2, 2, 32, 32, 8, 16, 4, 1, 2)                          \
+    X(64, 3, 1, 1, 1, 32, 32, 8, 16, 4, 1, 2)                                         \
+    X(64, 4, 1, 2, 2, 16, 16, 8, 16, 2, 2, 2)                                           \
+    X(128, 4, 2, 2, 2, 8, 8, 8, 8, 2, 2, 2)                                               \
+    X(256, 3, 1, 1, 1, 8, 8, 8, 8, 2, 2, 2)
+
+static bool disc3d_shape_of(int Cx, int k, int sd, int sh, int sw, int Ho, int Wo, int Cy) {
+#define X(C_, K_, SD_, SH_, SW_, HO_, WO_, TR_, TC_, WP_, WN_, TN_)                                                    \
+    if (Cx == C_ && k == K_ && sd == SD_ && sh == SH_ && sw == SW_ && Ho == HO_ && Wo == WO_ && Cy % (32 * WN_ * TN_) == 0) return true;
+    DISC3D_SHAPES(X)
+#undef X
+    return false;
+}
+
+static bool disc3d_shape(const SavpConvArgs* a) {
+    return a->kd == a->kh && a->kd == a->kw && disc3d_shape_of(a->Cx, a->kd, a->sd, a->sh, a->sw, a->Ho, a->Wo, a->Cy);
+}
+
+extern "C" int savp_disc3d_shape(int32_t Cx, int32_t k, int32_t sd, int32_t sh, int32_t sw, int32_t Ho, int32_t Wo, int32_t Cy) {
+    return disc3d_shape_of(Cx, k, sd, sh, sw, Ho, Wo, Cy) ? 1 : 0;
+}
+
+bool conv_disc3d_applies(const SavpConvArgs* a) {
+    if (!savp_opt(OPT_DISC3D_KERNEL)) return false;
+    if (!(a->mode == SAVP_CONV_FPROP && a->precision == SAVP_PREC_BF16 && !a->src_bf16 && !a->out_bf16 && a->w_frag && !a->aux && !a->stats &&
+          !a->dst_gap && !a->nb_ws && (a->act == SAVP_ACT_NONE || a->act == SAVP_ACT_LRELU)))
+        return false;
+    if (!(a->kd == a->kh && a->kd == a->kw && a->sh == a->sw && a->pd == 1 && a->ph == 1 && a->pw == 1 && a->N >= 1))
+        return false;
+    if (!(a->Do == (a->D + 2 - a->kd) / a->sd + 1 && a->Ho == (a->H + 2 - a->kh) / a->sh + 1 && a->Wo == (a->W + 2 - a->kw) / a->sw + 1))
+        return false;
+    if (!(a->x_sw == a->Cx && a->y_sw == a->Cy && a->y_sh == (long long)a->Wo * a->Cy && aligned16(a->x) && aligned16(a->w_frag) &&
+          a->x_sh % 4 == 0 && a->x_sd % 4 == 0 && a->x_sn % 4 == 0 && a->x_sh >= (long long)a->W * a->Cx))
+        return false;
+    return disc3d_shape(a);
+}
+
+bool conv_disc3d_try(const SavpConvArgs* a, hipStream_t st, int* rc) {
+    if (!conv_disc3d_applies(a)) return false;
+    Disc3dP p;
+    p.x = (const float*)a->x; p.x_sn = a->x_sn; p.x_sd = a->x_sd; p.x_sh = a->x_sh;
+    p.wfrag = (const uint4*)a->w_frag;
+    p.y = (float*)a->y; p.y_sn = a->y_sn; p.y_sd = a->y_sd; p.y_sh = a->y_sh;
+    p.bias = a->bias;
+    p.N = a->N; p.D = a->D; p.H = a->H; p.W = a->W; p.Do = a->Do; p.Ho = a->Ho; p.Wo = a->Wo; p.Cy = a->Cy;
+    p.pd = a->pd; p.ph = a->ph; p.pw = a->pw;
+    p.act = a->act; p.alpha = a->alpha; p.beta = a->beta;
+    hipError_t err = hipErrorInvalidValue;
+    bool done = false;
+#define X(C_, K_, SD_, SH_, SW_, HO_, WO_, TR_, TC_, WP_, WN_, TN_)                                                    \
+    if (!done && a->Cx == C_ && a->kd == K_ && a->sd == SD_ && a->sh == SH_ && a->sw == SW_ && a->Ho == HO_ && a->Wo == WO_ && \
+        a->Cy % (32 * WN_ * TN_) == 0) {                                                                               \
+        err = launch_disc3d<C_, K_, SD_, SH_, SW_, TR_, TC_, WP_, WN_, TN_>(p, st);                                    \
+        done = true;                                                                                                   \
+    }
+    DISC3D_SHAPES(X)
+#undef X
+    *rc = err == hipSuccess ? SAVP_OK : SAVP_ELAUNCH;
+    return true;
+}
diff --git a/video_prediction_amd/csrc/conv_igemm.hip b/video_prediction_amd/csrc/conv_igemm.hip
--- a/video_prediction_amd/csrc/conv_igemm.hip
+++ b/video_prediction_amd/csrc/conv_igemm.hip
@@ -775,7 +775,7 @@
 }
 
 extern "C" int savp_conv_special(const SavpConvArgs* a) {
-    if (a && conv_gate_applies(a)) return 1;
+    if (a && (conv_gate_applies(a) || conv_disc3d_applies(a))) return 1;
     if (!a || ((a->tile >> 8) & 3) != 0) return 0;
     return (conv_thin_applies(a) || conv_s2dgrad_applies(a) || conv_gate_applies(a)) ? 1 : 0;
 }
@@ -848,6 +848,7 @@
     if (a->mode == SAVP_CONV_FPROP) {
         int rc = SAVP_OK;
         if (conv_gate_try(a, st, &rc)) return rc;
+        if (conv_disc3d_try(a, st, &rc)) return rc;
     }
     if (a->mode == SAVP_CONV_FPROP || a->mode == SAVP_CONV_DGRAD) {
         const bool dg = a->mode == SAVP_CONV_DGRAD;
diff --git a/video_prediction_amd/csrc/opts.h b/video_prediction_amd/csrc/opts.h
--- a/video_prediction_amd/csrc/opts.h
+++ b/video_prediction_amd/csrc/opts.h
@@ -21,6 +21,7 @@
     OPT_GATE_CELL,
     OPT_GATE_WWARM,
     OPT_SPLITK_REDUCED,
+    OPT_DISC3D_KERNEL,
     OPT_COUNT
 };
 
diff --git a/video_prediction_amd/csrc/weight_prep.hip b/video_prediction_amd/csrc/weight_prep.hip
--- a/video_prediction_amd/csrc/weight_prep.hip
+++ b/video_prediction_amd/csrc/weight_prep.hip
@@ -53,7 +53,7 @@
 #define PACK_MAX 32
 struct PackBatch {
     const float* src[PACK_MAX]; const float* scale[PACK_MAX];
-    float* wt[PACK_MAX]; float* wd[PACK_MAX]; __bf16* wt16[PACK_MAX]; __bf16* wd16[PACK_MAX];
+    float* wt[PACK_MAX]; float* wd[PACK_MAX]; __bf16* wt16[PACK_MAX]; __bf16* wd16[PACK_MAX]; __bf16* wfrag[PACK_MAX];
     long long T[PACK_MAX]; int Cx[PACK_MAX], Cy[PACK_MAX];
 };
 
@@ -65,7 +65,7 @@
     const long long T = b.T[it];
     const int Cx = b.Cx[it], Cy = b.Cy[it];
     float* __restrict__ wt = b.wt[it]; float* __restrict__ wd = b.wd[it];
-    __bf16* __restrict__ wt16 = b.wt16[it]; __bf16* __restrict__ wd16 = b.wd16[it];
+    __bf16* __restrict__ wt16 = b.wt16[it]; __bf16* __restrict__ wd16 = b.wd16[it]; __bf16* __restrict__ wfrag = b.wfrag[it];
     const long long R = T * Cx;
     const float s = b.scale[it] ? *b.scale[it] : 1.f;
     const int tc = (Cy + PK_T - 1) / PK_T;
@@ -90,7 +90,7 @@
             }
         }
         __syncthreads();
-        if (wt || wt16) {
+        if (wt || wt16 || wfrag) {
 #pragma unroll 4
             for (int j = ty; j < PK_T; j += 4) {
                 const int cy = c0 + j;
@@ -99,6 +99,7 @@
                     const float v = tile[tx][j];
                     if (wt) wt[(long long)cy * R + r] = v;
                     if (wt16) wt16[(long long)cy * R + r] = (__bf16)v;
+                    if (wfrag) wfrag[((((long long)(cy >> 5) * (R >> 4) + (r >> 4)) * 64 + ((r >> 3) & 1) * 32 + (cy & 31)) << 3) + (r & 7)] = (__bf16)v;
                 }
             }
         }
@@ -111,9 +112,10 @@
     long long most = 0;
     for (int i = 0; i < n; ++i) {
         const SavpPackItem& q = items[i];
-        if (!q.src || (!q.wt && !q.wd && !q.wt_bf16 && !q.wd_bf16) || q.T < 1 || q.Cx < 1 || q.Cy < 1) return SAVP_EINVAL;
+        if (!q.src || (!q.wt && !q.wd && !q.wt_bf16 && !q.wd_bf16 && !q.wfrag) || q.T < 1 || q.Cx < 1 || q.Cy < 1) return SAVP_EINVAL;
+        if (q.wfrag && (q.Cx % 16 || q.Cy % 32)) return SAVP_EINVAL;
         b.src[i] = q.src; b.scale[i] = q.scale; b.wt[i] = q.wt; b.wd[i] = q.wd;
-        b.wt16[i] = (__bf16*)q.wt_bf16; b.wd16[i] = (__bf16*)q.wd_bf16;
+        b.wt16[i] = (__bf16*)q.wt_bf16; b.wd16[i] = (__bf16*)q.wd_bf16; b.wfrag[i] = (__bf16*)q.wfrag;
         b.T[i] = q.T; b.Cx[i] = q.Cx; b.Cy[i] = q.Cy;
         const long long tiles = (((long long)q.T * q.Cx + PK_T - 1) / PK_T) * ((q.Cy + PK_T - 1) / PK_T);
         if (tiles > most) most = tiles;
diff --git a/video_prediction_amd/engine.py b/video_prediction_amd/engine.py
--- a/video_prediction_amd/engine.py
+++ b/video_prediction_amd/engine.py
@@ -240,6 +240,7 @@
         self.need_wt = self.need_wd = True
         self.wfrag = None
         self.wfrag_il = None
+        self.wfrag3 = None
         self.prof = None
         self.ktimer = None
 
@@ -268,7 +269,8 @@
             src = self.wfp
         b16 = K.PRECISION['value'] == 1
         entry = {'src': src, 'wt': self.wt if self.need_wt else None, 'wd': self.wd if self.need_wd else None, 'scale': scale,
-                 'wt16': self.wt16 if (b16 and self.need_wt) else None, 'wd16': self.wd16 if (b16 and self.need_wd) else None}
+                 'wt16': self.wt16 if (b16 and self.need_wt) else None, 'wd16': self.wd16 if (b16 and self.need_wd) else None,
+                 'wfrag': self.wfrag3 if b16 else None}
         if defer_pack is not None:
             defer_pack.append(entry)
         else:
@@ -285,6 +287,14 @@
                 self.wfrag = torch.empty(n, device=self.W.device, dtype=torch.bfloat16)
                 if cell and self.cy % 32 == 0:
                     self.wfrag_il = torch.empty(n, device=self.W.device, dtype=torch.bfloat16)
+
+    def enable_disc3d_pack(self, out_hw):
+        k, s, p = self.geom.k, self.geom.s, self.geom.p
+        if (self.kind == 'conv' and not self.padded and k[0] == k[1] == k[2] and tuple(p) == (1, 1, 1) and
+                lib.get().savp_disc3d_shape(self.cx, k[0], s[0], s[1], s[2], out_hw[0], out_hw[1], self.cy)):
+            n = K.gate_weights_elems(self.taps, self.cx, self.cy)
+            if n:
+                self.wfrag3 = torch.zeros(n, device=self.W.device, dtype=torch.bfloat16)
 
     def commit_u(self):
         if self.sn_u_name:
@@ -304,7 +314,7 @@
                 return K.conv(lib.CONV_DGRAD, self.geom, y, x, self.wd, bias=b, beta=beta, act=act, alpha=alpha, w16=self.wd16, stats=stats,
                               defer=True)
             return K.conv(lib.CONV_FPROP, self.geom, x, y, self.wt, bias=b, beta=beta, act=act, alpha=alpha, w16=self.wt16, stats=stats,
-                          defer=True, w_frag=self.wfrag, w_frag_il=self.wfrag_il)
+                          defer=True, w_frag=self.wfrag if self.wfrag is not None else self.wfrag3, w_frag_il=self.wfrag_il)
         if self.ktimer is not None:
             self.ktimer.arm()
         if self.prof is not None:
@@ -313,7 +323,8 @@
         if self.kind == 'up':
             K.conv(lib.CONV_DGRAD, self.geom, y, x, self.wd, bias=b, beta=beta, act=act, alpha=alpha, w16=self.wd16, stats=stats)
         else:
-            K.conv(lib.CONV_FPROP, self.geom, x, y, self.wt, bias=b, beta=beta, act=act, alpha=alpha, w16=self.wt16, stats=stats, w_frag=self.wfrag)
+            K.conv(lib.CONV_FPROP, self.geom, x, y, self.wt, bias=b, beta=beta, act=act, alpha=alpha, w16=self.wt16, stats=stats,
+                   w_frag=self.wfrag if self.wfrag is not None else self.wfrag3)
         if self.prof is not None:
             e1.record()
             self.prof.append((e0, e1))
diff --git a/video_prediction_amd/kernels.py b/video_prediction_amd/kernels.py
--- a/video_prediction_amd/kernels.py
+++ b/video_prediction_amd/kernels.py
@@ -1161,7 +1161,9 @@
     acc.finish()
 
 
-def pack_weights(src, wt=None, wd=None, scale=None, wt16=None, wd16=None):
+def pack_weights(src, wt=None, wd=None, scale=None, wt16=None, wd16=None, wfrag=None):
+    if wfrag is not None:
+        return pack_weights_batch([dict(src=src, wt=wt, wd=wd, scale=scale, wt16=wt16, wd16=wd16, wfrag=wfrag)])
     Cx, Cy = src.shape[-2], src.shape[-1]
     T = src.numel() // (Cx * Cy)
     lib.check(_L().savp_pack_weights(lib.stream(), _p(src), T, Cx, Cy, _p(scale), _p(wt), _p(wd), _p(wt16), _p(wd16)),
@@ -1178,6 +1180,7 @@
             it = arr[i]
             it.src, it.scale = _p(src), _p(e.get('scale'))
             it.wt, it.wd, it.wt_bf16, it.wd_bf16 = _p(e.get('wt')), _p(e.get('wd')), _p(e.get('wt16')), _p(e.get('wd16'))
+            it.wfrag = _p(e.get('wfrag'))
             it.Cx, it.Cy = src.shape[-2], src.shape[-1]
             it.T = src.numel() // (it.Cx * it.Cy)
         lib.check(_L().savp_pack_weights_batch(lib.stream(), len(part), arr), 'savp_pack_weights_batch')
diff --git a/video_prediction_amd/lib.py b/video_prediction_amd/lib.py
--- a/video_prediction_amd/lib.py
+++ b/video_prediction_amd/lib.py
@@ -81,7 +81,8 @@
 
 
 OPTION_NAMES = ('conv_ring', 's2dgrad', 'thin', 'wgp_cfg', 'wgp_split', 'inorm_min_hw', 'colsum_2stage', 'dense_legacy', 'cdna_legacy',
-                'lstm_fused', 'ring_dma', 'lstm_q', 'ring_wwarm', 'wgp_dma', 'ring_early', 'gate_kernel', 'gate_alt', 'gate_cell', 'gate_wwarm', 'splitk_reduced')
+                'lstm_fused', 'ring_dma', 'lstm_q', 'ring_wwarm', 'wgp_dma', 'ring_early', 'gate_kernel', 'gate_alt', 'gate_cell', 'gate_wwarm', 'splitk_reduced',
+                'disc3d_kernel')
 
 
 def set_option(name, value):
@@ -123,6 +124,7 @@
     _sig(lib, 'savp_conv_workspace_bytes', [P(SavpConvArgs)], restype=c_i64)
     _sig(lib, 'savp_conv_special', [P(SavpConvArgs)])
     _sig(lib, 'savp_gate_weights_bytes', [c_i32, c_i32, c_i32], restype=c_i64)
+    _sig(lib, 'savp_disc3d_shape', [c_i32] * 8)
     _sig(lib, 'savp_conv_stats_ok', [P(SavpConvArgs)])
     _sig(lib, 'savp_set_option', [ctypes.c_char_p, c_i32])
     _sig(lib, 'savp_get_option', [ctypes.c_char_p, P(c_i32)])
@@ -343,7 +345,7 @@
 register('savp_fold_bilinear', [c_vp, c_vp, c_vp, c_i32, c_i32, c_i32, c_i32])
 class SavpPackItem(ctypes.Structure):
     _fields_ = [('src', c_vp), ('scale', c_vp), ('wt', c_vp), ('wd', c_vp), ('wt_bf16', c_vp), ('wd_bf16', c_vp), ('T', c_i64),
-                ('Cx', c_i32), ('Cy', c_i32)]
+                ('Cx', c_i32), ('Cy', c_i32), ('wfrag', c_vp)]
 
 
 register('savp_pack_weights_batch', [c_vp, c_i32, ctypes.POINTER(SavpPackItem)])
diff --git a/video_prediction_amd/models/networks.py b/video_prediction_amd/models/networks.py
--- a/video_prediction_amd/models/networks.py
+++ b/video_prediction_amd/models/networks.py
@@ -235,6 +235,7 @@
             k = kshape[0]
             if kind == 'video':
                 conv = ConvLayer(store, s + 'conv3d/kernel', s + 'bias', 'conv', (k, k, k), st, (1, 1, 1), sn_u=s + 'conv3d/u')
+                conv.enable_disc3d_pack(tuple(odims)[1:3])
             else:
                 conv = ConvLayer(store, s + 'conv2d/kernel', s + 'conv2d/bias', 'conv', (k, k), (st, st), (1, 1),
                                  sn_u=s + 'conv2d/u')
```

Measured after the change: 10790 (median of 6 runs). 1.03x the previous value.
